# rajgandhi1/threecrate

Hardware: AMD Instinct MI355X
Metric: ICP iterations/sec (whole job: k=16 normals + 50-iter point-to-plane ICP per 1M-pt pair; tc_cloud handles, inputs resident in HBM) (higher is better)
Workload: dtype f32; 1 GPU; 1000000-pt uniform-random cloud, k=16 normals + 50-iter point-to-plane ICP, independent sigma = 0.0001 noise on source and target, correspondences returned (BASELINE configs[1]; one independent pair per GPU); points=1000000, k=16, parallelism=pairs1, interface=tc_cloud handles (one index build per cloud)

## Files before the change

threecrate_amd/csrc/cloud.hip:

```cpp
#include "tc_internal.h"

#include <algorithm>
#include <cmath>
#include <cstring>

struct tc_cloud {
    tc_context *ctx = nullptr;
    size_t n = 0;
    tc::DevBuf xyz;
    tc::DeviceIndex ix;
    bool indexed = false;
    float factor = 0.0f;
    bool has_normals = false;
    tc::DevBuf normals6;
    bool has_normals6 = false;
};

namespace {

using namespace tc;


float shared_factor(float want) {
    return (want > 0.8f * kIcpCellFactor && want < 1.25f * kIcpCellFactor) ? kIcpCellFactor : want;
}

__global__ void __launch_bounds__(256) cloud_unsort_normals_kernel(const float4 *__restrict__ pts, const float4 *__restrict__ sorted_nrm,
                                                                  const float *__restrict__ xyz, uint32_t n, float *__restrict__ out6) {
    const uint32_t p = blockIdx.x * blockDim.x + threadIdx.x;
    if (p >= n) return;
    const uint32_t orig = __float_as_uint(pts[p].w);
    const float4 nr = sorted_nrm[p];
    float *o = out6 + 6 * (size_t)orig;
    o[0] = xyz[3 * (size_t)orig]; o[1] = xyz[3 * (size_t)orig + 1]; o[2] = xyz[3 * (size_t)orig + 2];
    o[3] = nr.x; o[4] = nr.y; o[5] = nr.z;
}

tc_status ensure_index(tc_cloud *c, float want_factor, float target_ppo, float min_h) {
    tc_context *ctx = c->ctx;
    const float f = shared_factor(want_factor);
    if (c->indexed && c->factor > 0.8f * f && c->factor < 1.25f * f && min_h <= c->ix.geom.h) return TC_OK;
    if (c->has_normals && !c->has_normals6 && c->indexed && c->n) {
        if (tc_status s = ensure(ctx, c->normals6, c->n * 6 * sizeof(float))) return s;
        hipLaunchKernelGGL(cloud_unsort_normals_kernel, dim3((unsigned)((c->n + 255) / 256)), dim3(256), 0, ctx->stream,
                           (const float4 *)c->ix.pts.p, (const float4 *)c->ix.normals.p, (const float *)c->xyz.p, (uint32_t)c->n,
                           (float *)c->normals6.p);
        TC_HIP_TRY(ctx, hipGetLastError());
        c->has_normals6 = true;
    }
    c->has_normals = false;
    if (tc_status s = build_index(ctx, c->ix, (const float *)c->xyz.p, c->n, f, nullptr, nullptr, nullptr, min_h, target_ppo)) return s;
    c->indexed = true;
    c->factor = f;
    return TC_OK;
}

tc_status cloud_create(tc_context *ctx, const float *p, size_t n, bool from_host, tc_cloud **out) {
    if (!ctx || !out) return TC_INVALID_DATA;
    *out = nullptr;
    if (tc_status s = check_point_count(ctx, n)) return s;
    TC_HIP_TRY(ctx, hipSetDevice(ctx->device));
    tc_cloud *c = new tc_cloud();
    c->ctx = ctx;
    c->n = n;
    if (n) {
        tc_status s = ensure(ctx, c->xyz, n * 3 * sizeof(float));
        if (s == TC_OK && hipMemcpyAsync(c->xyz.p, p, n * 3 * sizeof(float), from_host ? hipMemcpyHostToDevice : hipMemcpyDeviceToDevice,
                                         ctx->stream) != hipSuccess) s = fail(ctx, TC_GPU, "cloud upload failed");
        if (s == TC_OK && from_host && hipStreamSynchronize(ctx->stream) != hipSuccess) s = fail(ctx, TC_GPU, "cloud upload failed");
        if (s != TC_OK) { recycle(ctx, c->xyz); delete c; return s; }
    }
    *out = c;
    return TC_OK;
}

tc_status adopt_normals(tc_cloud *c, const float *d_normals, size_t stride) {
    if (tc_status s = ensure_index(c, kIcpCellFactor, 2.5f, 0.0f)) return s;
    if (tc_status s = gather_normals(c->ctx, c->ix, d_normals, stride)) return s;
    c->has_normals = true;
    return TC_OK;
}

tc_status prepare_target(tc_cloud *tgt, bool p2plane);

tc_status cloud_icp(tc_cloud *src, tc_cloud *tgt, bool p2plane, const float init[7], size_t max_iters, float max_dist, float conv_thr,
                    tc_icp_result *res) {
    if (!src || !tgt || !res || !init) return TC_INVALID_DATA;
    tc_context *ctx = tgt->ctx;
    if (src->ctx != ctx) return fail(ctx, TC_INVALID_DATA, "source and target handles belong to different contexts");
    if (src->n == 0 || tgt->n == 0) return fail(ctx, TC_INVALID_DATA, "Source or target point cloud is empty");
    if (p2plane && !tgt->has_normals && !tgt->has_normals6)
        return fail(ctx, TC_INVALID_DATA, "target_normals length must equal the number of target points (the target handle has no normals: "
                                          "tc_cloud_estimate_normals or tc_cloud_set_normals_device first)");
    if (max_iters == 0) return fail(ctx, TC_INVALID_DATA, "Max iterations must be positive");
    TC_HIP_TRY(ctx, hipSetDevice(ctx->device));
    if (tc_status s = prepare_target(tgt, p2plane)) return s;
    return icp_run(ctx, p2plane, (const float *)src->xyz.p, src->n, (const float *)tgt->xyz.p, tgt->n, nullptr, 0, init, max_iters, max_dist,
                   conv_thr, res, true, 0, &tgt->ix, (src->indexed && src != tgt) ? &src->ix : nullptr);
}

tc_status prepare_target(tc_cloud *tgt, bool p2plane) {
    tc_context *ctx = tgt->ctx;
    if (tc_status s = ensure_index(tgt, kIcpCellFactor, 2.5f, 0.0f)) return s;
    if (p2plane && !tgt->has_normals) {
        if (!tgt->has_normals6) return fail(ctx, TC_INVALID_DATA, "the target handle has no normals in input order to re-sort after its index was rebuilt");
        if (tc_status s = gather_normals(ctx, tgt->ix, (const float *)tgt->normals6.p + 3, 6)) return s;
        tgt->has_normals = true;
    }
    return TC_OK;
}

}

extern "C" {

tc_status tc_cloud_sharded_icp(tc_comm *comm, int shard_mode, int point_to_plane, const float *d_source, size_t n_source, tc_cloud *target,
                               const float init[7], size_t max_iters, float max_dist, float conv_thr, tc_icp_result *result) try {
    if (!comm || !target || !result || !init) return TC_INVALID_DATA;
    tc_context *ctx = target->ctx;
    if (comm->ctx != ctx) return fail(ctx, TC_INVALID_DATA, "the communicator belongs to another context");
    if (shard_mode != TC_SHARD_SPATIAL && shard_mode != TC_SHARD_LOCAL && shard_mode != TC_SHARD_INDEX) return fail(ctx, TC_INVALID_DATA, "unknown shard mode");
    const bool may_be_empty = shard_mode == TC_SHARD_LOCAL && comm->nranks > 1;
    if ((n_source == 0 && !may_be_empty) || target->n == 0) return fail(ctx, TC_INVALID_DATA, "Source or target point cloud is empty");
    if (point_to_plane && !target->has_normals && !target->has_normals6)
        return fail(ctx, TC_INVALID_DATA, "target_normals length must equal the number of target points (the target handle has no normals)");
    if (max_iters == 0) return fail(ctx, TC_INVALID_DATA, "Max iterations must be positive");
    TC_HIP_TRY(ctx, hipSetDevice(ctx->device));
    if (tc_status s = prepare_target(target, point_to_plane != 0)) return s;
    return icp_run_sharded(ctx, comm, shard_mode, point_to_plane != 0, d_source, n_source, (const float *)target->xyz.p, target->n, nullptr, 0, init,
                           max_iters, max_dist, conv_thr, result, &target->ix);
} TC_CATCH_STATUS((comm ? comm->ctx : nullptr))

tc_status tc_cloud_upload(tc_context *ctx, const float *xyz, size_t n, tc_cloud **out) try { return cloud_create(ctx, xyz, n, true, out); } TC_CATCH_STATUS(ctx)
tc_status tc_cloud_upload_device(tc_context *ctx, const float *d_xyz, size_t n, tc_cloud **out) try { return cloud_create(ctx, d_xyz, n, false, out); } TC_CATCH_STATUS(ctx)
size_t tc_cloud_size(const tc_cloud *c) { return c ? c->n : 0; }
const float *tc_cloud_points_device(const tc_cloud *c) { return c ? (const float *)c->xyz.p : nullptr; }
const float *tc_cloud_normals_device(const tc_cloud *cc) try {
    tc_cloud *c = const_cast<tc_cloud *>(cc);
    if (!c || c->n == 0) return nullptr;
    if (c->has_normals6) return (const float *)c->normals6.p;
    if (!c->has_normals || !c->indexed) return nullptr;
    tc_context *ctx = c->ctx;
    if (hipSetDevice(ctx->device) != hipSuccess) { (void)fail(ctx, TC_GPU, "tc_cloud_normals_device: hipSetDevice failed"); return nullptr; }
    if (ensure(ctx, c->normals6, c->n * 6 * sizeof(float)) != TC_OK) return nullptr;
    hipLaunchKernelGGL(cloud_unsort_normals_kernel, dim3((unsigned)((c->n + 255) / 256)), dim3(256), 0, ctx->stream,
                       (const float4 *)c->ix.pts.p, (const float4 *)c->ix.normals.p, (const float *)c->xyz.p, (uint32_t)c->n,
                       (float *)c->normals6.p);
    hipError_t e = hipGetLastError();
    if (e == hipSuccess) e = hipStreamSynchronize(ctx->stream);
    if (e != hipSuccess) { (void)fail(ctx, TC_GPU, std::string("tc_cloud_normals_device: ") + hipGetErrorString(e)); return nullptr; }
    c->has_normals6 = true;
    return (const float *)c->normals6.p;
} TC_CATCH_VALUE(nullptr)

static tc_status cloud_normals(tc_cloud *c, const tc_normal_config *cfg, float *out, bool out_on_host, bool keep6) {
    if (!c || !cfg) return TC_INVALID_DATA;
    tc_context *ctx = c->ctx;
    if (c->n == 0) return TC_OK;
    if (cfg->k_neighbors < 3) return fail(ctx, TC_INVALID_DATA, "k_neighbors must be at least 3");
    TC_HIP_TRY(ctx, hipSetDevice(ctx->device));
    const float min_h = cfg->has_radius ? cfg->radius * 0.5005f : 0.0f;
    c->has_normals = false;
    c->has_normals6 = false;
    if (tc_status s = ensure_index(c, normals_cell_factor(cfg->k_neighbors, c->n >= kAdaptMinPoints), normals_target_ppo(cfg->k_neighbors), min_h)) return s;
    if (tc_status s = ensure(ctx, c->ix.normals, c->n * sizeof(float4))) return s;
    const bool direct = out != nullptr && !out_on_host && !keep6;
    const bool want6 = (out != nullptr || keep6) && !direct;
    float *d_out6 = direct ? out : nullptr;
    if (want6) {
        if (tc_status s = ensure(ctx, c->normals6, c->n * 6 * sizeof(float))) return s;
        d_out6 = (float *)c->normals6.p;
    }
    c->has_normals = false;
    c->has_normals6 = false;
    if (tc_status s = normals_on_index(ctx, c->ix, false, 0.0f, (const float *)c->xyz.p, c->n, cfg, d_out6, 0, (size_t)-1, false,
                                       (float4 *)c->ix.normals.p, true)) return s;
    c->has_normals = true;
    c->has_normals6 = want6;
    if (out && !direct) TC_HIP_TRY(ctx, hipMemcpyAsync(out, d_out6, c->n * 6 * sizeof(float), out_on_host ? hipMemcpyDeviceToHost : hipMemcpyDeviceToDevice, ctx->stream));
    TC_HIP_TRY(ctx, hipStreamSynchronize(ctx->stream));
    return TC_OK;
}

tc_status tc_cloud_estimate_normals(tc_cloud *c, const tc_normal_config *cfg, float *out) try { return cloud_normals(c, cfg, out, true, false); } TC_CATCH_STATUS(c ? c->ctx : nullptr)
tc_status tc_cloud_estimate_normals_device(tc_cloud *c, const tc_normal_config *cfg, float *d_out) try { return cloud_normals(c, cfg, d_out, false, false); } TC_CATCH_STATUS(c ? c->ctx : nullptr)

tc_status tc_cloud_set_normals_device(tc_cloud *c, const float *d_normals, size_t n_normals, size_t stride) try {
    if (!c) return TC_INVALID_DATA;
    tc_context *ctx = c->ctx;
    if (n_normals != c->n) return fail(ctx, TC_INVALID_DATA, "target_normals length must equal the number of target points");
    if (stride < 3) return fail(ctx, TC_INVALID_DATA, "normal_stride must be >= 3");
    if (c->n == 0) return TC_OK;
    TC_HIP_TRY(ctx, hipSetDevice(ctx->device));
    c->has_normals = false;
    c->has_normals6 = false;
    if (tc_status s = adopt_normals(c, d_normals, stride)) return s;
    TC_HIP_TRY(ctx, hipStreamSynchronize(ctx->stream));
    return TC_OK;
} TC_CATCH_STATUS((c ? c->ctx : nullptr))

tc_status tc_cloud_icp_point_to_plane(tc_cloud *source, tc_cloud *target, const float init[7], size_t max_iters, float max_dist,
                                      float conv_thr, tc_icp_result *result) try {
    return cloud_icp(source, target, true, init, max_iters, max_dist, conv_thr, result);
} TC_CATCH_STATUS((source ? source->ctx : nullptr))

tc_status tc_cloud_icp_detailed(tc_cloud *source, tc_cloud *target, const float init[7], size_t max_iters, float max_dist,
                                float conv_thr, tc_icp_result *result) try {
    return cloud_icp(source, target, false, init, max_iters, max_dist, conv_thr, result);
} TC_CATCH_STATUS((source ? source->ctx : nullptr))

void tc_cloud_destroy(tc_cloud *c) try {
    if (!c) return;
    (void)hipSetDevice(c->ctx->device);
    (void)hipStreamSynchronize(c->ctx->stream);
    tc::recycle(c->ctx, c->xyz); tc::recycle(c->ctx, c->normals6);
    tc::recycle_index(c->ctx, c->ix);
    delete c;
} TC_CATCH_VOID

}
```

threecrate_amd/csrc/grid.hip:

```cpp
#include "tc_internal.h"
#include <rocprim/device/device_radix_sort.hpp>

#include <algorithm>
#include <cmath>
#include <cstring>

namespace tc {

__device__ __forceinline__ void isometry_apply(const float q[4], const float t[3], float x, float y, float z,
                                               float &ox, float &oy, float &oz) {
    float tx = (q[1] * z - q[2] * y) * 2.0f;
    float ty = (q[2] * x - q[0] * z) * 2.0f;
    float tz = (q[0] * y - q[1] * x) * 2.0f;
    float cx = q[1] * tz - q[2] * ty;
    float cy = q[2] * tx - q[0] * tz;
    float cz = q[0] * ty - q[1] * tx;
    ox = ((tx * q[3] + cx) + x) + t[0];
    oy = ((ty * q[3] + cy) + y) + t[1];
    oz = ((tz * q[3] + cz) + z) + t[2];
}

constexpr int kBboxBlocks = 256;
__device__ __forceinline__ uint32_t f2ord(float f) { const uint32_t b = __float_as_uint(f); return (b & 0x80000000u) ? ~b : (b | 0x80000000u); }
__device__ __forceinline__ float ord2f(uint32_t u) { return __uint_as_float((u & 0x80000000u) ? (u ^ 0x80000000u) : ~u); }
constexpr uint32_t kOrdPlusInf = 0xFF800000u, kOrdMinusInf = 0x007FFFFFu;
constexpr uint32_t kBboxAccStride = 32;
constexpr size_t kBboxStateBytes = 31 * kBboxAccStride * sizeof(uint32_t), kBboxBufBytes = kBboxStateBytes + 128 + 256;

template <bool VEC>
__global__ void __launch_bounds__(256) bbox_kernel(const float *__restrict__ xyz, uint32_t n, uint32_t *__restrict__ state, int robust,
                                                  float *__restrict__ out, uint32_t *__restrict__ done) {
    const bool sbox = robust != 0;
    __shared__ float sm[4][30];
    float v[30];
#pragma unroll
    for (int k = 0; k < 30; ++k) v[k] = (k % 6 < 3) ? INFINITY : -INFINITY;
    auto take = [&](float x, float y, float z, uint32_t i, int s) {
        if (!(fabsf(x) <= 3.0e38f && fabsf(y) <= 3.0e38f && fabsf(z) <= 3.0e38f)) return;
        v[0] = fminf(v[0], x); v[1] = fminf(v[1], y); v[2] = fminf(v[2], z);
        v[3] = fmaxf(v[3], x); v[4] = fmaxf(v[4], y); v[5] = fmaxf(v[5], z);
        if (sbox && ((i * 2654435761u) >> 28) == 0u) {
            float *b = v + 6 + 6 * s;
            b[0] = fminf(b[0], x); b[1] = fminf(b[1], y); b[2] = fminf(b[2], z);
            b[3] = fmaxf(b[3], x); b[4] = fmaxf(b[4], y); b[5] = fmaxf(b[5], z);
        }
    };
    const uint32_t gt = blockIdx.x * blockDim.x + threadIdx.x, stride = gridDim.x * blockDim.x;
    if constexpr (VEC) {
        const float4 *__restrict__ q = reinterpret_cast<const float4 *>(xyz);
        const uint32_t nq = n >> 2;
        constexpr int U = 4;
        for (uint32_t c0 = gt; c0 < nq; c0 += U * stride) {
            float4 a[U], b[U], c[U];
#pragma unroll
            for (int u = 0; u < U; ++u) {
                const uint32_t cc = min(c0 + (uint32_t)u * stride, nq - 1u);
                a[u] = q[3 * (size_t)cc]; b[u] = q[3 * (size_t)cc + 1]; c[u] = q[3 * (size_t)cc + 2];
            }
#pragma unroll
            for (int u = 0; u < U; ++u) {
                const uint32_t i = 4u * min(c0 + (uint32_t)u * stride, nq - 1u);
                take(a[u].x, a[u].y, a[u].z, i, 0);
                take(a[u].w, b[u].x, b[u].y, i + 1u, 1);
                take(b[u].z, b[u].w, c[u].x, i + 2u, 2);
                take(c[u].y, c[u].z, c[u].w, i + 3u, 3);
            }
        }
        if (gt < (n & 3u)) {
            const uint32_t i = (nq << 2) + gt;
            const float x = xyz[3 * (size_t)i], y = xyz[3 * (size_t)i + 1], z = xyz[3 * (size_t)i + 2];
            if ((i & 3u) == 0u) take(x, y, z, i, 0); else if ((i & 3u) == 1u) take(x, y, z, i, 1); else take(x, y, z, i, 2);
        }
    } else {
        for (uint32_t i = gt; i < n; i += stride) {
            const float x = xyz[3 * (size_t)i], y = xyz[3 * (size_t)i + 1], z = xyz[3 * (size_t)i + 2];
            const uint32_t sidx = threadIdx.x & 3u;
            if (sidx == 0u) take(x, y, z, i, 0); else if (sidx == 1u) take(x, y, z, i, 1); else if (sidx == 2u) take(x, y, z, i, 2); else take(x, y, z, i, 3);
        }
    }
#pragma unroll
    for (int k = 0; k < 30; ++k) {
        if (k < 6 || sbox) {
#pragma unroll
            for (int o = 32; o > 0; o >>= 1) {
                const float w = __shfl_xor(v[k], o);
                v[k] = (k % 6 < 3) ? fminf(v[k], w) : fmaxf(v[k], w);
            }
        }
    }
    if ((threadIdx.x & 63) == 0) {
#pragma unroll
        for (int k = 0; k < 30; ++k) sm[threadIdx.x >> 6][k] = v[k];
    }
    __syncthreads();
    uint32_t *acc = state + kBboxAccStride;
    if (threadIdx.x < (sbox ? 30 : 6)) {
        const bool is_min = threadIdx.x % 6 < 3;
        float r = sm[0][threadIdx.x];
        for (int w = 1; w < 4; ++w) r = is_min ? fminf(r, sm[w][threadIdx.x]) : fmaxf(r, sm[w][threadIdx.x]);
        if (is_min) atomicMin(&acc[threadIdx.x * kBboxAccStride], f2ord(r)); else atomicMax(&acc[threadIdx.x * kBboxAccStride], f2ord(r));
    }
    __shared__ uint32_t s_last;
    if (threadIdx.x < 64) {
        asm volatile("s_waitcnt vmcnt(0)" ::: "memory");
        if (threadIdx.x == 0) s_last = __hip_atomic_fetch_add(state, 1u, __ATOMIC_RELAXED, __HIP_MEMORY_SCOPE_AGENT) == gridDim.x - 1u ? 1u : 0u;
    }
    __syncthreads();
    if (!s_last) return;
    if (threadIdx.x < 30) {
        const uint32_t u = __hip_atomic_load(&acc[threadIdx.x * kBboxAccStride], __ATOMIC_RELAXED, __HIP_MEMORY_SCOPE_AGENT);
        __hip_atomic_store(&out[threadIdx.x], ord2f(u), __ATOMIC_RELAXED, __HIP_MEMORY_SCOPE_SYSTEM);
        __hip_atomic_store(&acc[threadIdx.x * kBboxAccStride], (threadIdx.x % 6 < 3) ? kOrdPlusInf : kOrdMinusInf, __ATOMIC_RELAXED, __HIP_MEMORY_SCOPE_AGENT);
    }
    if (threadIdx.x == 0) __hip_atomic_store(state, 0u, __ATOMIC_RELAXED, __HIP_MEMORY_SCOPE_AGENT);
    if (done) {
        if (threadIdx.x < 30) __threadfence_system();
        __syncthreads();
        if (threadIdx.x == 0) __hip_atomic_store(done, 1u, __ATOMIC_RELEASE, __HIP_MEMORY_SCOPE_SYSTEM);
    }
}

__global__ void bbox_state_init_kernel(uint32_t *__restrict__ state) {
    const uint32_t t = threadIdx.x;
    if (t == 0) state[0] = 0u;
    if (t < 30) state[(t + 1) * kBboxAccStride] = (t % 6 < 3) ? kOrdPlusInf : kOrdMinusInf;
}


__global__ void __launch_bounds__(256) cell_hist_kernel(const float *__restrict__ xyz, uint32_t n, GridGeom g,
                                                       const IcpState *__restrict__ st, TileGeom tg, int tile_major, uint32_t nkeys,
                                                       uint32_t *__restrict__ cell_of, uint32_t *__restrict__ hist,
                                                       uint32_t *__restrict__ arrival, uint32_t *__restrict__ pts_pad,
                                                       uint32_t *__restrict__ cs_front, uint32_t *__restrict__ cs_tail, uint32_t rank_max) {
    uint32_t i = blockIdx.x * blockDim.x + threadIdx.x;
    if (blockIdx.x == 0 && threadIdx.x < 4 * kPtsPad + kCellStartFront + kCellStartPad) {
        const uint32_t t = threadIdx.x;
        if (t < 4 * kPtsPad) pts_pad[t] = 0x7F7F7F7Fu;
        else if (t < 4 * kPtsPad + kCellStartFront) cs_front[t - 4 * kPtsPad] = 0u;
        else cs_tail[t - 4 * kPtsPad - kCellStartFront] = 0u;
    }
    if (i >= n) return;
    float x = xyz[3 * (size_t)i], y = xyz[3 * (size_t)i + 1], z = xyz[3 * (size_t)i + 2];
    if (st) {
        float q[4] = {st->q[0], st->q[1], st->q[2], st->q[3]}, t[3] = {st->t[0], st->t[1], st->t[2]};
        float ox, oy, oz;
        isometry_apply(q, t, x, y, z, ox, oy, oz);
        x = ox; y = oy; z = oz;
    }
    int ix = cell_coord(x, g.minx, g.inv_h, g.gx);
    int iy = cell_coord(y, g.miny, g.inv_h, g.gy);
    int iz = cell_coord(z, g.minz, g.inv_h, g.gz);
    uint32_t c = tile_major ? tile_major_id(tg, ix, iy, iz) : ((uint32_t)iz * g.gy + iy) * g.gx + ix;
    if (!(fabsf(x) <= 3.0e38f && fabsf(y) <= 3.0e38f && fabsf(z) <= 3.0e38f)) c = nkeys;
    cell_of[i] = c;
    const uint32_t a = atomicAdd(&hist[c], 1u);
    arrival[i] = a;
    if (a == rank_max) hist[nkeys + 1] = 1u;
}

__global__ void __launch_bounds__(256) iota_kernel(uint32_t *__restrict__ p, uint32_t n) {
    const uint32_t i = blockIdx.x * blockDim.x + threadIdx.x;
    if (i < n) p[i] = i;
}

constexpr int kScanItems = 8;
constexpr int kScanBlock = 256;
constexpr int kScanTile = kScanItems * kScanBlock;

__global__ void __launch_bounds__(kScanBlock) scan_reduce_kernel(const uint32_t *__restrict__ in, uint32_t n,
                                                                 uint32_t *__restrict__ blocksum) {
    __shared__ uint32_t wsum[kScanBlock / 64], wnz[kScanBlock / 64];
    uint32_t base = blockIdx.x * kScanTile;
    uint32_t s = 0, nz = 0;
#pragma unroll
    for (int k = 0; k < kScanItems; ++k) {
        uint32_t i = base + k * kScanBlock + threadIdx.x;
        if (i < n) { const uint32_t v = in[i]; s += v; nz += v != 0; }
    }
#pragma unroll
    for (int o = 32; o > 0; o >>= 1) { s += __shfl_xor(s, o); nz += __shfl_xor(nz, o); }
    if ((threadIdx.x & 63) == 0) { wsum[threadIdx.x >> 6] = s; wnz[threadIdx.x >> 6] = nz; }
    __syncthreads();
    if (threadIdx.x == 0) {
        blocksum[blockIdx.x] = wsum[0] + wsum[1] + wsum[2] + wsum[3];
        blocksum[gridDim.x + blockIdx.x] = wnz[0] + wnz[1] + wnz[2] + wnz[3];
    }
}

constexpr uint32_t kScanFusedMax = 2048;
__global__ void __launch_bounds__(1024) scan_top_kernel(uint32_t *__restrict__ blocksum, uint32_t nb) {
    __shared__ uint32_t wtot[16];
    uint32_t carry = 0;
    for (uint32_t base = 0; base < nb; base += 1024) {
        const uint32_t i = base + threadIdx.x;
        const uint32_t v = i < nb ? blocksum[i] : 0u;
        uint32_t inc = v;
#pragma unroll
        for (int o = 1; o < 64; o <<= 1) {
            const uint32_t t = __shfl_up(inc, o);
            if ((threadIdx.x & 63) >= (unsigned)o) inc += t;
        }
        if ((threadIdx.x & 63) == 63) wtot[threadIdx.x >> 6] = inc;
        __syncthreads();
        uint32_t woff = 0, tot = 0;
        for (int w = 0; w < 16; ++w) { if (w < (int)(threadIdx.x >> 6)) woff += wtot[w]; tot += wtot[w]; }
        if (i < nb) blocksum[i] = carry + woff + inc - v;
        carry += tot;
        __syncthreads();
    }
}

__global__ void __launch_bounds__(kScanBlock) scan_apply_kernel(const uint32_t *__restrict__ in, uint32_t n,
                                                                uint32_t *__restrict__ blocksum,
                                                                uint32_t *__restrict__ out , uint32_t *__restrict__ occ_out, int prefixed,
                                                                unsigned long long *__restrict__ occ_host) {
    __shared__ uint32_t wtot[kScanBlock / 64];
    __shared__ uint32_t wpre[kScanBlock / 64], wnz[kScanBlock / 64];
    uint32_t pre = 0, nzt = 0;
    if (prefixed) { if (threadIdx.x == 0) pre = blocksum[blockIdx.x]; }
    else for (uint32_t i = threadIdx.x; i < blockIdx.x; i += kScanBlock) pre += blocksum[i];
    if (blockIdx.x == 0) for (uint32_t i = threadIdx.x; i < gridDim.x; i += kScanBlock) nzt += blocksum[gridDim.x + i];
#pragma unroll
    for (int o = 32; o > 0; o >>= 1) { pre += __shfl_xor(pre, o); nzt += __shfl_xor(nzt, o); }
    if ((threadIdx.x & 63) == 0) { wpre[threadIdx.x >> 6] = pre; wnz[threadIdx.x >> 6] = nzt; }
    uint32_t base = blockIdx.x * kScanTile + threadIdx.x * kScanItems;
    uint32_t v[kScanItems];
    uint32_t s = 0;
#pragma unroll
    for (int k = 0; k < kScanItems; ++k) {
        uint32_t i = base + k;
        v[k] = (i < n) ? in[i] : 0;
        s += v[k];
    }
    uint32_t inc = s;
#pragma unroll
    for (int o = 1; o < 64; o <<= 1) {
        uint32_t t = __shfl_up(inc, o);
        if ((threadIdx.x & 63) >= (unsigned)o) inc += t;
    }
    if ((threadIdx.x & 63) == 63) wtot[threadIdx.x >> 6] = inc;
    __syncthreads();
    uint32_t woff = 0;
    for (int w = 0; w < (int)(threadIdx.x >> 6); ++w) woff += wtot[w];
    uint32_t block_pre = 0;
    for (int w = 0; w < kScanBlock / 64; ++w) block_pre += wpre[w];
    if (blockIdx.x == 0 && threadIdx.x == 0) {
        uint32_t t = 0;
        for (int w = 0; w < kScanBlock / 64; ++w) t += wnz[w];
        blocksum[2 * gridDim.x] = t;
        if (occ_out) *occ_out = t;
        if (occ_host) __hip_atomic_store(occ_host, (1ull << 32) | (unsigned long long)t, __ATOMIC_RELAXED, __HIP_MEMORY_SCOPE_SYSTEM);
    }
    uint32_t run = block_pre + woff + inc - s;
#pragma unroll
    for (int k = 0; k < kScanItems; ++k) {
        uint32_t i = base + k;
        if (i < n) out[i] = run;
        run += v[k];
        if (i == n - 1) out[n] = run;
    }
}

__global__ void __launch_bounds__(256) rank_gather_kernel(const float *__restrict__ xyz, uint32_t n, uint32_t nkeys,
                                                         const uint32_t *__restrict__ cell_of,
                                                         const uint32_t *__restrict__ cell_start,
                                                         const uint32_t *__restrict__ slot,
                                                         float4 *__restrict__ pts, int slot_is_ordered, uint32_t rank_max) {
    uint32_t p = blockIdx.x * blockDim.x + threadIdx.x;
    if (p >= n) return;
    uint32_t i = slot[p];
    uint32_t c = cell_of[i];
    uint32_t s = cell_start[c], e = cell_start[c + 1];
    uint32_t rank;
    if (slot_is_ordered) {
        rank = p - s;
    } else if (e - s <= rank_max) {
        rank = 0;
        for (uint32_t j = s; j < e; ++j) rank += (slot[j] < i) ? 1u : 0u;
    } else {
        rank = p - s;
    }
    float4 r;
    r.x = xyz[3 * (size_t)i]; r.y = xyz[3 * (size_t)i + 1]; r.z = xyz[3 * (size_t)i + 2];
    if (c == nkeys) r.x = r.y = r.z = __uint_as_float(0x7F7F7F7Fu);
    r.w = __uint_as_float(i);
    pts[s + rank] = r;
}

__global__ void __launch_bounds__(256) place_kernel(const float *__restrict__ xyz, uint32_t n, uint32_t nkeys,
                                                   const uint32_t *__restrict__ cell_of, const uint32_t *__restrict__ cell_start,
                                                   const uint32_t *__restrict__ arrival, float4 *__restrict__ tmp) {
    const uint32_t i = blockIdx.x * blockDim.x + threadIdx.x;
    if (i >= n) return;
    const uint32_t c = cell_of[i];
    const uint32_t pos = cell_start[c] + arrival[i];
    float4 r;
    r.x = xyz[3 * (size_t)i]; r.y = xyz[3 * (size_t)i + 1]; r.z = xyz[3 * (size_t)i + 2];
    if (c == nkeys) r.x = r.y = r.z = __uint_as_float(0x7F7F7F7Fu);
    r.w = __uint_as_float(i);
    tmp[pos] = r;
}

__global__ void __launch_bounds__(256) rerank_kernel(uint32_t n, GridGeom g, const IcpState *__restrict__ st, TileGeom tg, int tile_major,
                                                    uint32_t nkeys, const uint32_t *__restrict__ cell_start, const float4 *__restrict__ tmp,
                                                    float4 *__restrict__ pts, uint32_t rank_max) {
    const uint32_t p = blockIdx.x * blockDim.x + threadIdx.x;
    if (p >= n) return;
    const float4 r = tmp[p];
    uint32_t c;
    {
        float x = r.x, y = r.y, z = r.z;
        if (st) {
            float q[4] = {st->q[0], st->q[1], st->q[2], st->q[3]}, t[3] = {st->t[0], st->t[1], st->t[2]};
            float ox, oy, oz;
            isometry_apply(q, t, x, y, z, ox, oy, oz);
            x = ox; y = oy; z = oz;
        }
        const int ix = cell_coord(x, g.minx, g.inv_h, g.gx), iy = cell_coord(y, g.miny, g.inv_h, g.gy), iz = cell_coord(z, g.minz, g.inv_h, g.gz);
        c = tile_major ? tile_major_id(tg, ix, iy, iz) : ((uint32_t)iz * g.gy + iy) * g.gx + ix;
        if (!(fabsf(x) <= 3.0e38f && fabsf(y) <= 3.0e38f && fabsf(z) <= 3.0e38f)) c = nkeys;
    }
    const uint32_t s = cell_start[c], e = cell_start[c + 1];
    const uint32_t i = __float_as_uint(r.w);
    uint32_t rank;
    if (e - s <= rank_max) {
        rank = 0;
#pragma unroll 4
        for (uint32_t j = s; j < e; ++j) rank += (__float_as_uint(tmp[j].w) < i) ? 1u : 0u;
    } else {
        rank = p - s;
    }
    pts[s + rank] = r;
}

__global__ void __launch_bounds__(256) gather_normals_kernel(const float4 *__restrict__ pts, uint32_t n,
                                                            const float *__restrict__ nrm, size_t stride,
                                                            float4 *__restrict__ out) {
    uint32_t p = blockIdx.x * blockDim.x + threadIdx.x;
    if (p >= n) return;
    uint32_t i = __float_as_uint(pts[p].w);
    const float *s = nrm + (size_t)i * stride;
    out[p] = make_float4(s[0], s[1], s[2], 0.0f);
}

GridView view_of(const DeviceIndex &ix) {
    GridView v;
    v.g = ix.geom;
    v.pts = (const float4 *)ix.pts.p;
    v.cell_start = (const uint32_t *)ix.cell_start.p + kCellStartFront;
    v.pts12 = ix.pts12_valid ? (const float *)ix.pts12.p : nullptr;
    return v;
}

static void set_cell_edge(GridGeom &g, double h, size_t n, double cells_per_point) {
    const double e[3] = {(double)g.maxx - g.minx, (double)g.maxy - g.miny, (double)g.maxz - g.minz};
    const double max_cells = std::max<double>(cells_per_point * (double)n, 4096.0);
    for (int guard = 0; guard < 200; ++guard) {
        double gx = std::floor(e[0] / h) + 1.0, gy = std::floor(e[1] / h) + 1.0, gz = std::floor(e[2] / h) + 1.0;
        if (gx * gy * gz <= max_cells && gx * gy * gz < 2.0e9) {
            g.gx = (int)gx; g.gy = (int)gy; g.gz = (int)gz;
            break;
        }
        h *= 1.2;
    }
    g.h = (float)h;
    g.inv_h = 1.0f / g.h;
    g.ncell = (uint32_t)g.gx * (uint32_t)g.gy * (uint32_t)g.gz;
    g.n = (uint32_t)n;
}

static void derive_geom(GridGeom &g, const float mn[3], const float mx[3], size_t n, float f, float min_h) {
    g.minx = mn[0]; g.miny = mn[1]; g.minz = mn[2];
    g.maxx = mx[0]; g.maxy = mx[1]; g.maxz = mx[2];
    g.cx = 0.5f * (mn[0] + mx[0]); g.cy = 0.5f * (mn[1] + mx[1]); g.cz = 0.5f * (mn[2] + mx[2]);
    double e[3] = {(double)mx[0] - mn[0], (double)mx[1] - mn[1], (double)mx[2] - mn[2]};
    double emax = std::max(e[0], std::max(e[1], e[2]));
    double h = 1.0;
    if (!(emax > 0.0) || !std::isfinite(emax)) {
        h = 1.0;
    } else {
        double measure = 1.0;
        int dims = 0;
        for (int a = 0; a < 3; ++a)
            if (e[a] > 1e-6 * emax) { measure *= e[a]; ++dims; }
        h = f * std::pow(measure / (double)std::max<size_t>(n, 1), 1.0 / (double)dims);
        if (!(h > 0.0) || !std::isfinite(h)) h = emax;
        h = std::max(h, emax * 1e-4);
    }
    if (min_h > 0.0f && std::isfinite(min_h)) h = std::max(h, (double)min_h);
    set_cell_edge(g, h, n, 8.0);
}

TileGeom make_tiles(const GridGeom &g, int tx, int ty, int tz) {
    TileGeom t;
    t.tx = std::max(tx, 1); t.ty = std::max(ty, 1); t.tz = std::max(tz, 1);
    t.ntx = (g.gx + t.tx - 1) / t.tx; t.nty = (g.gy + t.ty - 1) / t.ty; t.ntz = (g.gz + t.tz - 1) / t.tz;
    t.cpt = (uint32_t)(t.tx * t.ty * t.tz);
    t.ntiles = (uint32_t)t.ntx * (uint32_t)t.nty * (uint32_t)t.ntz;
    return t;
}

tc_status exclusive_scan_u32(tc_context *ctx, const uint32_t *d_in, uint32_t n, uint32_t *d_out, DevBuf &blocksum, uint32_t *occ_out,
                             unsigned long long *occ_host) {
    hipStream_t st = ctx->stream;
    const uint32_t nscan = (n + kScanTile - 1) / kScanTile;
    if (tc_status s = ensure(ctx, blocksum, ((size_t)2 * nscan + 1) * sizeof(uint32_t))) return s;
    hipLaunchKernelGGL(scan_reduce_kernel, dim3(nscan), dim3(kScanBlock), 0, st, d_in, n, (uint32_t *)blocksum.p);
    const char *fm = getenv("TC_SCAN_FUSED_MAX");
    const bool prefixed = nscan > (fm ? (uint32_t)atoi(fm) : kScanFusedMax);
    if (prefixed) hipLaunchKernelGGL(scan_top_kernel, dim3(1), dim3(1024), 0, st, (uint32_t *)blocksum.p, nscan);
    hipLaunchKernelGGL(scan_apply_kernel, dim3(nscan), dim3(kScanBlock), 0, st, d_in, n, (uint32_t *)blocksum.p, d_out, occ_out, prefixed ? 1 : 0, occ_host);
    TC_HIP_TRY(ctx, hipGetLastError());
    return TC_OK;
}

static tc_status cloud_bbox_impl(tc_context *ctx, const float *d_xyz, size_t n, float mn[3], float mx[3], float *rmn, float *rmx,
                                 bool *clamped) {
    hipStream_t st = ctx->stream;
    const int nb = (int)((n + 255) / 256);
    const int bb = std::min(nb, kBboxBlocks);
    const bool robust = rmn != nullptr && n >= 4096;
    const bool poll = pinned_poll_enabled();
    const bool fresh = ctx->bbox.p == nullptr;
    if (tc_status s = ensure(ctx, ctx->bbox, kBboxBufBytes)) return s;
    uint32_t *d_state = (uint32_t *)ctx->bbox.p;
    if (fresh) hipLaunchKernelGGL(bbox_state_init_kernel, dim3(1), dim3(64), 0, st, d_state);
    float *hb = (float *)((char *)ctx->pinned + 2048);
    volatile uint32_t *h_done = (volatile uint32_t *)((char *)ctx->pinned + 2048 + 8192 + 192);
    float *d_out = (float *)((char *)ctx->bbox.p + kBboxStateBytes + 128);
    uint32_t *d_done = nullptr;
    if (poll) {
        d_out = (float *)pinned_dev_ptr(ctx, hb);
        d_done = (uint32_t *)pinned_dev_ptr(ctx, (const void *)h_done);
        if (!d_out || !d_done) return fail(ctx, TC_GPU, "bbox: the pinned block has no device address");
        *h_done = 0u;
    }
    {
        ProfScope ps(ctx, "bbox");
        if (((uintptr_t)d_xyz & 15u) == 0u)
            hipLaunchKernelGGL(bbox_kernel<true>, dim3(std::min((int)((n / 4 + 255) / 256) + 1, kBboxBlocks)), dim3(256), 0, st, d_xyz, (uint32_t)n, d_state, robust ? 1 : 0, d_out, d_done);
        else
            hipLaunchKernelGGL(bbox_kernel<false>, dim3(bb), dim3(256), 0, st, d_xyz, (uint32_t)n, d_state, robust ? 1 : 0, d_out, d_done);
    }
    TC_HIP_TRY(ctx, hipGetLastError());
    if (poll) {
        if (tc_status s = wait_pinned_word(ctx, h_done, "bounding box")) { hipLaunchKernelGGL(bbox_state_init_kernel, dim3(1), dim3(64), 0, st, d_state); return s; }
    } else {
        TC_HIP_TRY(ctx, hipMemcpyAsync(hb, d_out, 30 * sizeof(float), hipMemcpyDeviceToHost, st));
        TC_HIP_TRY(ctx, hipStreamSynchronize(st));
    }
    const float *hs = hb + 6;
    for (int c = 0; c < 3; ++c) { mn[c] = INFINITY; mx[c] = -INFINITY; }
    for (int c = 0; c < 3; ++c) { mn[c] = std::fmin(mn[c], hb[c]); mx[c] = std::fmax(mx[c], hb[3 + c]); }
    if (rmn) {
        for (int c = 0; c < 3; ++c) { rmn[c] = mn[c]; rmx[c] = mx[c]; }
        *clamped = false;
    }
    if (!robust) return TC_OK;
    float acc[24];
    for (int i = 0; i < 24; ++i) acc[i] = (i % 6 < 3) ? INFINITY : -INFINITY;
    for (int i = 0; i < 24; ++i) acc[i] = (i % 6 < 3) ? (hs[i] < acc[i] ? hs[i] : acc[i]) : (hs[i] > acc[i] ? hs[i] : acc[i]);
    for (int c = 0; c < 3; ++c) {
        float lo[4], hi[4];
        for (int k = 0; k < 4; ++k) { lo[k] = acc[6 * k + c]; hi[k] = acc[6 * k + 3 + c]; }
        std::sort(lo, lo + 4);
        std::sort(hi, hi + 4, [](float a, float b) { return a > b; });
        const float slo = lo[2], shi = hi[2];
        if (!(slo <= shi) || !std::isfinite(slo) || !std::isfinite(shi)) continue;
        const float ext = shi - slo, full = mx[c] - mn[c];
        if (!(full > 1.3f * ext) || !(full > 0.0f)) continue;
        rmn[c] = std::fmax(mn[c], slo - 0.05f * ext);
        rmx[c] = std::fmin(mx[c], shi + 0.05f * ext);
        *clamped = true;
    }
    return TC_OK;
}

tc_status cloud_bbox(tc_context *ctx, const float *d_xyz, size_t n, float mn[3], float mx[3]) {
    return cloud_bbox_impl(ctx, d_xyz, n, mn, mx, nullptr, nullptr, nullptr);
}


constexpr int kBinBlocks = 256;
constexpr int kBinWalkThreads = 1024;
#ifndef TC_BIN_TARGET
#define TC_BIN_TARGET 2048
#endif
#ifndef TC_BIN_PLACE_THREADS
#define TC_BIN_PLACE_THREADS 512
#endif
constexpr uint32_t kBinTarget = TC_BIN_TARGET;
constexpr uint32_t kBinCap = 2 * kBinTarget;
constexpr uint32_t kBinKeysMax = 2 * kBinTarget;
static_assert((kBinKeysMax + 3 * kBinCap) * sizeof(uint32_t) + 256 <= 160 * 1024, "bin_place_kernel's static LDS exceeds a gfx950 CU's 160 KB");
#if defined(__HIP_DEVICE_COMPILE__) && !defined(__gfx950__)
#error "libthreecrate_hip is written for gfx950 (MI355X): bin_place_kernel alone needs more than 64 KB of LDS per workgroup"
#endif
constexpr uint32_t kBinMaxBins = 8192;
constexpr int kBinPlaceThreads = TC_BIN_PLACE_THREADS;

__device__ __forceinline__ uint32_t point_key(float x, float y, float z, const GridGeom &g, const IcpState *__restrict__ st, const TileGeom &tg,
                                              int tile_major, uint32_t nkeys) {
    if (st) {
        float q[4] = {st->q[0], st->q[1], st->q[2], st->q[3]}, t[3] = {st->t[0], st->t[1], st->t[2]};
        float ox, oy, oz;
        isometry_apply(q, t, x, y, z, ox, oy, oz);
        x = ox; y = oy; z = oz;
    }
    const int ix = cell_coord(x, g.minx, g.inv_h, g.gx), iy = cell_coord(y, g.miny, g.inv_h, g.gy), iz = cell_coord(z, g.minz, g.inv_h, g.gz);
    uint32_t c = tile_major ? tile_major_id(tg, ix, iy, iz) : ((uint32_t)iz * g.gy + iy) * g.gx + ix;
    if (!(fabsf(x) <= 3.0e38f && fabsf(y) <= 3.0e38f && fabsf(z) <= 3.0e38f)) c = nkeys;
    return c;
}

__global__ void __launch_bounds__(kBinWalkThreads) bin_count_kernel(const float *__restrict__ xyz, uint32_t n, GridGeom g, const IcpState *__restrict__ st,
                                                       TileGeom tg, int tile_major, uint32_t nkeys, uint32_t kpb, uint32_t nbins,
                                                       uint32_t *__restrict__ cnt , uint32_t *__restrict__ pts_pad,
                                                       uint32_t *__restrict__ cs_front, uint32_t *__restrict__ cs_tail) {
    __shared__ uint32_t c[kBinMaxBins];
    if (blockIdx.x == 0 && threadIdx.x < 4 * kPtsPad + kCellStartFront + kCellStartPad) {
        const uint32_t t = threadIdx.x;
        if (t < 4 * kPtsPad) pts_pad[t] = 0x7F7F7F7Fu;
        else if (t < 4 * kPtsPad + kCellStartFront) cs_front[t - 4 * kPtsPad] = 0u;
        else cs_tail[t - 4 * kPtsPad - kCellStartFront] = 0u;
    }
    for (uint32_t b = threadIdx.x; b < nbins; b += kBinWalkThreads) c[b] = 0u;
    __syncthreads();
    const uint32_t per = (n + kBinBlocks - 1) / kBinBlocks;
    const uint32_t i0 = blockIdx.x * per, i1 = min(i0 + per, n);
    for (uint32_t i = i0 + threadIdx.x; i < i1; i += kBinWalkThreads) {
        const uint32_t k = point_key(xyz[3 * (size_t)i], xyz[3 * (size_t)i + 1], xyz[3 * (size_t)i + 2], g, st, tg, tile_major, nkeys);
        atomicAdd(&c[min(k / kpb, nbins - 1u)], 1u);
    }
    __syncthreads();
    for (uint32_t b = threadIdx.x; b < nbins; b += kBinWalkThreads) cnt[(size_t)b * kBinBlocks + blockIdx.x] = c[b];
}

static_assert(kBinBlocks == 256, "one wave x four entries per lane");
__global__ void __launch_bounds__(256) bin_offsets_kernel(uint32_t *__restrict__ cnt, uint32_t nbins, uint32_t *__restrict__ tot) {
    const uint32_t b = blockIdx.x * 4u + (threadIdx.x >> 6), lane = threadIdx.x & 63u;
    if (b >= nbins) return;
    uint4 *row = reinterpret_cast<uint4 *>(cnt + (size_t)b * kBinBlocks);
    const uint4 v = row[lane];
    const uint32_t s = v.x + v.y + v.z + v.w;
    uint32_t inc = s;
#pragma unroll
    for (int o = 1; o < 64; o <<= 1) {
        const uint32_t t = __shfl_up(inc, o);
        if (lane >= (unsigned)o) inc += t;
    }
    const uint32_t ex = inc - s;
    row[lane] = make_uint4(ex, ex + v.x, ex + v.x + v.y, ex + v.x + v.y + v.z);
    if (lane == 63u) tot[b] = inc;
}

__global__ void __launch_bounds__(kBinWalkThreads) bin_scatter_kernel(const float *__restrict__ xyz, uint32_t n, GridGeom g, const IcpState *__restrict__ st,
                                                         TileGeom tg, int tile_major, uint32_t nkeys, uint32_t kpb, uint32_t nbins,
                                                         const uint32_t *__restrict__ off ,
                                                         const uint32_t *__restrict__ tot, uint32_t *__restrict__ binstart,
                                                         uint32_t *__restrict__ occ_ticket, unsigned long long *__restrict__ host_word,
                                                         float4 *__restrict__ tmp) {
    static_assert(kBinWalkThreads == 1024, "the scan below is written for 16 waves");
    __shared__ uint32_t cur[kBinMaxBins];
    __shared__ uint32_t wtot[16], wmax[16];
    uint32_t carry = 0, mx = 0;
    for (uint32_t base = 0; base < nbins; base += kBinWalkThreads) {
        const uint32_t i = base + threadIdx.x;
        const uint32_t v = i < nbins ? tot[i] : 0u;
        const uint32_t o_mine = i < nbins ? off[(size_t)i * kBinBlocks + blockIdx.x] : 0u;
        mx = max(mx, v);
        uint32_t inc = v;
#pragma unroll
        for (int o = 1; o < 64; o <<= 1) {
            const uint32_t t = __shfl_up(inc, o);
            if ((threadIdx.x & 63) >= (unsigned)o) inc += t;
        }
        if ((threadIdx.x & 63) == 63) wtot[threadIdx.x >> 6] = inc;
        __syncthreads();
        uint32_t woff = 0, total = 0;
        for (int w = 0; w < 16; ++w) { if (w < (int)(threadIdx.x >> 6)) woff += wtot[w]; total += wtot[w]; }
        const uint32_t start = carry + woff + inc - v;
        if (i < nbins) {
            cur[i] = start + o_mine;
            if (blockIdx.x == 0) binstart[i] = start;
        }
        carry += total;
        __syncthreads();
    }
    if (blockIdx.x == 0) {
#pragma unroll
        for (int o = 32; o > 0; o >>= 1) mx = max(mx, (uint32_t)__shfl_xor(mx, o));
        if ((threadIdx.x & 63) == 0) wmax[threadIdx.x >> 6] = mx;
        __syncthreads();
        if (threadIdx.x == 0) {
            binstart[nbins] = carry;
            uint32_t m = 0;
            for (int w = 0; w < 16; ++w) m = max(m, wmax[w]);
            occ_ticket[0] = 0u; occ_ticket[1] = 0u;
            occ_ticket[2] = m;
            __hip_atomic_store(host_word, (1ull << 32) | (unsigned long long)m, __ATOMIC_RELAXED, __HIP_MEMORY_SCOPE_SYSTEM);
        }
    }
    const uint32_t per = (n + kBinBlocks - 1) / kBinBlocks;
    const uint32_t i0 = blockIdx.x * per, i1 = min(i0 + per, n);
    for (uint32_t i = i0 + threadIdx.x; i < i1; i += kBinWalkThreads) {
        float4 r;
        r.x = xyz[3 * (size_t)i]; r.y = xyz[3 * (size_t)i + 1]; r.z = xyz[3 * (size_t)i + 2];
        const uint32_t k = point_key(r.x, r.y, r.z, g, st, tg, tile_major, nkeys);
        if (k == nkeys) r.x = r.y = r.z = __uint_as_float(0x7F7F7F7Fu);
        r.w = __uint_as_float(i);
        tmp[atomicAdd(&cur[min(k / kpb, nbins - 1u)], 1u)] = r;
    }
}

__global__ void __launch_bounds__(kBinPlaceThreads) bin_place_kernel(const float4 *__restrict__ tmp, const uint32_t *__restrict__ binstart,
                                                                     uint32_t nbins, uint32_t kpb, uint32_t nkeys, GridGeom g,
                                                                     const IcpState *__restrict__ st, TileGeom tg, int tile_major,
                                                                     uint32_t *__restrict__ cs, float4 *__restrict__ pts,
                                                                     uint32_t *__restrict__ occ_ticket, uint32_t *__restrict__ occ_out,
                                                                     unsigned long long *__restrict__ occ_host) {
    __shared__ uint32_t cnt[kBinKeysMax];
    __shared__ uint32_t rkey[kBinCap];
    __shared__ uint32_t ridx[kBinCap];
    __shared__ uint32_t slot[kBinCap];
    __shared__ uint32_t wsum[kBinPlaceThreads / 64];
    __shared__ uint32_t s_occ;
    const uint32_t bin = blockIdx.x, tid = threadIdx.x;
    if (occ_ticket[2] > kBinCap) return;
    const uint32_t bs = binstart[bin], P = binstart[bin + 1] - bs;
    const uint32_t k0 = bin * kpb, K = min(kpb, nkeys + 1u - k0);
    for (uint32_t k = tid; k < K; k += kBinPlaceThreads) cnt[k] = 0u;
    if (tid == 0) s_occ = 0u;
    __syncthreads();
    for (uint32_t i = tid; i < P; i += kBinPlaceThreads) {
        const float4 r = tmp[bs + i];
        const uint32_t k = min(point_key(r.x, r.y, r.z, g, st, tg, tile_major, nkeys) - k0, K - 1u);
        const uint32_t a = atomicAdd(&cnt[k], 1u);
        rkey[i] = k | (a << 16);
        ridx[i] = __float_as_uint(r.w);
    }
    __syncthreads();
    constexpr uint32_t kPer = kBinKeysMax / kBinPlaceThreads;
    uint32_t v[kPer], sum = 0, nz = 0;
#pragma unroll
    for (uint32_t t = 0; t < kPer; ++t) {
        const uint32_t k = tid * kPer + t;
        v[t] = k < K ? cnt[k] : 0u;
        sum += v[t];
        nz += v[t] != 0u;
    }
    uint32_t inc = sum;
#pragma unroll
    for (int o = 1; o < 64; o <<= 1) {
        const uint32_t t2 = __shfl_up(inc, o);
        if ((tid & 63) >= (unsigned)o) inc += t2;
    }
#pragma unroll
    for (int o = 32; o > 0; o >>= 1) nz += __shfl_xor(nz, o);
    if ((tid & 63) == 63) wsum[tid >> 6] = inc;
    if ((tid & 63) == 0 && nz) atomicAdd(&s_occ, nz);
    __syncthreads();
    uint32_t run = inc - sum;
    for (uint32_t w = 0; w < (tid >> 6); ++w) run += wsum[w];
#pragma unroll
    for (uint32_t t = 0; t < kPer; ++t) {
        const uint32_t k = tid * kPer + t;
        if (k < K) { cnt[k] = run; cs[k0 + k] = bs + run; }
        run += v[t];
    }
    if (bin == nbins - 1 && tid == 0) cs[nkeys + 1] = bs + P;
    __syncthreads();
    for (uint32_t i = tid; i < P; i += kBinPlaceThreads) slot[cnt[rkey[i] & 0xFFFFu] + (rkey[i] >> 16)] = ridx[i];
    __syncthreads();
    for (uint32_t i = tid; i < P; i += kBinPlaceThreads) {
        const uint32_t k = rkey[i] & 0xFFFFu, me = ridx[i];
        const uint32_t s0 = cnt[k], e0 = (k + 1 < K) ? cnt[k + 1] : P;
        uint32_t rank = 0;
        for (uint32_t j = s0; j < e0; ++j) rank += slot[j] < me ? 1u : 0u;
        rkey[i] = s0 + rank;
    }
    __syncthreads();
    for (uint32_t i = tid; i < P; i += kBinPlaceThreads) slot[rkey[i]] = i;
    __syncthreads();
    for (uint32_t t = tid; t < P; t += kBinPlaceThreads) pts[bs + t] = tmp[bs + slot[t]];
    if (tid == 0) {
        const unsigned long long mine = ((unsigned long long)s_occ << 32) | 1ull;
        const unsigned long long old = __hip_atomic_fetch_add(reinterpret_cast<unsigned long long *>(occ_ticket), mine, __ATOMIC_RELAXED, __HIP_MEMORY_SCOPE_AGENT);
        if ((uint32_t)old == nbins - 1u) {
            const uint32_t occ = (uint32_t)(old >> 32) + s_occ;
            if (occ_out) __hip_atomic_store(occ_out, occ, __ATOMIC_RELAXED, __HIP_MEMORY_SCOPE_AGENT);
            if (occ_host) __hip_atomic_store(occ_host, (1ull << 32) | (unsigned long long)occ, __ATOMIC_RELAXED, __HIP_MEMORY_SCOPE_SYSTEM);
        }
    }
}

static uint32_t rank_quadratic_max() {
    const char *e = getenv("TC_RANK_QUADRATIC_MAX");
    return e ? (uint32_t)std::max(1, atoi(e)) : kRankQuadraticMax;
}

static bool binned_build_enabled() {
    const char *e = getenv("TC_INDEX_BINNED");
    return !(e && atoi(e) == 0);
}

tc_status build_index(tc_context *ctx, DeviceIndex &ix, const float *d_xyz, size_t n, float cell_factor,
                      const GridGeom *reuse_geom, const IcpState *d_state_transform, const TileGeom *tile_major,
                      float min_cell_edge, float target_ppo, bool strict_order) {
    if (n == 0 || n >= kMaxPoints) return fail(ctx, TC_INVALID_DATA, "build_index: bad point count");
    ctx->stat_indexed_points += n;
    ctx->stat_index_builds += 1;
    ix.vor_valid = false;
    ix.pts12_valid = false;
    ix.occ_host_valid = false;
    hipStream_t st = ctx->stream;
    const uint32_t n32 = (uint32_t)n;
    const int nb = (int)((n + 255) / 256);
    const int dbg = debug_flags();
    const uint32_t rank_max = rank_quadratic_max();

    if (reuse_geom) {
        ix.geom = *reuse_geom;
        ix.geom.n = n32;
    } else {
        float mn[3], mx[3], rmn[3], rmx[3];
        bool clamped = false;
        if (tc_status s = cloud_bbox_impl(ctx, d_xyz, n, mn, mx, rmn, rmx, &clamped)) return s;
        if (dbg & 2048) clamped = false, std::memcpy(rmn, mn, sizeof(mn)), std::memcpy(rmx, mx, sizeof(mx));
        for (int c = 0; c < 3; ++c) {
            if (!(mn[c] <= mx[c]) || !std::isfinite(mn[c]) || !std::isfinite(mx[c])) { mn[c] = 0.0f; mx[c] = 0.0f; rmn[c] = 0.0f; rmx[c] = 0.0f; }
            ix.exact_min[c] = mn[c]; ix.exact_max[c] = mx[c];
        }
        derive_geom(ix.geom, rmn, rmx, n, cell_factor, min_cell_edge);
        ix.geom.clamped = clamped ? 1 : 0;
        if ((dbg & 256) && clamped)
            fprintf(stderr, "[tc] index: box clamped to %g..%g %g..%g %g..%g (exact %g..%g %g..%g %g..%g)\n", rmn[0], rmx[0], rmn[1], rmx[1],
                    rmn[2], rmx[2], mn[0], mx[0], mn[1], mx[1], mn[2], mx[2]);
    }
    const bool adapt = target_ppo > 0.0f && !reuse_geom && !tile_major && n >= kAdaptMinPoints && !(dbg & 512);
    uint32_t nkeys_final = 0;
    const uint32_t *cs_final = nullptr;
    for (int attempt = 0;; ++attempt) {
        const GridGeom g = ix.geom;
        TileGeom tg{};
        uint32_t nkeys = g.ncell;
        if (tile_major) {
            tg = *tile_major;
            ix.tile = tg;
            const uint64_t nk = (uint64_t)tg.ntiles * tg.cpt;
            if (nk >= kMaxPoints) return fail(ctx, TC_UNSUPPORTED, "tile-major key space too large");
            nkeys = (uint32_t)nk;
        }

        if (tc_status s = ensure(ctx, ix.pts, (n + kPtsPad) * sizeof(float4))) return s;
        if (tc_status s = ensure(ctx, ix.cell_of, n * sizeof(uint32_t))) return s;
        if (tc_status s = ensure(ctx, ix.slot, n * sizeof(uint32_t))) return s;
        if (tc_status s = ensure(ctx, ix.arrival, n * sizeof(uint32_t))) return s;
        const size_t fill_bytes = (((size_t)nkeys + 2) * sizeof(uint32_t) + 255) & ~(size_t)255;
        if (tc_status s = ensure(ctx, ix.fill, fill_bytes)) return s;
        if (tc_status s = ensure(ctx, ix.cell_start, (kCellStartFront + (size_t)nkeys + 2 + kCellStartPad) * sizeof(uint32_t))) return s;
        uint32_t *const cs = (uint32_t *)ix.cell_start.p + kCellStartFront;
        nkeys_final = nkeys; cs_final = cs;
        const bool check = adapt && attempt < 3;
        volatile uint32_t *h_occ = (volatile uint32_t *)((char *)ctx->pinned + 2048 + 8192);

        bool binned_done = false;
        if (binned_build_enabled() && pinned_poll_enabled() && !strict_order && n >= kAdaptMinPoints && n <= (1u << 24) && nkeys < 0x7FFFFFF0u) {
            const uint32_t keys = nkeys + 1u;
            uint32_t nbins = std::max<uint32_t>((n32 + kBinTarget - 1) / kBinTarget, (keys + kBinKeysMax - 1) / kBinKeysMax);
            const uint32_t kpb = (keys + nbins - 1) / nbins;
            nbins = (keys + kpb - 1) / kpb;
            if (nbins <= kBinMaxBins && kpb <= kBinKeysMax) {
                const size_t words = 4 + (size_t)kBinBlocks * nbins + nbins + (nbins + 1);
                if (tc_status s = ensure(ctx, ix.fill, std::max(fill_bytes, words * sizeof(uint32_t)))) return s;
                uint32_t *occ_ticket = (uint32_t *)ix.fill.p, *cnt = occ_ticket + 4, *tot = cnt + (size_t)kBinBlocks * nbins, *binstart = tot + nbins;
                volatile uint32_t *h_max = (volatile uint32_t *)((char *)ctx->pinned + 2048 + 8192 + 256);
                unsigned long long *d_max = (unsigned long long *)pinned_dev_ptr(ctx, (const void *)h_max);
                if (!d_max) return fail(ctx, TC_GPU, "index build: the pinned block has no device address");
                h_max[0] = 0u; h_max[1] = 0u;
                {
                    ProfScope ps(ctx, "cell_bin_count");
                    hipLaunchKernelGGL(bin_count_kernel, dim3(kBinBlocks), dim3(kBinWalkThreads), 0, st, d_xyz, n32, g, d_state_transform, tg, tile_major ? 1 : 0, nkeys, kpb,
                                       nbins, cnt, reinterpret_cast<uint32_t *>((float4 *)ix.pts.p + n), (uint32_t *)ix.cell_start.p, cs + nkeys + 2);
                }
                {
                    ProfScope ps(ctx, "cell_bin_offsets");
                    hipLaunchKernelGGL(bin_offsets_kernel, dim3((nbins + 3) / 4), dim3(256), 0, st, cnt, nbins, tot);
                }
                if (tc_status s = ensure(ctx, ctx->build_tmp, (n + kPtsPad) * sizeof(float4))) return s;
                {
                    ProfScope ps(ctx, "cell_bin_scatter");
                    hipLaunchKernelGGL(bin_scatter_kernel, dim3(kBinBlocks), dim3(kBinWalkThreads), 0, st, d_xyz, n32, g, d_state_transform, tg, tile_major ? 1 : 0, nkeys,
                                       kpb, nbins, (const uint32_t *)cnt, (const uint32_t *)tot, binstart, occ_ticket, d_max, (float4 *)ctx->build_tmp.p);
                }
                if (check) { h_occ[0] = 0u; h_occ[1] = 0u; }
                unsigned long long *d_occ_host = check ? (unsigned long long *)pinned_dev_ptr(ctx, (const void *)h_occ) : nullptr;
                {
                    ProfScope ps(ctx, "cell_bin_place");
                    hipLaunchKernelGGL(bin_place_kernel, dim3(nbins), dim3(kBinPlaceThreads), 0, st, (const float4 *)ctx->build_tmp.p, (const uint32_t *)binstart,
                                       nbins, kpb, nkeys, g, d_state_transform, tg, tile_major ? 1 : 0, cs, (float4 *)ix.pts.p, occ_ticket,
                                       (uint32_t *)ix.cell_start.p, d_occ_host);
                }
                TC_HIP_TRY(ctx, hipGetLastError());
                if (tc_status s = wait_pinned_word(ctx, h_max + 1, "index build (bin populations)")) return s;
                if (h_max[0] <= kBinCap) {
                    binned_done = true;
                } else if (dbg & 256) {
                    fprintf(stderr, "[tc] index: largest bin holds %u points (> %u): atomic counting sort\n", h_max[0], kBinCap);
                }
            }
        }
        if (!binned_done) {
        TC_HIP_TRY(ctx, hipMemsetAsync(ix.fill.p, 0, fill_bytes, st));
        {
            ProfScope ps(ctx, "cell_hist");
            hipLaunchKernelGGL(cell_hist_kernel, dim3(nb), dim3(256), 0, st, d_xyz, n32, g, d_state_transform, tg, tile_major ? 1 : 0, nkeys,
                               (uint32_t *)ix.cell_of.p, (uint32_t *)ix.fill.p, (uint32_t *)ix.arrival.p,
                               reinterpret_cast<uint32_t *>((float4 *)ix.pts.p + n), (uint32_t *)ix.cell_start.p, cs + nkeys + 2, rank_max);
        }
        {
            ProfScope ps(ctx, "cell_scan");
            if (check) { h_occ[0] = 0u; h_occ[1] = 0u; }
            unsigned long long *d_occ_host = (check && pinned_poll_enabled()) ? (unsigned long long *)pinned_dev_ptr(ctx, (const void *)h_occ) : nullptr;
            if (check && pinned_poll_enabled() && !d_occ_host) return fail(ctx, TC_GPU, "index build: the pinned block has no device address");
            if (tc_status s = exclusive_scan_u32(ctx, (const uint32_t *)ix.fill.p, nkeys + 1, cs, ix.blocksum, (uint32_t *)ix.cell_start.p, d_occ_host)) return s;
        }
        if (tc_status s = ensure(ctx, ctx->build_tmp, (n + kPtsPad) * sizeof(float4))) return s;
        {
            ProfScope ps(ctx, "cell_place");
            hipLaunchKernelGGL(place_kernel, dim3(nb), dim3(256), 0, st, d_xyz, n32, nkeys, (const uint32_t *)ix.cell_of.p, (const uint32_t *)cs,
                               (const uint32_t *)ix.arrival.p, (float4 *)ctx->build_tmp.p);
        }
        {
            ProfScope ps(ctx, "cell_rerank");
            hipLaunchKernelGGL(rerank_kernel, dim3(nb), dim3(256), 0, st, n32, g, d_state_transform, tg, tile_major ? 1 : 0, nkeys, (const uint32_t *)cs,
                               (const float4 *)ctx->build_tmp.p, (float4 *)ix.pts.p, rank_max);
        }
        }
        TC_HIP_TRY(ctx, hipGetLastError());
        if (!check) break;
        if (pinned_poll_enabled()) {
            if (tc_status s = wait_pinned_word(ctx, h_occ + 1, "index build (occupied cells)")) return s;
        } else {
            const uint32_t nscan = (nkeys + 1 + kScanTile - 1) / kScanTile;
            TC_HIP_TRY(ctx, hipMemcpyAsync((void *)h_occ, (const uint32_t *)ix.blocksum.p + 2 * nscan, sizeof(uint32_t), hipMemcpyDeviceToHost, st));
            TC_HIP_TRY(ctx, hipStreamSynchronize(st));
        }
        const uint32_t occ_now = h_occ[0];
        const double ppo = (double)n / (double)std::max<uint32_t>(occ_now, 1u);
        ix.occ_host = occ_now; ix.occ_host_valid = true;
        if (dbg & 256)
            fprintf(stderr, "[tc] index: n %zu h %.5f grid %d x %d x %d = %u cells (%.2f n), %u occupied, %.2f points each (want %.1f)\n", n,
                    g.h, g.gx, g.gy, g.gz, g.ncell, (double)g.ncell / (double)n, occ_now, ppo, target_ppo);
        if (!(ppo > 2.0 * target_ppo)) break;
        double h = (double)g.h * std::min(0.8, std::max(0.35, std::sqrt((double)target_ppo / ppo)));
        if (min_cell_edge > 0.0f) h = std::max(h, (double)min_cell_edge);
        GridGeom ng = g;
        set_cell_edge(ng, h, n, 32.0);
        if (!(ng.h < 0.95f * g.h)) break;
        ix.geom = ng;
        ix.occ_host_valid = false;
    }
    if (strict_order) {
        uint32_t *h_big = (uint32_t *)((char *)ctx->pinned + 2048 + 8192 + 64);
        TC_HIP_TRY(ctx, hipMemcpyAsync(h_big, (const uint32_t *)ix.fill.p + nkeys_final + 1, sizeof(uint32_t), hipMemcpyDeviceToHost, st));
        TC_HIP_TRY(ctx, hipStreamSynchronize(st));
        if (*h_big) {
            if (tc_status s = ensure(ctx, ctx->overflow, n * sizeof(uint32_t))) return s;
            uint32_t *iota = (uint32_t *)ix.arrival.p, *keys_out = (uint32_t *)ctx->overflow.p;
            hipLaunchKernelGGL(iota_kernel, dim3(nb), dim3(256), 0, st, iota, n32);
            unsigned bits = 1;
            while (bits < 32 && (1ull << bits) <= (unsigned long long)nkeys_final) ++bits;
            size_t temp_bytes = 0;
            TC_HIP_TRY(ctx, rocprim::radix_sort_pairs(nullptr, temp_bytes, (const uint32_t *)ix.cell_of.p, keys_out, (const uint32_t *)iota,
                                                      (uint32_t *)ix.slot.p, n, 0u, bits, st));
            if (tc_status s = ensure(ctx, ix.blocksum, temp_bytes)) return s;
            TC_HIP_TRY(ctx, rocprim::radix_sort_pairs(ix.blocksum.p, temp_bytes, (const uint32_t *)ix.cell_of.p, keys_out, (const uint32_t *)iota,
                                                      (uint32_t *)ix.slot.p, n, 0u, bits, st));
            ProfScope ps(ctx, "cell_rank_gather_strict");
            hipLaunchKernelGGL(rank_gather_kernel, dim3(nb), dim3(256), 0, st, d_xyz, n32, nkeys_final, (const uint32_t *)ix.cell_of.p,
                               (const uint32_t *)cs_final, (const uint32_t *)ix.slot.p, (float4 *)ix.pts.p, 1, rank_max);
            TC_HIP_TRY(ctx, hipGetLastError());
        }
    }
    return TC_OK;
}

tc_status gather_normals(tc_context *ctx, DeviceIndex &ix, const float *d_normals, size_t stride) {
    const size_t n = ix.geom.n;
    if (tc_status s = ensure(ctx, ix.normals, n * sizeof(float4))) return s;
    ProfScope ps(ctx, "gather_normals");
    hipLaunchKernelGGL(gather_normals_kernel, dim3((unsigned)((n + 255) / 256)), dim3(256), 0, ctx->stream,
                       (const float4 *)ix.pts.p, (uint32_t)n, d_normals, stride, (float4 *)ix.normals.p);
    TC_HIP_TRY(ctx, hipGetLastError());
    return TC_OK;
}

}
```

threecrate_amd/csrc/icp.hip:

```cpp
#include "tc_internal.h"
#include <hip/hip_ext.h>

#include <algorithm>
#include <type_traits>
#include <cmath>
#include <cstring>
#include <cstdlib>
#include <cstdio>

namespace tc {

__device__ __forceinline__ void iso_apply(const float q[4], const float t[3], float x, float y, float z,
                                          float &ox, float &oy, float &oz) {
    float tx = (q[1] * z - q[2] * y) * 2.0f;
    float ty = (q[2] * x - q[0] * z) * 2.0f;
    float tz = (q[0] * y - q[1] * x) * 2.0f;
    float cx = q[1] * tz - q[2] * ty;
    float cy = q[2] * tx - q[0] * tz;
    float cz = q[0] * ty - q[1] * tx;
    ox = ((tx * q[3] + cx) + x) + t[0];
    oy = ((ty * q[3] + cy) + y) + t[1];
    oz = ((tz * q[3] + cz) + z) + t[2];
}

// ... 691 lines not shown
__device__ __forceinline__ unsigned long long refine_shell(const GridView &tgt, const __amdgpu_buffer_rsrc_t &cs_rsrc,
                                                           const __amdgpu_buffer_rsrc_t &pt_rsrc, int Rrt, int lg, float x, float y,
                                                           float z, int cx, int cy, int cz, unsigned long long bestkey, bool &touched) {
    const GridGeom &g = tgt.g;
    const int R = RC > 0 ? RC : Rrt;
    const int W = 2 * R + 1, V = W - 2;
    const int ncell = 2 * W * W + 2 * W * V + 2 * V * V;
    const float bestd = __uint_as_float((uint32_t)(bestkey >> 32));
    const bool have = bestkey != ~0ull;
    unsigned long long lk = ~0ull;
    touched = false;
    for (int idx0 = lg; idx0 < ncell; idx0 += kRG * kRB) {
        uint32_t s0[kRB], e0[kRB];
#pragma unroll
        for (int t = 0; t < kRB; ++t) {
            const int idx = idx0 + t * kRG;
            int ox = 0, oy = 0, oz = 0;
            shell_cell(min(idx, ncell - 1), R, W, V, ox, oy, oz);
            const int ccx = cx + ox, ccy = cy + oy, ccz = cz + oz;
            bool in = idx < ncell && ccx >= 0 && ccx < g.gx && ccy >= 0 && ccy < g.gy && ccz >= 0 && ccz < g.gz;
            if (in && have) {
                const float gx = axis_gap(x, g.minx, g.h, ccx, g.gx - 1, g.clamped), gy = axis_gap(y, g.miny, g.h, ccy, g.gy - 1, g.clamped),
                            gz = axis_gap(z, g.minz, g.h, ccz, g.gz - 1, g.clamped);
                in = !(gx * gx + gy * gy + gz * gz > bestd);
            }
            touched |= in;
            const uint32_t c = in ? ((uint32_t)ccz * g.gy + ccy) * g.gx + ccx : 0u;
            const uint2 w = __builtin_bit_cast(uint2, __builtin_amdgcn_raw_buffer_load_b64(cs_rsrc, c << 2, 0, 0));
            s0[t] = w.x;
            e0[t] = in ? w.y : w.x;
        }
#pragma unroll
        for (int t = 0; t < kRB; ++t) {
            const uint32_t jj = s0[t], o = jj << 4;
            const f32x3 p0 = __builtin_bit_cast(f32x3, __builtin_amdgcn_raw_buffer_load_b96(pt_rsrc, o, 0, 0));
            const f32x3 p1 = __builtin_bit_cast(f32x3, __builtin_amdgcn_raw_buffer_load_b96(pt_rsrc, o + 16u, 0, 0));
            const f32x3 p2 = __builtin_bit_cast(f32x3, __builtin_amdgcn_raw_buffer_load_b96(pt_rsrc, o + 32u, 0, 0));
            const f32x3 p3 = __builtin_bit_cast(f32x3, __builtin_amdgcn_raw_buffer_load_b96(pt_rsrc, o + 48u, 0, 0));
            const unsigned long long k0 = ((unsigned long long)__float_as_uint(d2_nc(p0.x, p0.y, p0.z, x, y, z)) << 32) | jj;
            const unsigned long long k1 = ((unsigned long long)__float_as_uint(d2_nc(p1.x, p1.y, p1.z, x, y, z)) << 32) | (jj + 1);
            const unsigned long long k2 = ((unsigned long long)__float_as_uint(d2_nc(p2.x, p2.y, p2.z, x, y, z)) << 32) | (jj + 2);
            const unsigned long long k3 = ((unsigned long long)__float_as_uint(d2_nc(p3.x, p3.y, p3.z, x, y, z)) << 32) | (jj + 3);
            const unsigned long long ka = k0 < k1 ? k0 : k1, kb = k2 < k3 ? k2 : k3;
            const unsigned long long kc = ka < kb ? ka : kb;
            if (s0[t] < e0[t]) lk = kc < lk ? kc : lk;
        }
#pragma unroll
        for (int t = 0; t < kRB; ++t) {
            for (uint32_t jj = s0[t] + 4; jj < e0[t]; ++jj) {
                const f32x3 p = __builtin_bit_cast(f32x3, __builtin_amdgcn_raw_buffer_load_b96(pt_rsrc, jj << 4, 0, 0));
                const unsigned long long key = ((unsigned long long)__float_as_uint(d2_nc(p.x, p.y, p.z, x, y, z)) << 32) | jj;
                lk = key < lk ? key : lk;
            }
        }
    }
    return group_min_u64(lk);
}

__device__ __forceinline__ unsigned long long refine_ball_scan(const GridView &tgt, const __amdgpu_buffer_rsrc_t &cs_rsrc,
                                                               const __amdgpu_buffer_rsrc_t &pt_rsrc, int lg, float x, float y, float z,
                                                               unsigned long long bestkey, float cap2) {
    const GridGeom &g = tgt.g;
    float lim = fminf(__uint_as_float((uint32_t)(bestkey >> 32)), cap2);
    const float ox = g.clamped ? 0.0f : fmaxf(fmaxf(g.minx - x, x - g.maxx), 0.0f) * 0.9999f;
    const float oy = g.clamped ? 0.0f : fmaxf(fmaxf(g.miny - y, y - g.maxy), 0.0f) * 0.9999f;
    const float oz = g.clamped ? 0.0f : fmaxf(fmaxf(g.minz - z, z - g.maxz), 0.0f) * 0.9999f;
    const float ry = sqrtf(fmaxf(lim - ox * ox - oz * oz, 0.0f)) * 1.0001f + 4e-3f * g.h;
    const float rz = sqrtf(fmaxf(lim - ox * ox - oy * oy, 0.0f)) * 1.0001f + 4e-3f * g.h;
    const int y0 = cell_coord(fminf(fmaxf(y - ry, g.miny), g.maxy), g.miny, g.inv_h, g.gy), y1 = cell_coord(fminf(fmaxf(y + ry, g.miny), g.maxy), g.miny, g.inv_h, g.gy);
    const int z0 = cell_coord(fminf(fmaxf(z - rz, g.minz), g.maxz), g.minz, g.inv_h, g.gz), z1 = cell_coord(fminf(fmaxf(z + rz, g.minz), g.maxz), g.minz, g.inv_h, g.gz);
    const int ny = y1 - y0 + 1;
    const uint32_t nrows = (uint32_t)ny * (uint32_t)(z1 - z0 + 1);
    unsigned long long lk = bestkey;
    uint32_t batch = 0;
    for (uint32_t r0i = (uint32_t)lg; r0i < nrows; r0i += kRG * kRB, ++batch) {
        uint32_t s0[kRB], e0[kRB];
#pragma unroll
        for (int t = 0; t < kRB; ++t) {
            const uint32_t ri = r0i + (uint32_t)t * kRG;
            const int zz = z0 + (int)(min(ri, nrows - 1) / (uint32_t)ny), yy = y0 + (int)(min(ri, nrows - 1) % (uint32_t)ny);
            const float gy = axis_gap(y, g.miny, g.h, yy, g.gy - 1, g.clamped), gz = axis_gap(z, g.minz, g.h, zz, g.gz - 1, g.clamped);
            const float rg = gy * gy + gz * gz;
            bool in = ri < nrows && !(rg + ox * ox > lim);
            int xa = 0, xb = 0;
            if (in) {
                const float rx = __builtin_amdgcn_sqrtf(fmaxf(lim - rg, 0.0f)) * 1.0001f + 4e-3f * g.h;
                const float fa = fminf(fmaxf((x - rx - g.minx) * g.inv_h, 0.0f), (float)(g.gx - 1));
                const float fb = fmaxf(fminf((x + rx - g.minx) * g.inv_h, (float)(g.gx - 1)), 0.0f);
                xa = (int)fa; xb = (int)fb;
                in = xa <= xb;
            }
            const uint32_t row = ((uint32_t)zz * g.gy + yy) * g.gx;
            uint32_t s = 0, e = 0;
            if (in) {
                s = __builtin_amdgcn_raw_buffer_load_b32(cs_rsrc, (row + (uint32_t)xa) << 2, 0, 0);
                e = __builtin_amdgcn_raw_buffer_load_b32(cs_rsrc, (row + (uint32_t)xb + 1u) << 2, 0, 0);
            }
            s0[t] = s; e0[t] = e;
        }
#pragma unroll
        for (int t = 0; t < kRB; ++t) {
            for (uint32_t jj = s0[t]; jj < e0[t]; jj += 4) {
                const uint32_t o = jj << 4;
                const f32x3 p0 = __builtin_bit_cast(f32x3, __builtin_amdgcn_raw_buffer_load_b96(pt_rsrc, o, 0, 0));
                const f32x3 p1 = __builtin_bit_cast(f32x3, __builtin_amdgcn_raw_buffer_load_b96(pt_rsrc, o + 16u, 0, 0));
                const f32x3 p2 = __builtin_bit_cast(f32x3, __builtin_amdgcn_raw_buffer_load_b96(pt_rsrc, o + 32u, 0, 0));
                const f32x3 p3 = __builtin_bit_cast(f32x3, __builtin_amdgcn_raw_buffer_load_b96(pt_rsrc, o + 48u, 0, 0));
                const unsigned long long k0 = ((unsigned long long)__float_as_uint(d2_nc(p0.x, p0.y, p0.z, x, y, z)) << 32) | jj;
                const unsigned long long k1 = ((unsigned long long)__float_as_uint(d2_nc(p1.x, p1.y, p1.z, x, y, z)) << 32) | (jj + 1);
                const unsigned long long k2 = ((unsigned long long)__float_as_uint(d2_nc(p2.x, p2.y, p2.z, x, y, z)) << 32) | (jj + 2);
                const unsigned long long k3 = ((unsigned long long)__float_as_uint(d2_nc(p3.x, p3.y, p3.z, x, y, z)) << 32) | (jj + 3);
                const unsigned long long ka = k0 < k1 ? k0 : k1, kb = k2 < k3 ? k2 : k3;
                const unsigned long long kc = ka < kb ? ka : kb;
                lk = kc < lk ? kc : lk;
            }
        }
        lim = fminf(lim, __uint_as_float((uint32_t)(lk >> 32)));
        if ((batch & 3u) == 3u) {
            float gl = lim;
#pragma unroll
            for (int o = kRG / 2; o > 0; o >>= 1) gl = fminf(gl, __shfl_xor(gl, o));
            lim = gl;
        }
    }
    return group_min_u64(lk);
}

template <int MODE>
__global__ void __launch_bounds__(kRefineThreads) icp_refine_kernel(
    GridView tgt, const float4 *__restrict__ tgt_nrm, const float4 *__restrict__ src,
    IcpState *__restrict__ st, uint32_t *__restrict__ corr_pos , uint32_t *__restrict__ rlist,
    const double *__restrict__ main_rows, uint32_t n_main_rows, uint32_t seg_stride, double *__restrict__ partial_rows,
    const float4 *__restrict__ src_cov, int dbg) {
    constexpr bool P2PLANE = MODE == 1;
    constexpr int NACC = MODE == 0 ? TC_ICP_SUMS_P2P : TC_ICP_SUMS_P2PLANE;
    const IcpHeader hd = load_header(st);
    const bool dbg_shells = (dbg & 8192) != 0;
    __shared__ float lacc[kRefineThreads / kRG][TC_ICP_SUMS_STRIDE];
    const uint32_t rows_per = (n_main_rows + gridDim.x - 1) / gridDim.x;
    const uint32_t mr0 = min(blockIdx.x * rows_per, n_main_rows), mr1 = min(mr0 + rows_per, n_main_rows);
    constexpr int kFoldBatch = kMaxPartialBlocks / kRefineBlocks;
    double fr[kFoldBatch];
#pragma unroll
    for (int k = 0; k < kFoldBatch; ++k) {
        const double v = main_rows[(size_t)min(mr0 + k, n_main_rows - 1) * TC_ICP_SUMS_STRIDE + (threadIdx.x & (TC_ICP_SUMS_STRIDE - 1))];
        fr[k] = (mr0 + k < mr1) ? v : 0.0;
    }
    constexpr int kSegPerRow = kIcpBlock / 64;
    constexpr int kCntPer = kMaxPartialBlocks * kSegPerRow / kRefineThreads;
    const uint32_t n_segs = n_main_rows * kSegPerRow;
    constexpr uint32_t per = kCntPer;
    uint32_t cnt[kCntPer];
#pragma unroll
    for (int k = 0; k < kCntPer; ++k) {
        const uint32_t b = threadIdx.x * per + k;
        const uint32_t v = rlist[min(b, n_segs - 1)];
        cnt[k] = b < n_segs ? v : 0u;
    }
    if (hd.done) return;
    double folded = 0.0;
#pragma unroll
    for (int k = 0; k < kFoldBatch; ++k) folded += fr[k];
    if (threadIdx.x < TC_ICP_SUMS_STRIDE)
        for (uint32_t r = mr0 + kFoldBatch; r < mr1; ++r) folded += main_rows[(size_t)r * TC_ICP_SUMS_STRIDE + threadIdx.x];
    const GridGeom &g = tgt.g;
    const float q[4] = {hd.q[0], hd.q[1], hd.q[2], hd.q[3]};
    const float max_dist = hd.max_dist;
    __shared__ uint32_t seg_off[kMaxPartialBlocks * kSegPerRow + 1];
    __shared__ uint32_t wave_tot[kRefineThreads / 64];
    {
        uint32_t run = 0;
#pragma unroll
        for (int k = 0; k < kCntPer; ++k) run += cnt[k];
        uint32_t inc = run;
#pragma unroll
        for (int o = 1; o < 64; o <<= 1) {
            const uint32_t v = __shfl_up(inc, o);
            if ((int)(threadIdx.x & 63) >= o) inc += v;
        }
        if ((threadIdx.x & 63) == 63) wave_tot[threadIdx.x >> 6] = inc;
        __syncthreads();
        uint32_t ex = inc - run;
        for (int w2 = 0; w2 < (int)(threadIdx.x >> 6); ++w2) ex += wave_tot[w2];
#pragma unroll
        for (int k = 0; k < kCntPer; ++k) {
            const uint32_t b = threadIdx.x * per + k;
            if (b <= n_segs) seg_off[b] = ex;
            ex += cnt[k];
        }
        if (threadIdx.x == kRefineThreads - 1) seg_off[n_segs] = ex;
        __syncthreads();
    }
    const uint32_t count = seg_off[n_segs];
    const uint4 *__restrict__ entries = refine_entries(rlist);
    if (blockIdx.x == 0 && threadIdx.x == 0) {
        st->refine_total += count;
        st->refine_max = max(st->refine_max, count);
    }
    if ((uint32_t)blockIdx.x >= count) {
        if (threadIdx.x < TC_ICP_SUMS_STRIDE) partial_rows[(size_t)blockIdx.x * TC_ICP_SUMS_STRIDE + threadIdx.x] = folded;
        return;
    }
    const __amdgpu_buffer_rsrc_t pt_rsrc = raw_rsrc(tgt.pts), cs_rsrc = raw_rsrc(tgt.cell_start);
    const int lg = threadIdx.x & (kRG - 1);
    const uint32_t group = (threadIdx.x / kRG) * gridDim.x + blockIdx.x, ngroups = gridDim.x * kRefineThreads / kRG;
    const unsigned long long gmask = (kRG == 64) ? ~0ull : (((1ull << kRG) - 1ull) << ((threadIdx.x & 63) & ~(kRG - 1)));
    float *const acc = lacc[threadIdx.x / kRG];
    for (int k = lg; k < NACC; k += kRG) acc[k] = 0.0f;
    __builtin_amdgcn_fence(__ATOMIC_RELEASE, "wavefront");
    auto locate = [&](uint32_t i) -> size_t {
        uint32_t lo = 0, nleft = n_segs;
        while (nleft > 1) {
            const uint32_t stride = (nleft + kRG - 1) / kRG;
            const bool le = (uint32_t)lg * stride < nleft && seg_off[lo + lg * stride] <= i;
            const uint32_t m = (uint32_t)((__ballot(le) & gmask) >> ((threadIdx.x & 63) & ~(kRG - 1)));
            const uint32_t k = 31u - (uint32_t)__clz((int)m);
            lo += k * stride;
            nleft = min(stride, nleft - k * stride);
        }
        return (size_t)lo * seg_stride + (i - seg_off[lo]);
    };
    uint4 n0 = make_uint4(0, 0, 0, 0), n1 = n0;
    if (group < count) { const size_t a = locate(group); n0 = entries[2 * a]; n1 = entries[2 * a + 1]; }
    for (uint32_t i = group; i < count; i += ngroups) {
        const uint4 e0 = n0, e1 = n1;
        if (i + ngroups < count) { const size_t a = locate(i + ngroups); n0 = entries[2 * a]; n1 = entries[2 * a + 1]; }
        const uint32_t j = e0.w, pj = e1.y;
        const float x = __uint_as_float(e0.x), y = __uint_as_float(e0.y), z = __uint_as_float(e0.z);
        const float qx = fminf(fmaxf(x, g.minx), g.maxx), qy = fminf(fmaxf(y, g.miny), g.maxy),
                    qz = fminf(fmaxf(z, g.minz), g.maxz);
        const int cx = cell_coord(qx, g.minx, g.inv_h, g.gx), cy = cell_coord(qy, g.miny, g.inv_h, g.gy),
                  cz = cell_coord(qz, g.minz, g.inv_h, g.gz);
        const float fx = (qx - g.minx) * g.inv_h - (float)cx, fy = (qy - g.miny) * g.inv_h - (float)cy,
                    fz = (qz - g.minz) * g.inv_h - (float)cz;
        const float out2 = outside_d2(x, y, z, qx, qy, qz, g.clamped);
        unsigned long long bestkey = ~0ull;
        if (pj != 0xFFFFFFFFu) bestkey = ((unsigned long long)e1.x << 32) | pj;
        if (bestkey != ~0ull && !dbg_shells)
            bestkey = refine_ball_scan(tgt, cs_rsrc, pt_rsrc, lg, x, y, z, bestkey, max_dist >= 0.0f ? max_dist * max_dist * 1.0001f : INFINITY);
        else
        for (int R = 2;; ++R) {
            bool touched;
            const unsigned long long lk = (R == 2) ? refine_shell<2>(tgt, cs_rsrc, pt_rsrc, 2, lg, x, y, z, cx, cy, cz, bestkey, touched)
                                                   : refine_shell<0>(tgt, cs_rsrc, pt_rsrc, R, lg, x, y, z, cx, cy, cz, bestkey, touched);
            bestkey = lk < bestkey ? lk : bestkey;
            const bool any_touched = (__ballot(touched) & gmask) != 0ull;
            const bool covers = (cx - R <= 0) && (cx + R >= g.gx - 1) && (cy - R <= 0) && (cy + R >= g.gy - 1) &&
                                (cz - R <= 0) && (cz + R >= g.gz - 1);
            const float big = 1.0e30f;
            const float mf = fmaxf(fminf(fminf(fminf(cx - R >= 1 ? fx : big, cx + R <= g.gx - 2 ? 1.0f - fx : big),
                                               fminf(cy - R >= 1 ? fy : big, cy + R <= g.gy - 2 ? 1.0f - fy : big)),
                                         fminf(cz - R >= 1 ? fz : big, cz + R <= g.gz - 2 ? 1.0f - fz : big)), 0.0f);
            const float bound = ((float)R + mf - 2e-3f) * g.h;
            const float bd = __uint_as_float((uint32_t)(bestkey >> 32));
#ifdef TC_REFINE_STATS
            if (lg == 0 && (covers || !any_touched || (bestkey != ~0ull && bd <= bound * bound + out2) || (max_dist >= 0.0f && bound > max_dist)))
                atomicAdd(const_cast<uint32_t *>(&st->refine_ring_hist[min(R, 7)]), 1u);
#endif
            if (covers || !any_touched) break;
            if (bestkey != ~0ull && bd <= bound * bound + out2) break;
            if (max_dist >= 0.0f && bound > max_dist) break;
            if (bestkey != ~0ull && !(dbg_shells)) {
                bestkey = refine_ball_scan(tgt, cs_rsrc, pt_rsrc, lg, x, y, z, bestkey, max_dist >= 0.0f ? max_dist * max_dist * 1.0001f : INFINITY);
                break;
            }
        }
        if (lg == 0) {
            const float best = __uint_as_float((uint32_t)(bestkey >> 32));
            const uint32_t bestg = (uint32_t)bestkey;
            bool valid = bestkey != ~0ull;
            if (valid && max_dist >= 0.0f) valid = !(sqrtf(best) > max_dist);
            corr_pos[4 * (size_t)j] = valid ? bestg : 0xFFFFFFFFu;
            if (valid) {
                const float4 c = tgt.pts[bestg];
                float a[NACC];
#pragma unroll
                for (int k = 0; k < NACC; ++k) a[k] = acc[k];
                if constexpr (MODE == 2) {
                    float R[9];
                    quat_to_rot(q, R);
                    accumulate_gicp(a, x, y, z, c, best, R, src_cov[2 * (size_t)j], src_cov[2 * (size_t)j + 1], tgt_nrm[2 * (size_t)bestg],
                                    tgt_nrm[2 * (size_t)bestg + 1]);
                } else {
                    float4 n = make_float4(0.f, 0.f, 0.f, 0.f);
                    if (P2PLANE) n = tgt_nrm[bestg];
                    accumulate_pair<P2PLANE, NACC>(g, a, x, y, z, c, n);
                }
#pragma unroll
                for (int k = 0; k < NACC; ++k) acc[k] = a[k];
            }
        }
    }
    __syncthreads();
    if (threadIdx.x < TC_ICP_SUMS_STRIDE) {
        double sum = 0.0;
        if (threadIdx.x < NACC) {
#pragma unroll 8
            for (int g2 = 0; g2 < kRefineThreads / kRG; ++g2) sum += (double)lacc[g2][threadIdx.x];
        }
        partial_rows[(size_t)blockIdx.x * TC_ICP_SUMS_STRIDE + threadIdx.x] = sum + folded;
    }
}

__global__ void __launch_bounds__(256) icp_write_corr_kernel(GridView tgt, const float4 *__restrict__ src, uint32_t ns,
                                                            const uint32_t *__restrict__ corr_pos,
                                                            uint32_t *__restrict__ corr) {
    const uint32_t j = blockIdx.x * blockDim.x + threadIdx.x;
    if (j >= ns) return;
    const uint32_t so = __float_as_uint(src[j].w);
    const uint32_t pj = corr_pos[4 * (size_t)j];
    corr[so] = (pj == 0xFFFFFFFFu) ? 0xFFFFFFFFu : __float_as_uint(tgt.pts[pj].w);
}

__global__ void __launch_bounds__(kIcpBlock) icp_final_mse_kernel(GridView tgt, const float4 *__restrict__ src, uint32_t ns,
                                                                  uint32_t chunk, const IcpState *__restrict__ st,
                                                                  const uint32_t *__restrict__ corr_pos,
                                                                  double *__restrict__ partials) {
    if (st->done) return;
    __shared__ double red[kIcpBlock / 64][TC_ICP_SUMS_STRIDE];
    const float q[4] = {st->q[0], st->q[1], st->q[2], st->q[3]};
    const float t[3] = {st->t[0], st->t[1], st->t[2]};
    double acc[2] = {0.0, 0.0};
    const uint32_t beg = blockIdx.x * chunk, end = min(beg + chunk, ns);
    for (uint32_t j = beg + threadIdx.x; j < end; j += kIcpBlock) {
        const float4 s = src[j];
        const uint32_t bj = __float_as_uint(s.w);
        if (bj == 0xFFFFFFFFu) continue;
        float x, y, z;
        iso_apply(q, t, s.x, s.y, s.z, x, y, z);
        const float4 c = tgt.pts[bj];
        const float ex = x - c.x, ey = y - c.y, ez = z - c.z;
        acc[0] += (double)(ex * ex + ey * ey + ez * ez);
        acc[1] += 1.0;
    }
    block_reduce_store<2>(acc, partials + (size_t)blockIdx.x * TC_ICP_SUMS_STRIDE, red);
}

__global__ void __launch_bounds__(256) icp_target_nn_bound_kernel(GridView tgt, float4 *__restrict__ vor, const IcpState *__restrict__ st) {
    const uint32_t p = blockIdx.x * blockDim.x + threadIdx.x;
    const GridGeom &g = tgt.g;
    if (p >= g.n || (st && st->done)) return;
    const float4 q = tgt.pts[p];
    const int cx = cell_coord(q.x, g.minx, g.inv_h, g.gx), cy = cell_coord(q.y, g.miny, g.inv_h, g.gy), cz = cell_coord(q.z, g.minz, g.inv_h, g.gz);
    const int x0 = max(cx - 1, 0), x1 = min(cx + 1, g.gx - 1);
    const float hb = 0.996f * g.h;
    float m = hb * hb;
    for (int z = max(cz - 1, 0); z <= min(cz + 1, g.gz - 1); ++z)
        for (int y = max(cy - 1, 0); y <= min(cy + 1, g.gy - 1); ++y) {
            const uint32_t row = ((uint32_t)z * g.gy + y) * g.gx;
            const uint32_t s = tgt.cell_start[row + x0], e = tgt.cell_start[row + x1 + 1];
            for (uint32_t j = s; j < e; ++j) {
                const float4 c = tgt.pts[j];
                const float v = d2_nc(c.x, c.y, c.z, q.x, q.y, q.z);
                m = (j != p) ? fminf(m, v) : m;
            }
        }
    vor[p] = make_float4(q.x, q.y, q.z, 0.25f * 0.9999f * m);
}

__device__ __forceinline__ constexpr int tri(int r, int c) { return r * (r + 1) / 2 + c; }
__device__ __forceinline__ bool chol6_solve(const double *Su, const double *b, double (&x)[6]) {
    double L[21];
    {
        int o = 0;
#pragma unroll
        for (int r = 0; r < 6; ++r)
#pragma unroll
            for (int c = r; c < 6; ++c) { L[tri(c, r)] = Su[o]; ++o; }
    }
    bool ok = true;
    double rinv[6];
#pragma unroll
    for (int j = 0; j < 6; ++j) {
#pragma unroll
        for (int k = 0; k < j; ++k) {
            const double f = L[tri(j, k)];
#pragma unroll
            for (int r = j; r < 6; ++r) L[tri(r, j)] -= f * L[tri(r, k)];
        }
        const double d = L[tri(j, j)];
        ok = ok && (d > 0.0);
        const double dp = d > 0.0 ? d : 1.0;
        double inv = __builtin_amdgcn_rsq(dp);
        inv = inv * fma(-0.5 * dp * inv, inv, 1.5);
        inv = inv * fma(-0.5 * dp * inv, inv, 1.5);
        const double sd = dp * inv;
        rinv[j] = inv;
        L[tri(j, j)] = sd;
#pragma unroll
        for (int r = j + 1; r < 6; ++r) L[tri(r, j)] *= inv;
    }
    if (!ok) return false;
#pragma unroll
    for (int i = 0; i < 6; ++i) {
        double s = b[i];
#pragma unroll
        for (int k = 0; k < i; ++k) s -= L[tri(i, k)] * x[k];
        x[i] = s * rinv[i];
    }
#pragma unroll
    for (int i = 5; i >= 0; --i) {
        double s = x[i];
#pragma unroll
        for (int k = i + 1; k < 6; ++k) s -= L[tri(k, i)] * x[k];
        x[i] = s * rinv[i];
    }
    return true;
}

__device__ __noinline__ bool lu6_solve(double (*A)[6], double *x) {
    for (int i = 0; i < 6; ++i) {
        int piv = i; double best = fabs(A[i][i]);
        for (int r = i + 1; r < 6; ++r) { const double v = fabs(A[r][i]); if (v > best) { best = v; piv = r; } }
        if (A[piv][i] == 0.0) continue;
        if (piv != i) {
            for (int c = 0; c < 6; ++c) { const double tt = A[i][c]; A[i][c] = A[piv][c]; A[piv][c] = tt; }
            const double tt = x[i]; x[i] = x[piv]; x[piv] = tt;
        }
        const double inv = 1.0 / A[i][i];
        for (int r = i + 1; r < 6; ++r) {
            const double f = A[r][i] * inv;
            A[r][i] = f;
            for (int c = i + 1; c < 6; ++c) A[r][c] -= f * A[i][c];
            x[r] -= f * x[i];
        }
    }
    for (int i = 5; i >= 0; --i) {
        if (A[i][i] == 0.0) return false;
        double s = x[i];
        for (int c = i + 1; c < 6; ++c) s -= A[i][c] * x[c];
        x[i] = s / A[i][i];
    }
    return true;
}

__device__ __forceinline__ void quat_mul_f(const float a[4], const float b[4], float o[4]) {
    const float w = a[3] * b[3] - a[0] * b[0] - a[1] * b[1] - a[2] * b[2];
    const float i = a[3] * b[0] + a[0] * b[3] + a[1] * b[2] - a[2] * b[1];
    const float j = a[3] * b[1] - a[0] * b[2] + a[1] * b[3] + a[2] * b[0];
    const float k = a[3] * b[2] + a[0] * b[1] - a[1] * b[0] + a[2] * b[3];
    o[0] = i; o[1] = j; o[2] = k; o[3] = w;
}

__device__ void compose(const IcpHeader &hd, IcpState *st, const float dq[4], const float dt[3], const GridGeom &g, double searchers, double pairs, int cert_active) {
    if (cert_active != 0) {
        st->searchers = (uint32_t)fmin(searchers, 4.0e9);
        const bool was_on = hd.d_ang >= 0.0f;
        bool wanted = false;
        float ang = -1.0f, tn = 0.0f;
        if (was_on || searchers > 0.1 * pairs) {
            ang = 2.0f * __builtin_amdgcn_sqrtf(dq[0] * dq[0] + dq[1] * dq[1] + dq[2] * dq[2]) * 1.0001f;
            tn = __builtin_amdgcn_sqrtf(dt[0] * dt[0] + dt[1] * dt[1] + dt[2] * dt[2]) * 1.0001f;
            const float rx_ = fmaxf(fabsf(g.minx), fabsf(g.maxx)), ry_ = fmaxf(fabsf(g.miny), fabsf(g.maxy)), rz_ = fmaxf(fabsf(g.minz), fabsf(g.maxz));
            const float far = __builtin_amdgcn_sqrtf(rx_ * rx_ + ry_ * ry_ + rz_ * rz_) * 1.0001f;
            const float moved = ang * far + tn;
            wanted = ang < 5e-3f && moved < (was_on ? 0.01f : 0.003f) * g.h;
        }
        st->d_ang = wanted ? ang : -1.0f;
        st->d_t = tn;
        st->d_run = (wanted && (cert_active & 1)) ? min(hd.d_run + 1u, 1000000u) : 0u;
    }
    const float cq[4] = {hd.q[0], hd.q[1], hd.q[2], hd.q[3]};
    const float ct[3] = {hd.t[0], hd.t[1], hd.t[2]};
    const float zero[3] = {0.0f, 0.0f, 0.0f};
    float rx, ry, rz;
    iso_apply(dq, zero, ct[0], ct[1], ct[2], rx, ry, rz);
    float nq[4];
    quat_mul_f(dq, cq, nq);
    st->q[0] = nq[0]; st->q[1] = nq[1]; st->q[2] = nq[2]; st->q[3] = nq[3];
    st->t[0] = dt[0] + rx; st->t[1] = dt[1] + ry; st->t[2] = dt[2] + rz;
}

__device__ void kabsch_rotation(const double Hin[3][3], double R[3][3]) {
    double H[3][3], V[3][3];
    for (int i = 0; i < 3; ++i) for (int j = 0; j < 3; ++j) { H[i][j] = Hin[i][j]; V[i][j] = (i == j) ? 1.0 : 0.0; }
    for (int sweep = 0; sweep < 30; ++sweep) {
        double off = 0.0;
        for (int p = 0; p < 2; ++p) for (int qq = p + 1; qq < 3; ++qq) {
            double alpha = 0, beta = 0, gamma = 0;
            for (int i = 0; i < 3; ++i) { alpha += H[i][p] * H[i][p]; beta += H[i][qq] * H[i][qq]; gamma += H[i][p] * H[i][qq]; }
            if (gamma == 0.0 || fabs(gamma) <= 1e-18 * sqrt(alpha * beta)) continue;
            off = fmax(off, fabs(gamma) / sqrt(alpha * beta));
            const double zeta = (beta - alpha) / (2.0 * gamma);
            const double tt = (zeta >= 0.0 ? 1.0 : -1.0) / (fabs(zeta) + sqrt(1.0 + zeta * zeta));
            const double c = 1.0 / sqrt(1.0 + tt * tt), s = c * tt;
            for (int i = 0; i < 3; ++i) {
                const double hp = H[i][p], hq = H[i][qq];
                H[i][p] = c * hp - s * hq; H[i][qq] = s * hp + c * hq;
                const double vp = V[i][p], vq = V[i][qq];
                V[i][p] = c * vp - s * vq; V[i][qq] = s * vp + c * vq;
            }
        }
        if (off < 1e-15) break;
    }
    double sig[3], U[3][3];
    for (int j = 0; j < 3; ++j) sig[j] = sqrt(H[0][j] * H[0][j] + H[1][j] * H[1][j] + H[2][j] * H[2][j]);
    int order[3] = {0, 1, 2};
    for (int i = 0; i < 3; ++i) for (int j = i + 1; j < 3; ++j) if (sig[order[j]] > sig[order[i]]) { int t0 = order[i]; order[i] = order[j]; order[j] = t0; }
    const int i0 = order[0], i1 = order[1], i2 = order[2];
    const double smax = sig[i0];
    for (int i = 0; i < 3; ++i) { U[i][i0] = 0; U[i][i1] = 0; U[i][i2] = 0; }
    if (smax > 0.0) for (int i = 0; i < 3; ++i) U[i][i0] = H[i][i0] / smax; else U[0][i0] = 1.0;
    if (sig[i1] > 1e-14 * smax && sig[i1] > 0.0) {
        for (int i = 0; i < 3; ++i) U[i][i1] = H[i][i1] / sig[i1];
    } else {
        double ax = fabs(U[0][i0]), ay = fabs(U[1][i0]), az = fabs(U[2][i0]);
        double e[3] = {0, 0, 0};
        e[(ax <= ay && ax <= az) ? 0 : (ay <= az ? 1 : 2)] = 1.0;
        double d = e[0] * U[0][i0] + e[1] * U[1][i0] + e[2] * U[2][i0];
        double v[3] = {e[0] - d * U[0][i0], e[1] - d * U[1][i0], e[2] - d * U[2][i0]};
        double nv = sqrt(v[0] * v[0] + v[1] * v[1] + v[2] * v[2]);
        for (int i = 0; i < 3; ++i) U[i][i1] = v[i] / nv;
    }
    bool u2_from_cross = !(sig[i2] > 1e-14 * smax && sig[i2] > 0.0);
    if (!u2_from_cross) {
        for (int i = 0; i < 3; ++i) U[i][i2] = H[i][i2] / sig[i2];
    } else {
        U[0][i2] = U[1][i0] * U[2][i1] - U[2][i0] * U[1][i1];
        U[1][i2] = U[2][i0] * U[0][i1] - U[0][i0] * U[2][i1];
        U[2][i2] = U[0][i0] * U[1][i1] - U[1][i0] * U[0][i1];
    }
    for (int i = 0; i < 3; ++i) for (int j = 0; j < 3; ++j) R[i][j] = V[i][0] * U[j][0] + V[i][1] * U[j][1] + V[i][2] * U[j][2];
    const double det = R[0][0] * (R[1][1] * R[2][2] - R[1][2] * R[2][1]) - R[0][1] * (R[1][0] * R[2][2] - R[1][2] * R[2][0]) +
                       R[0][2] * (R[1][0] * R[2][1] - R[1][1] * R[2][0]);
    if (det < 0.0) {
        for (int i = 0; i < 3; ++i) for (int j = 0; j < 3; ++j) R[i][j] -= 2.0 * V[i][i2] * U[j][i2];
    }
}

__device__ void rotmat_to_quat(const double m[3][3], float q[4]) {
    const double tr = m[0][0] + m[1][1] + m[2][2];
    double w, i, j, k;
    if (tr > 0.0) {
        const double d = sqrt(tr + 1.0) * 2.0;
        w = 0.25 * d; i = (m[2][1] - m[1][2]) / d; j = (m[0][2] - m[2][0]) / d; k = (m[1][0] - m[0][1]) / d;
    } else if (m[0][0] > m[1][1] && m[0][0] > m[2][2]) {
        const double d = sqrt(1.0 + m[0][0] - m[1][1] - m[2][2]) * 2.0;
        w = (m[2][1] - m[1][2]) / d; i = 0.25 * d; j = (m[0][1] + m[1][0]) / d; k = (m[0][2] + m[2][0]) / d;
    } else if (m[1][1] > m[2][2]) {
        const double d = sqrt(1.0 + m[1][1] - m[0][0] - m[2][2]) * 2.0;
        w = (m[0][2] - m[2][0]) / d; i = (m[0][1] + m[1][0]) / d; j = 0.25 * d; k = (m[1][2] + m[2][1]) / d;
    } else {
        const double d = sqrt(1.0 + m[2][2] - m[0][0] - m[1][1]) * 2.0;
        w = (m[1][0] - m[0][1]) / d; i = (m[0][2] + m[2][0]) / d; j = (m[1][2] + m[2][1]) / d; k = 0.25 * d;
    }
    const double nq = sqrt(w * w + i * i + j * j + k * k);
    q[0] = (float)(i / nq); q[1] = (float)(j / nq); q[2] = (float)(k / nq); q[3] = (float)(w / nq);
}

__device__ void finish_iteration(const IcpHeader &hd, IcpState *st, float mse, uint32_t n) {
    st->iterations = hd.iterations + 1u;
    st->mse = mse;
    st->n_corr = n;
    const float change = fabsf(hd.prev_mse - mse);
    if (change < hd.conv_thr) { st->converged = 1; st->done = 1; return; }
    st->prev_mse = mse;
}

constexpr int kFinalizeThreads = 512;
template <int MODE>
__device__ void finalize_body(const double *__restrict__ partials, uint32_t nblocks, IcpState *__restrict__ st, const GridGeom &g,
                              int do_sum, int do_apply, double (*sm)[TC_ICP_SUMS_STRIDE], const IcpHeader &hd, int cert_active = 0) {
    const bool done = hd.done != 0;
    constexpr bool P2PLANE = MODE != 0;
    if (do_sum) {
        constexpr int G = kFinalizeThreads / 32;
        {
            const int col = threadIdx.x & 31, grp = threadIdx.x >> 5;
            double s0 = 0.0, s1 = 0.0, s2 = 0.0, s3 = 0.0;
            uint32_t b = grp;
            if (nblocks == 256) {
                double v[256 / G];
#pragma unroll
                for (int k = 0; k < 256 / G; ++k) v[k] = partials[(size_t)(grp + G * k) * TC_ICP_SUMS_STRIDE + col];
#pragma unroll
                for (int k = 0; k < 256 / G; k += 4) { s0 += v[k]; s1 += v[k + 1]; s2 += v[k + 2]; s3 += v[k + 3]; }
                b = 256 + grp;
            }
            for (; b + 3 * G < nblocks; b += 4 * G) {
                s0 += partials[(size_t)b * TC_ICP_SUMS_STRIDE + col];
                s1 += partials[(size_t)(b + G) * TC_ICP_SUMS_STRIDE + col];
                s2 += partials[(size_t)(b + 2 * G) * TC_ICP_SUMS_STRIDE + col];
                s3 += partials[(size_t)(b + 3 * G) * TC_ICP_SUMS_STRIDE + col];
            }
            for (; b < nblocks; b += G) s0 += partials[(size_t)b * TC_ICP_SUMS_STRIDE + col];
            sm[grp][col] = (s0 + s1) + (s2 + s3);
        }
        __syncthreads();
        double tot = 0.0;
        if (threadIdx.x < TC_ICP_SUMS_STRIDE) {
#pragma unroll
            for (int gi = 0; gi < G; ++gi) tot += sm[gi][threadIdx.x];
            if (!done) st->sums[threadIdx.x] = tot;
        }
        __syncthreads();
        if (threadIdx.x < TC_ICP_SUMS_STRIDE) sm[0][threadIdx.x] = tot;
        __syncthreads();
    }
    if (!do_apply || threadIdx.x != 0 || done) return;
    const double *S = do_sum ? &sm[0][0] : st->sums;
    if (P2PLANE) {
        const double cnt = S[28];
        if (cnt < 6.0) { st->status = TC_ALGORITHM; st->done = 1; return; }
        double x[6];
        if (!chol6_solve(S, S + 21, x)) {
            __shared__ double sA[6][6], sx[6];
            int o = 0;
#pragma unroll
            for (int r = 0; r < 6; ++r)
#pragma unroll
                for (int c = r; c < 6; ++c) { sA[r][c] = S[o]; sA[c][r] = S[o]; ++o; }
#pragma unroll
            for (int r = 0; r < 6; ++r) sx[r] = S[21 + r];
            if (!lu6_solve(sA, sx)) { st->status = TC_ALGORITHM; st->done = 1; return; }
#pragma unroll
            for (int r = 0; r < 6; ++r) x[r] = sx[r];
        }
        const float hx = (float)x[0] / 2.0f, hy = (float)x[1] / 2.0f, hz = (float)x[2] / 2.0f;
        float sx, cx, sy, cy, sz, cz;
        sincosf(hx, &sx, &cx); sincosf(hy, &sy, &cy); sincosf(hz, &sz, &cz);
        const float qx[4] = {sx, 0.0f, 0.0f, cx};
        const float qy[4] = {0.0f, sy, 0.0f, cy};
        const float qz[4] = {0.0f, 0.0f, sz, cz};
        float zy[4], rot[4];
        quat_mul_f(qz, qy, zy);
        quat_mul_f(zy, qx, rot);
        const float dt[3] = {(float)x[3], (float)x[4], (float)x[5]};
        compose(hd, st, rot, dt, g, S[kSearchersCol], cnt, cert_active);
        finish_iteration(hd, st, (float)(S[27] / cnt), (uint32_t)cnt);
    } else {
        const double cnt = S[16];
        if (cnt < 3.0) { st->status = TC_ALGORITHM; st->done = 1; return; }
        const double ms[3] = {S[0] / cnt, S[1] / cnt, S[2] / cnt}, mq[3] = {S[3] / cnt, S[4] / cnt, S[5] / cnt};
        double H[3][3], R[3][3];
        for (int r = 0; r < 3; ++r) for (int c = 0; c < 3; ++c) H[r][c] = S[6 + 3 * r + c] - cnt * ms[r] * mq[c];
        if (st->kiss) {
            double hn = 0.0;
            for (int r = 0; r < 3; ++r) for (int c = 0; c < 3; ++c) hn += H[r][c] * H[r][c];
            if (sqrt(hn) < 1e-10) { st->status = TC_ALGORITHM; st->done = 1; return; }
        }
        kabsch_rotation(H, R);
        const double cs[3] = {ms[0] + (double)g.cx, ms[1] + (double)g.cy, ms[2] + (double)g.cz};
        const double cq[3] = {mq[0] + (double)g.cx, mq[1] + (double)g.cy, mq[2] + (double)g.cz};
        float dq[4];
        rotmat_to_quat(R, dq);
        float dt[3];
        for (int r = 0; r < 3; ++r) dt[r] = (float)(cq[r] - (R[r][0] * cs[0] + R[r][1] * cs[1] + R[r][2] * cs[2]));
        compose(hd, st, dq, dt, g, S[kSearchersCol], cnt, cert_active);
        double nmse = S[15];
        if (st->kiss) {
            const double d0 = ms[0] - mq[0], d1 = ms[1] - mq[1], d2 = ms[2] - mq[2];
            double rh = 0.0;
            for (int i = 0; i < 3; ++i) for (int j = 0; j < 3; ++j) rh += R[i][j] * H[j][i];
            nmse = S[15] - cnt * (d0 * d0 + d1 * d1 + d2 * d2) + 2.0 * (H[0][0] + H[1][1] + H[2][2]) - 2.0 * rh;
            nmse = fmax(nmse, 0.0);
        }
        finish_iteration(hd, st, (float)(nmse / cnt), (uint32_t)cnt);
    }
}

template <int MODE>
__global__ void __launch_bounds__(kFinalizeThreads) icp_finalize_kernel(const double *__restrict__ partials, uint32_t nblocks,
                                                           IcpState *__restrict__ st, const GridGeom g, int do_sum, int do_apply,
                                                           int32_t *__restrict__ done_out, int cert_active) {
    const IcpHeader hd = load_header(st);
    __shared__ double sm[kFinalizeThreads / 32][TC_ICP_SUMS_STRIDE];
    if (hd.done && !do_sum) { if (done_out && threadIdx.x == 0) __hip_atomic_store(done_out, 1, __ATOMIC_RELAXED, __HIP_MEMORY_SCOPE_SYSTEM); return; }
#ifdef TC_PHASE_STAMPS
    const unsigned long long t0 = __builtin_amdgcn_s_memtime();
    finalize_body<MODE>(partials, nblocks, st, g, do_sum, 0, sm, hd);
    const unsigned long long t1 = __builtin_amdgcn_s_memtime();
    finalize_body<MODE>(partials, nblocks, st, g, 0, do_apply, sm, hd, cert_active | (done_out != nullptr ? 2 : 0));
    const unsigned long long t2 = __builtin_amdgcn_s_memtime();
    if (threadIdx.x == 0) { st->refine_ring_hist[0] += (uint32_t)(t1 - t0); st->refine_ring_hist[1] += (uint32_t)(t2 - t1); }
#else
    finalize_body<MODE>(partials, nblocks, st, g, do_sum, do_apply, sm, hd, cert_active | (done_out != nullptr ? 2 : 0));
#endif
    if (done_out && threadIdx.x == 0)
        __hip_atomic_store(done_out, (hd.done || st->done) ? 1 : (st->d_ang >= 0.0f ? 3 : 2), __ATOMIC_RELAXED, __HIP_MEMORY_SCOPE_SYSTEM);
}

constexpr int kStateWords = (int)(offsetof(IcpState, sums) / sizeof(uint32_t));
static_assert(kStateWords <= 64, "one lane per word");
__device__ __forceinline__ void publish_state(const IcpState *st, IcpState *host_out, uint32_t *lds) {
    if (threadIdx.x == 0) {
        const uint32_t *s = reinterpret_cast<const uint32_t *>(st);
        for (int i = 0; i < kStateWords; ++i) lds[i] = s[i];
    }
    __syncthreads();
    if ((int)threadIdx.x < kStateWords)
        __hip_atomic_store(reinterpret_cast<uint32_t *>(host_out) + threadIdx.x, lds[threadIdx.x], __ATOMIC_RELAXED, __HIP_MEMORY_SCOPE_SYSTEM);
}
__global__ void icp_finish_kernel(IcpState *__restrict__ st, const double *__restrict__ partials, uint32_t nblocks, int p2plane, int from_sums,
                                  IcpState *__restrict__ host_out) {
    __shared__ uint32_t lds[64];
    if (threadIdx.x == 0 && !st->done) {
    st->converged = 0;
    if (p2plane || st->kiss) {
        st->mse = st->prev_mse;
    } else {
        double s = 0.0, c = 0.0;
        if (from_sums) { s = st->sums[0]; c = st->sums[1]; }
        else for (uint32_t b = 0; b < nblocks; ++b) { s += partials[(size_t)b * TC_ICP_SUMS_STRIDE]; c += partials[(size_t)b * TC_ICP_SUMS_STRIDE + 1]; }
        st->mse = (c > 0.0) ? (float)(s / c) : st->prev_mse;
    }
    st->done = 1;
    }
    if (host_out) publish_state(st, host_out, lds);
}

__global__ void icp_final_mse_fold_kernel(IcpState *__restrict__ st, const double *__restrict__ partials, uint32_t nblocks) {
    if (threadIdx.x >= TC_ICP_SUMS_STRIDE) return;
    double s = 0.0;
    if (threadIdx.x < 2 && !st->done)
        for (uint32_t b = 0; b < nblocks; ++b) s += partials[(size_t)b * TC_ICP_SUMS_STRIDE + threadIdx.x];
    st->sums[threadIdx.x] = s;
}

struct IcpLaunch {
    uint32_t nblocks = 0, chunk = 0;
    uint32_t mse_blocks = 0, mse_chunk = 0;
};
static IcpLaunch plan_launch(size_t ns) {
    IcpLaunch l;
    constexpr size_t kResidentBlocks = 4 * 256;
    size_t chunk = (ns + kResidentBlocks - 1) / kResidentBlocks;
    chunk = std::max<size_t>((chunk + kIcpBlock - 1) / kIcpBlock * kIcpBlock, kIcpBlock);
    uint32_t nb = (uint32_t)((ns + chunk - 1) / chunk);
    nb = std::max<uint32_t>((nb + 7) / 8 * 8, 8);
    l.nblocks = nb; l.chunk = (uint32_t)chunk;
    l.mse_blocks = nb; l.mse_chunk = (uint32_t)chunk;
    return l;
}

static TileGeom plan_tiles(const GridGeom &g, size_t ns) {
    const double rho = (double)ns / std::max<double>(g.ncell, 1.0);
    const double want = 256.0 / std::max(rho, 1e-6);
    static const int cand[][3] = {{8, 2, 2}, {8, 3, 2}, {8, 3, 3}, {8, 4, 3}, {8, 4, 4}, {8, 5, 4}, {8, 5, 5}, {8, 6, 5},
                                  {8, 6, 6}, {10, 6, 6}, {12, 6, 6}, {16, 6, 6}, {16, 8, 8}, {4, 2, 2}, {4, 2, 1}, {2, 2, 1}};
    int best = 0; double bd = 1e300;
    for (int i = 0; i < (int)(sizeof(cand) / sizeof(cand[0])); ++i) {
        const double c = (double)cand[i][0] * cand[i][1] * cand[i][2];
        const double d = std::fabs(std::log(c / want));
        if (d < bd) { bd = d; best = i; }
    }
    return make_tiles(g, cand[best][0], cand[best][1], cand[best][2]);
}

static void launch_iteration(tc_context *ctx, int mode, const GridView &tv, const float4 *nrm, const float4 *src,
                             uint32_t ns, const IcpLaunch &l, IcpState *st, uint32_t *corr_pos, uint32_t *rlist,
                             double *partials, bool do_sum, bool do_apply, bool do_reduce, const float4 *src_cov = nullptr,
                             const float4 *vor = nullptr, int32_t *done_out = nullptr, float4 *wl = nullptr, bool cert = false) {
    hipStream_t s = ctx->stream;
    const int dbg = debug_flags() | (ctx->profiling == 3 ? 8 : 0);
    double *refine_rows = partials + (size_t)l.nblocks * TC_ICP_SUMS_STRIDE;
    if (do_reduce) {
        {
            ProfScope ps(ctx, mode == 1 ? "icp_correspond_reduce_p2plane" : mode == 2 ? "icp_correspond_reduce_gicp" : "icp_correspond_reduce_p2p", true);
            auto kern = mode == 1 ? icp_correspond_reduce_kernel<1> : mode == 2 ? icp_correspond_reduce_kernel<2> : icp_correspond_reduce_kernel<0>;
            if (dbg & 8) kern = mode == 1 ? icp_correspond_reduce_kernel<1, true> : mode == 2 ? icp_correspond_reduce_kernel<2, true> : icp_correspond_reduce_kernel<0, true>;
            cert = cert && wl != nullptr && mode != 2 && !(dbg & 8);
            if (cert) kern = mode == 1 ? icp_correspond_reduce_kernel<1, false, true> : icp_correspond_reduce_kernel<0, false, true>;
            else if (done_out != nullptr && wl != nullptr && mode != 2 && !(dbg & 8))
                kern = mode == 1 ? icp_correspond_reduce_kernel<1, false, false, true> : icp_correspond_reduce_kernel<0, false, false, true>;
            const float4 *vor_arg = (dbg & 4) ? nullptr : vor;
            unsigned long long *times_arg = (dbg & 1024) ? (unsigned long long *)ctx->dbg_times.p : nullptr;
            if (ps.active())
                hipExtLaunchKernelGGL(kern, dim3(l.nblocks), dim3(kIcpBlock), 0, s, ps.e0, ps.e1, 0, tv, nrm, const_cast<float4 *>(src), ns, l.chunk,
                                      (const IcpState *)st, rlist, partials, dbg, src_cov, vor_arg, times_arg, tv.pts12);
            else
                hipLaunchKernelGGL(kern, dim3(l.nblocks), dim3(kIcpBlock), 0, s, tv, nrm, const_cast<float4 *>(src), ns, l.chunk, st, rlist, partials, dbg, src_cov,
                                   vor_arg, times_arg, tv.pts12);
        }
        ProfScope ps(ctx, "icp_refine");
        auto kern = mode == 1 ? icp_refine_kernel<1> : mode == 2 ? icp_refine_kernel<2> : icp_refine_kernel<0>;
        hipLaunchKernelGGL(kern, dim3(kRefineBlocks), dim3(kRefineThreads), 0, s, tv, nrm, src, st, corr_pos, rlist, partials, l.nblocks, l.chunk / (kIcpBlock / 64),
                           refine_rows, src_cov, dbg);
    }
    if (do_sum || do_apply) {
        ProfScope ps(ctx, "icp_finalize");
        const uint32_t rows = kRefineBlocks;
        auto kern = mode == 0 ? icp_finalize_kernel<0> : icp_finalize_kernel<1>;
        hipLaunchKernelGGL(kern, dim3(1), dim3(kFinalizeThreads), 0, s, refine_rows, rows, st, tv.g, do_sum ? 1 : 0, (do_apply && !(dbg & 32)) ? 1 : 0, do_apply ? done_out : nullptr, (cert && do_reduce) ? 1 : 0);
    }
}

static size_t vor_after() {
    static const size_t v = [] { const char *e = getenv("TC_VOR_AFTER"); return e ? (size_t)atoi(e) : (size_t)6; }();
    return v;
}
static tc_status launch_target_nn_bounds(tc_context *ctx, DeviceIndex &ix, const GridView &tv, const IcpState *st, const float4 **out) {
    *out = nullptr;
    if (ix.vor_valid) { *out = (const float4 *)ix.vor.p; return TC_OK; }
    if (tc_status s = ensure(ctx, ix.vor, (size_t)ix.geom.n * sizeof(float4))) return s;
    ProfScope ps(ctx, "icp_target_nn_bounds");
    const bool persistent = &ix != &ctx->tgt_index;
    hipLaunchKernelGGL(icp_target_nn_bound_kernel, dim3((ix.geom.n + 255) / 256), dim3(256), 0, ctx->stream, tv, (float4 *)ix.vor.p,
                       persistent ? nullptr : st);
    ix.vor_valid = persistent;
    *out = (const float4 *)ix.vor.p;
    return TC_OK;
}

__global__ void __launch_bounds__(256) icp_pack12_kernel(const float4 *__restrict__ pts, uint32_t n, uint32_t npad, float *__restrict__ out) {
    const uint32_t i = blockIdx.x * blockDim.x + threadIdx.x;
    if (i >= npad) return;
    float4 r = make_float4(__uint_as_float(0x7F7F7F7Fu), __uint_as_float(0x7F7F7F7Fu), __uint_as_float(0x7F7F7F7Fu), 0.f);
    if (i < n) r = pts[i];
    out[3 * (size_t)i] = r.x; out[3 * (size_t)i + 1] = r.y; out[3 * (size_t)i + 2] = r.z;
}

__global__ void __launch_bounds__(256) icp_working_source_kernel(const float4 *__restrict__ src, uint32_t n, float4 *__restrict__ out, float4 *__restrict__ wl) {
    const uint32_t i = blockIdx.x * blockDim.x + threadIdx.x;
    if (i >= n) return;
    if (wl) wl[i] = make_float4(0.f, 0.f, 0.f, 0.f);
    float4 r = src[i];
    r.w = __uint_as_float(0xFFFFFFFFu);
    out[i] = r;
}

struct IcpSetup {
    IcpLaunch l;
    GridView tv;
    TileGeom tg;
    DeviceIndex *tix = nullptr;
    const float4 *src = nullptr;
    float4 *wsrc = nullptr;
    float4 *wl = nullptr;
};
static inline uint32_t *match_words(float4 *wsrc) { return reinterpret_cast<uint32_t *>(wsrc) + 3; }

static tc_status icp_setup(tc_context *ctx, bool p2plane, const float *d_src, size_t ns, const float *d_tgt, size_t nt,
                           const float *d_nrm, size_t nstride, const float init[7], float max_dist, float conv_thr,
                           IcpSetup &out, int kiss = 0, DeviceIndex *tgt_prebuilt = nullptr, const DeviceIndex *src_presorted = nullptr,
                           bool strict_source_order = false) {
    if (nt >= (1ull << 28) || ns >= (1ull << 28)) return fail(ctx, TC_UNSUPPORTED, "ICP clouds are limited to 2^28 - 1 points");
    out.tix = tgt_prebuilt ? tgt_prebuilt : &ctx->tgt_index;
    if (!tgt_prebuilt) {
        if (tc_status s = build_index(ctx, ctx->tgt_index, d_tgt, nt, kIcpCellFactor, nullptr, nullptr, nullptr, 0.0f, 2.5f)) return s;
        if (tc_status s = wait_uploads(ctx)) return s;
        if (p2plane)
            if (tc_status s = gather_normals(ctx, ctx->tgt_index, d_nrm, nstride)) return s;
    }
    if (tc_status s = wait_uploads(ctx)) return s;
    if (tc_status s = ensure(ctx, ctx->state, sizeof(IcpState))) return s;
    IcpState *hs = (IcpState *)((char *)ctx->pinned + 256);
    std::memset(hs, 0, sizeof(IcpState));
    for (int i = 0; i < 4; ++i) hs->q[i] = init[i];
    for (int i = 0; i < 3; ++i) hs->t[i] = init[4 + i];
    hs->prev_mse = INFINITY;
    hs->d_ang = -1.0f; hs->d_t = 0.0f; hs->d_run = 0;
    hs->conv_thr = conv_thr;
    hs->max_dist = max_dist;
    hs->kiss = kiss;
    hs->status = TC_OK;
    TC_HIP_TRY(ctx, hipMemcpyAsync(ctx->state.p, hs, sizeof(IcpState), hipMemcpyHostToDevice, ctx->stream));
    out.tg = plan_tiles((*out.tix).geom, ns);
    if (src_presorted && src_presorted->geom.n == ns) {
        out.src = (const float4 *)src_presorted->pts.p;
    } else {
        if (ns > 0)
            if (tc_status s = build_index(ctx, ctx->src_index, d_src, ns, 0.0f, &(*out.tix).geom, (const IcpState *)ctx->state.p, &out.tg, 0.0f, 0.0f,
                                          strict_source_order)) return s;
        out.src = (const float4 *)ctx->src_index.pts.p;
    }
    out.l = plan_launch(ns);
    if (tc_status s = ensure(ctx, ctx->partials, ((size_t)(kMaxPartialBlocks + kRefineBlocks) * TC_ICP_SUMS_STRIDE + 2) * sizeof(double))) return s;
    if (tc_status s = ensure(ctx, ctx->corr, (2 * ns + (size_t)kMaxPartialBlocks * (kIcpBlock / 64) + 4 + kRefineEntryWords * (size_t)out.l.nblocks * out.l.chunk) * sizeof(uint32_t))) return s;
    if (!out.tix->pts12_valid) {
        const uint32_t npad = (uint32_t)nt + 16u;
        if (tc_status s = ensure(ctx, out.tix->pts12, (size_t)npad * 12 + 64)) return s;
        ProfScope ps(ctx, "icp_pack12");
        hipLaunchKernelGGL(icp_pack12_kernel, dim3((npad + 255) / 256), dim3(256), 0, ctx->stream, (const float4 *)(*out.tix).pts.p, (uint32_t)nt, npad,
                           (float *)out.tix->pts12.p);
        out.tix->pts12_valid = true;
    }
    out.tv = view_of((*out.tix));
    if (tc_status s = ensure(ctx, ctx->icp_wsrc, 2 * (ns + 4) * sizeof(float4))) return s;
    out.wsrc = (float4 *)ctx->icp_wsrc.p;
    out.wl = out.wsrc + ns + 4;
    if (ns > 0) {
        ProfScope ps(ctx, "icp_working_source");
        hipLaunchKernelGGL(icp_working_source_kernel, dim3((unsigned)((ns + 255) / 256)), dim3(256), 0, ctx->stream, out.src, (uint32_t)ns, out.wsrc, (float4 *)nullptr);
    }
    return TC_OK;
}

__global__ void __launch_bounds__(256) gather_cov_kernel(const float4 *__restrict__ pts_sorted, uint32_t n, const float4 *__restrict__ cov_orig,
                                                        float4 *__restrict__ out) {
    const uint32_t i = blockIdx.x * blockDim.x + threadIdx.x;
    if (i >= n) return;
    const uint32_t o = __float_as_uint(pts_sorted[i].w);
    out[2 * (size_t)i] = cov_orig[2 * (size_t)o];
    out[2 * (size_t)i + 1] = cov_orig[2 * (size_t)o + 1];
}

static tc_status icp_run_mode(tc_context *ctx, int mode, const float *d_src, size_t ns, const float *d_tgt, size_t nt,
                              const float *d_nrm, size_t nstride, const float init[7], size_t max_iters, float max_dist,
                              float conv_thr, tc_icp_result *res, bool corr_on_device, int kiss, const float *d_cov_src,
                              const float *d_cov_tgt, DeviceIndex *tgt_prebuilt = nullptr, const DeviceIndex *src_presorted = nullptr);

tc_status icp_run(tc_context *ctx, bool p2plane, const float *d_src, size_t ns, const float *d_tgt, size_t nt,
                  const float *d_nrm, size_t nstride, const float init[7], size_t max_iters, float max_dist,
                  float conv_thr, tc_icp_result *res, bool corr_on_device, int kiss, DeviceIndex *tgt_prebuilt, const DeviceIndex *src_presorted) {
    return icp_run_mode(ctx, p2plane ? 1 : 0, d_src, ns, d_tgt, nt, d_nrm, nstride, init, max_iters, max_dist, conv_thr, res, corr_on_device,
                        kiss, nullptr, nullptr, tgt_prebuilt, src_presorted);
}

tc_status icp_run_gicp(tc_context *ctx, const float *d_src, size_t ns, const float *d_tgt, size_t nt, const float *d_cov_src,
                       const float *d_cov_tgt, const float init[7], size_t max_iters, float max_dist, float conv_thr,
                       tc_icp_result *res, bool corr_on_device) {
    return icp_run_mode(ctx, 2, d_src, ns, d_tgt, nt, nullptr, 0, init, max_iters, max_dist, conv_thr, res, corr_on_device, 0, d_cov_src,
                        d_cov_tgt);
}

static void fold_search_stats(tc_context *ctx, const IcpState *hs) {
    if (!((debug_flags() & 8) || ctx->profiling == 3)) return;
    const uint32_t *h = hs->refine_ring_hist;
    unsigned long long needed;
    std::memcpy(&needed, &h[3], sizeof(needed));
    ctx->stat_icp[0] += hs->iterations; ctx->stat_icp[1] += h[5]; ctx->stat_icp[2] += h[6]; ctx->stat_icp[3] += h[7];
    ctx->stat_icp[4] += needed; ctx->stat_icp[5] += h[2];
    if (debug_flags() & 8)
        fprintf(stderr, "[tc] icp main pass over %u iterations: wave trips %u, without a search %u (%.1f %%); searches %u, candidate steps needed %llu "
                        "(%.2f per search), steps taken by the trips' slowest lanes %u (%.2f per searching trip): lock-step ratio (lane slots spent / steps needed) %.2f\n",
                hs->iterations, h[5], h[6], 100.0 * h[6] / std::max(h[5], 1u), h[7], needed, (double)needed / std::max(h[7], 1u), h[2],
                (double)h[2] / std::max(h[5] - h[6], 1u), (double)h[2] * 64.0 / std::max<double>((double)needed, 1.0));
}

static tc_status check_iteration_count(tc_context *ctx, const IcpState *hs, size_t max_iters) {
    if (hs->status == TC_OK && !hs->converged && hs->iterations != max_iters)
        return fail(ctx, TC_GPU, "internal error: the ICP loop executed " + std::to_string(hs->iterations) + " of " + std::to_string(max_iters) + " iterations");
    return TC_OK;
}

template <typename F>
static tc_status run_chunked(tc_context *ctx, size_t max_iters, IcpState *dstate, F &&enqueue_iteration) {
    auto chunk_len = [](size_t c) -> size_t { return c == 0 ? 6 : c == 1 ? 2 : c <= 4 ? 4 : 8; };
    size_t nchunks = 0;
    for (size_t covered = 0; covered < max_iters; ++nchunks) covered += chunk_len(nchunks);
    volatile int32_t *flags = (volatile int32_t *)((char *)ctx->pinned + 1024);
    int32_t *d_flags = nullptr;
    TC_HIP_TRY(ctx, hipHostGetDevicePointer((void **)&d_flags, (void *)flags, 0));
    const size_t max_flags = 200;
    size_t it = 0;
    const bool sticky = ctx->icp_cert_hint && nchunks >= 3;
    ctx->icp_cert = sticky;
    struct Hint { tc_context *c; bool wanted; ~Hint() { c->icp_cert_hint = wanted; } } hint{ctx, sticky};
    for (size_t c = 0; c < nchunks; ++c) {
        if (c >= 2 && c - 2 < max_flags) {
            if (tc_status s = wait_pinned_word(ctx, (volatile uint32_t *)&flags[c - 2], "ICP loop")) return s;
            if (flags[c - 2] == 1) break;
            hint.wanted = flags[c - 2] == 3;
            ctx->icp_cert = sticky || hint.wanted;
        }
        if (c < max_flags) flags[c] = 0;
        for (size_t k = 0; k < chunk_len(c) && it < max_iters; ++k, ++it) {
            const bool last = k + 1 == chunk_len(c) || it + 1 == max_iters;
            if (tc_status s = enqueue_iteration((last && c < max_flags) ? d_flags + c : nullptr)) return s;
        }
    }
    return TC_OK;
}

static tc_status icp_run_mode(tc_context *ctx, int mode, const float *d_src, size_t ns, const float *d_tgt, size_t nt,
                              const float *d_nrm, size_t nstride, const float init[7], size_t max_iters, float max_dist,
                              float conv_thr, tc_icp_result *res, bool corr_on_device, int kiss, const float *d_cov_src,
                              const float *d_cov_tgt, DeviceIndex *tgt_prebuilt, const DeviceIndex *src_presorted) {
    const bool p2plane = mode == 1;
    IcpSetup su;
    if (tc_status s = icp_setup(ctx, p2plane, d_src, ns, d_tgt, nt, d_nrm, nstride, init, max_dist, conv_thr, su, kiss, tgt_prebuilt,
                                mode == 2 ? nullptr : src_presorted)) return s;
    hipStream_t st = ctx->stream;
    IcpState *dstate = (IcpState *)ctx->state.p;
    uint32_t *corr = (uint32_t *)ctx->corr.p, *corr_pos = match_words(su.wsrc);
    double *partials = (double *)ctx->partials.p;
    const float4 *src = su.src;
    const float4 *src_cov = nullptr;
    if (mode == 2) {
        if (tc_status s = ensure(ctx, (*su.tix).normals, nt * 2 * sizeof(float4))) return s;
        if (tc_status s = ensure(ctx, ctx->gicp_src_cov, ns * 2 * sizeof(float4))) return s;
        hipLaunchKernelGGL(gather_cov_kernel, dim3((unsigned)((nt + 255) / 256)), dim3(256), 0, st, (const float4 *)(*su.tix).pts.p,
                           (uint32_t)nt, (const float4 *)d_cov_tgt, (float4 *)(*su.tix).normals.p);
        hipLaunchKernelGGL(gather_cov_kernel, dim3((unsigned)((ns + 255) / 256)), dim3(256), 0, st, src, (uint32_t)ns,
                           (const float4 *)d_cov_src, (float4 *)ctx->gicp_src_cov.p);
        src_cov = (const float4 *)ctx->gicp_src_cov.p;
    }
    const float4 *nrm = (const float4 *)(*su.tix).normals.p;

    size_t enq = 0;
    const float4 *vor = su.tix->vor_valid ? (const float4 *)su.tix->vor.p : nullptr;
    if (debug_flags() & 1024)
        if (tc_status s = ensure(ctx, ctx->dbg_times, 10 * (size_t)kMaxPartialBlocks * sizeof(unsigned long long))) return s;
    if (tc_status s = run_chunked(ctx, max_iters, dstate, [&](int32_t *done_out) -> tc_status {
            if (enq++ == vor_after() && !vor)
                if (tc_status s = launch_target_nn_bounds(ctx, (*su.tix), su.tv, dstate, &vor)) return s;
            launch_iteration(ctx, mode, su.tv, nrm, su.wsrc, (uint32_t)ns, su.l, dstate, corr_pos, corr + 2 * ns, partials, true, true, true, src_cov, vor, done_out, su.wl, ctx->icp_cert);
            return TC_OK;
        })) return s;
    if (mode == 0) {
        ProfScope ps(ctx, "icp_final_mse");
        hipLaunchKernelGGL(icp_final_mse_kernel, dim3(su.l.mse_blocks), dim3(kIcpBlock), 0, st, su.tv, (const float4 *)su.wsrc, (uint32_t)ns,
                           su.l.mse_chunk, dstate, corr_pos, partials);
    }
    IcpState *hs = (IcpState *)((char *)ctx->pinned + 640);
    IcpState *hs_dev = (IcpState *)pinned_dev_ptr(ctx, hs);
    if (!hs_dev) return fail(ctx, TC_GPU, "ICP: the pinned block has no device address");
    hs->status = TC_GPU; hs->iterations = 0;
    hipLaunchKernelGGL(icp_finish_kernel, dim3(1), dim3(64), 0, st, dstate, partials, su.l.mse_blocks, mode != 0 ? 1 : 0, 0, pinned_poll_enabled() ? hs_dev : nullptr);
    if (!pinned_poll_enabled()) TC_HIP_TRY(ctx, hipMemcpyAsync(hs, dstate, sizeof(IcpState), hipMemcpyDeviceToHost, st));
    if (res->corr_target) {
        hipLaunchKernelGGL(icp_write_corr_kernel, dim3((unsigned)((ns + 255) / 256)), dim3(256), 0, st, su.tv, src, (uint32_t)ns,
                           corr_pos, corr_on_device ? res->corr_target : corr);
        if (!corr_on_device) TC_HIP_TRY(ctx, hipMemcpyAsync(res->corr_target, corr, ns * sizeof(uint32_t), hipMemcpyDeviceToHost, st));
    }
    TC_HIP_TRY(ctx, hipStreamSynchronize(st));
    TC_HIP_TRY(ctx, hipGetLastError());
    if ((debug_flags() & 1024) && ctx->dbg_times.p) {
        std::vector<unsigned long long> h(2 * (size_t)su.l.nblocks);
        (void)hipMemcpy(h.data(), ctx->dbg_times.p, h.size() * sizeof(unsigned long long), hipMemcpyDeviceToHost);
        unsigned long long t0 = ~0ull, t1 = 0;
        for (size_t b = 0; b < su.l.nblocks; ++b) { t0 = std::min(t0, h[2 * b]); t1 = std::max(t1, h[2 * b + 1]); }
        std::vector<double> dur, endt, startt;
        for (size_t b = 0; b < su.l.nblocks; ++b) { dur.push_back((h[2 * b + 1] - h[2 * b]) * 0.01); endt.push_back((h[2 * b + 1] - t0) * 0.01); startt.push_back((h[2 * b] - t0) * 0.01); }
        std::sort(dur.begin(), dur.end()); std::sort(endt.begin(), endt.end()); std::sort(startt.begin(), startt.end());
        auto q = [](const std::vector<double> &v, double f) { return v[(size_t)(f * (v.size() - 1))]; };
        fprintf(stderr, "[tc] main pass blocks: %u; span %.1f us; block duration us min %.1f p10 %.1f p50 %.1f p90 %.1f p99 %.1f max %.1f; start p50 %.1f p99 %.1f max %.1f; end p10 %.1f p50 %.1f p90 %.1f\n",
                su.l.nblocks, (t1 - t0) * 0.01, dur.front(), q(dur, 0.1), q(dur, 0.5), q(dur, 0.9), q(dur, 0.99), dur.back(), q(startt, 0.5), q(startt, 0.99), startt.back(),
                q(endt, 0.1), q(endt, 0.5), q(endt, 0.9));
#ifdef TC_PHASE_STAMPS
        {
            std::vector<unsigned long long> hp(8 * (size_t)su.l.nblocks);
            (void)hipMemcpy(hp.data(), (unsigned long long *)ctx->dbg_times.p + 2 * kMaxPartialBlocks, hp.size() * sizeof(unsigned long long), hipMemcpyDeviceToHost);
            double m[8] = {0};
            for (size_t b = 0; b < su.l.nblocks; ++b) for (int i = 0; i < 8; ++i) m[i] += (double)hp[8 * b + i] / su.l.nblocks;
            fprintf(stderr, "[tc]   wave 0 phases, mean s_memtime ticks: stage1-2 %.0f  windows %.0f  loop %.0f  post %.0f  stage4 %.0f  fold %.0f  end %.0f\n", m[0], m[1], m[2], m[3], m[4], m[5], m[6]);
        }
#endif
        fprintf(stderr, "[tc]   per XCD (block & 7): mean duration / last end, us:");
        for (int x = 0; x < 8; ++x) {
            double sum = 0, last = 0; int cnt = 0;
            for (size_t b = x; b < su.l.nblocks; b += 8) { sum += (h[2 * b + 1] - h[2 * b]) * 0.01; last = std::max(last, (h[2 * b + 1] - t0) * 0.01); ++cnt; }
            fprintf(stderr, " %.1f/%.1f", sum / std::max(cnt, 1), last);
        }
        fprintf(stderr, "\n");
    }
    fold_search_stats(ctx, hs);
    if (debug_flags() & 64)
        fprintf(stderr, "[tc] icp: searching lanes at the last evaluation of the certificate's gate %u (d_run %u, wanted %d)\n", hs->searchers, hs->d_run, hs->d_ang >= 0.0f ? 1 : 0);
    if (debug_flags() & 64)
        fprintf(stderr, "[tc] icp: %u iterations, refine queries total %u max %u  exit ring hist %u %u %u %u %u %u %u %u\n", hs->iterations,
                hs->refine_total, hs->refine_max, hs->refine_ring_hist[0], hs->refine_ring_hist[1], hs->refine_ring_hist[2], hs->refine_ring_hist[3],
                hs->refine_ring_hist[4], hs->refine_ring_hist[5], hs->refine_ring_hist[6], hs->refine_ring_hist[7]);
    if (hs->status != TC_OK) {
        return fail(ctx, (tc_status)hs->status,
                    mode == 2 ? "GICP: insufficient correspondences (need >= 6) or ill-conditioned Gauss-Newton system"
                    : p2plane ? "Insufficient correspondences for point-to-plane ICP (need >= 6) or ill-conditioned system"
                            : "Insufficient correspondences found");
    }
    if (tc_status s = check_iteration_count(ctx, hs, max_iters)) return s;
    for (int i = 0; i < 4; ++i) res->transformation[i] = hs->q[i];
    for (int i = 0; i < 3; ++i) res->transformation[4 + i] = hs->t[i];
    res->mse = hs->mse;
    res->iterations = hs->converged ? hs->iterations : max_iters;
    res->converged = hs->converged;
    res->n_correspondences = hs->n_corr;
    return TC_OK;
}


__global__ void __launch_bounds__(256) icp_zero_u32_kernel(uint32_t *__restrict__ p, uint32_t n) {
    const uint32_t i = blockIdx.x * blockDim.x + threadIdx.x;
    if (i < n) p[i] = 0u;
}

tc_status icp_run_sharded(tc_context *ctx, tc_comm *comm, int shard_mode, bool p2plane, const float *d_src, size_t ns, const float *d_tgt,
                          size_t nt, const float *d_nrm, size_t nstride, const float init[7], size_t max_iters, float max_dist,
                          float conv_thr, tc_icp_result *res, DeviceIndex *tgt_prebuilt) {
    const int mode = p2plane ? 1 : 0;
    const int W = comm ? comm->nranks : 1, rank = comm ? comm->rank : 0;
    IcpSetup su;
    const size_t rows = (ns + (size_t)W - 1) / (size_t)W;
    size_t ilo = 0, ihi = ns;
    if (shard_mode == TC_SHARD_INDEX) { ilo = std::min((size_t)rank * rows, ns); ihi = std::min(ilo + rows, ns); }
    const size_t n_setup = ihi - ilo;
    tc_status setup_rc = icp_setup(ctx, p2plane, d_src + 3 * ilo, n_setup, d_tgt, nt, d_nrm, nstride, init, max_dist, conv_thr, su, 0, tgt_prebuilt, nullptr,
                                   shard_mode == TC_SHARD_SPATIAL && W > 1);
    if (setup_rc == TC_OK && !su.tix->vor_valid) setup_rc = ensure(ctx, su.tix->vor, (size_t)su.tix->geom.n * sizeof(float4));
    const bool gather_index = shard_mode == TC_SHARD_INDEX && res->corr_target && ns > 0 && (W > 1 || (comm && comm->nccl));
    if (setup_rc == TC_OK && gather_index) setup_rc = ensure(ctx, ctx->out_a, (size_t)W * rows * sizeof(uint32_t));
    if (tc_status s = comm_agree(comm, setup_rc)) return s;
    hipStream_t st = ctx->stream;
    IcpState *dstate = (IcpState *)ctx->state.p;
    size_t lo = 0, hi = n_setup;
    if (shard_mode == TC_SHARD_SPATIAL) { lo = ns * (size_t)rank / (size_t)W; hi = ns * ((size_t)rank + 1) / (size_t)W; }
    const size_t nl = hi - lo;
    const IcpLaunch l = plan_launch(nl);
    uint32_t *corr = (uint32_t *)ctx->corr.p, *rlist = corr + 2 * n_setup;
    double *partials = (double *)ctx->partials.p;
    const float4 *src = su.src + lo;
    float4 *wsrc = su.wsrc + lo;
    uint32_t *corr_pos = match_words(wsrc);
    const float4 *nrm = (const float4 *)(*su.tix).normals.p;
    size_t enq = 0;
    const float4 *vor = su.tix->vor_valid ? (const float4 *)su.tix->vor.p : nullptr;
    if (tc_status s = run_chunked(ctx, max_iters, dstate, [&](int32_t *done_out) -> tc_status {
            if (enq++ == vor_after() && !vor)
                if (tc_status s = launch_target_nn_bounds(ctx, (*su.tix), su.tv, dstate, &vor)) return s;
            launch_iteration(ctx, mode, su.tv, nrm, wsrc, (uint32_t)nl, l, dstate, corr_pos, rlist, partials, true, false, true, nullptr, vor);
            if (tc_status s = comm_allreduce_f64(comm, dstate->sums, TC_ICP_SUMS_STRIDE)) return s;
            launch_iteration(ctx, mode, su.tv, nrm, wsrc, (uint32_t)nl, l, dstate, corr_pos, rlist, partials, false, true, false, nullptr, nullptr, done_out);
            return TC_OK;
        })) return s;
    if (mode == 0) {
        hipLaunchKernelGGL(icp_final_mse_kernel, dim3(l.mse_blocks), dim3(kIcpBlock), 0, st, su.tv, (const float4 *)wsrc, (uint32_t)nl, l.mse_chunk, dstate,
                           corr_pos, partials);
        hipLaunchKernelGGL(icp_final_mse_fold_kernel, dim3(1), dim3(64), 0, st, dstate, partials, l.mse_blocks);
        if (tc_status s = comm_allreduce_f64(comm, dstate->sums, TC_ICP_SUMS_STRIDE)) return s;
    }
    IcpState *hs = (IcpState *)((char *)ctx->pinned + 640);
    IcpState *hs_dev = (IcpState *)pinned_dev_ptr(ctx, hs);
    if (!hs_dev) return fail(ctx, TC_GPU, "ICP: the pinned block has no device address");
    hs->status = TC_GPU; hs->iterations = 0;
    hipLaunchKernelGGL(icp_finish_kernel, dim3(1), dim3(64), 0, st, dstate, partials, 0u, mode != 0 ? 1 : 0, 1, pinned_poll_enabled() ? hs_dev : nullptr);
    if (!pinned_poll_enabled()) TC_HIP_TRY(ctx, hipMemcpyAsync(hs, dstate, sizeof(IcpState), hipMemcpyDeviceToHost, st));
    if (res->corr_target && ns > 0) {
        if (gather_index) {
            uint32_t *all = (uint32_t *)ctx->out_a.p;
            if (nl > 0)
                hipLaunchKernelGGL(icp_write_corr_kernel, dim3((unsigned)((nl + 255) / 256)), dim3(256), 0, st, su.tv, src, (uint32_t)nl, corr_pos,
                                   all + (size_t)rank * rows);
            if (tc_status s = comm_allgather(comm, all, rows * sizeof(uint32_t))) return s;
            TC_HIP_TRY(ctx, hipMemcpyAsync(res->corr_target, all, ns * sizeof(uint32_t), hipMemcpyDeviceToDevice, st));
        } else {
            const bool gather = shard_mode == TC_SHARD_SPATIAL && (W > 1 || (comm && comm->nccl));
            if (gather) hipLaunchKernelGGL(icp_zero_u32_kernel, dim3((unsigned)((ns + 255) / 256)), dim3(256), 0, st, corr, (uint32_t)ns);
            if (nl > 0)
                hipLaunchKernelGGL(icp_write_corr_kernel, dim3((unsigned)((nl + 255) / 256)), dim3(256), 0, st, su.tv, src, (uint32_t)nl, corr_pos, corr);
            if (gather)
                if (tc_status s = comm_allreduce_u32(comm, corr, ns)) return s;
            TC_HIP_TRY(ctx, hipMemcpyAsync(res->corr_target, corr, n_setup * sizeof(uint32_t), hipMemcpyDeviceToDevice, st));
        }
    }
    TC_HIP_TRY(ctx, hipStreamSynchronize(st));
    TC_HIP_TRY(ctx, hipGetLastError());
    fold_search_stats(ctx, hs);
    if (hs->status != TC_OK)
        return fail(ctx, (tc_status)hs->status, p2plane ? "Insufficient correspondences for point-to-plane ICP (need >= 6) or ill-conditioned system"
                                                        : "Insufficient correspondences found");
    if (tc_status s = check_iteration_count(ctx, hs, max_iters)) return s;
    for (int i = 0; i < 4; ++i) res->transformation[i] = hs->q[i];
    for (int i = 0; i < 3; ++i) res->transformation[4 + i] = hs->t[i];
    res->mse = hs->mse;
    res->iterations = hs->converged ? hs->iterations : max_iters;
    res->converged = hs->converged;
    res->n_correspondences = hs->n_corr;
    return TC_OK;
}

}

struct tc_icp_shard {
    tc_context *ctx;
    bool p2plane;
    size_t ns;
    tc::IcpSetup su;
};

extern "C" {

tc_status tc_icp_shard_create(tc_context *ctx, int point_to_plane, const float *d_source_slice, size_t n_source_slice,
                              const float *d_target, size_t n_target, const float *d_target_normals, size_t normal_stride,
                              const float init[7], float max_correspondence_distance, float convergence_threshold,
                              tc_icp_shard **out) try {
    if (!ctx || !out) return TC_INVALID_DATA;
    if (n_source_slice == 0 || n_target == 0) return tc::fail(ctx, TC_INVALID_DATA, "Source or target point cloud is empty");
    if (!point_to_plane) return tc::fail(ctx, TC_UNSUPPORTED, "tc_icp_shard_*: point-to-plane only; use tc_sharded_icp_detailed_device");
    tc_icp_shard *s = new tc_icp_shard{ctx, point_to_plane != 0, n_source_slice, {}};
    tc_status rc = tc::icp_setup(ctx, s->p2plane, d_source_slice, n_source_slice, d_target, n_target, d_target_normals,
                                 normal_stride, init, max_correspondence_distance, convergence_threshold, s->su);
    if (rc != TC_OK) { delete s; return rc; }
    *out = s;
    return TC_OK;
} TC_CATCH_STATUS(ctx)

double *tc_icp_shard_sums(tc_icp_shard *s) { return ((tc::IcpState *)s->ctx->state.p)->sums; }

tc_status tc_icp_shard_get_sums(tc_icp_shard *s, double *d_out) try {
    tc_context *ctx = s->ctx;
    TC_HIP_TRY(ctx, hipMemcpyAsync(d_out, ((tc::IcpState *)ctx->state.p)->sums, TC_ICP_SUMS_STRIDE * sizeof(double),
                                   hipMemcpyDeviceToDevice, ctx->stream));
    return TC_OK;
} TC_CATCH_STATUS((s ? s->ctx : nullptr))

tc_status tc_icp_shard_set_sums(tc_icp_shard *s, const double *d_in) try {
    tc_context *ctx = s->ctx;
    TC_HIP_TRY(ctx, hipMemcpyAsync(((tc::IcpState *)ctx->state.p)->sums, d_in, TC_ICP_SUMS_STRIDE * sizeof(double),
                                   hipMemcpyDeviceToDevice, ctx->stream));
    return TC_OK;
} TC_CATCH_STATUS((s ? s->ctx : nullptr))

tc_status tc_icp_shard_done(tc_icp_shard *s, int *done) try {
    tc_context *ctx = s->ctx;
    int32_t *h = (int32_t *)((char *)ctx->pinned + 1024);
    TC_HIP_TRY(ctx, hipMemcpyAsync(h, &((tc::IcpState *)ctx->state.p)->done, sizeof(int32_t), hipMemcpyDeviceToHost, ctx->stream));
    TC_HIP_TRY(ctx, hipStreamSynchronize(ctx->stream));
    *done = *h;
    return TC_OK;
} TC_CATCH_STATUS((s ? s->ctx : nullptr))

tc_status tc_icp_shard_reduce(tc_icp_shard *s) try {
    tc_context *ctx = s->ctx;
    uint32_t *corr = (uint32_t *)ctx->corr.p;
    tc::launch_iteration(ctx, s->p2plane, s->su.tv, (const float4 *)ctx->tgt_index.normals.p, s->su.wsrc,
                         (uint32_t)s->ns, s->su.l, (tc::IcpState *)ctx->state.p, tc::match_words(s->su.wsrc), corr + 2 * s->ns,
                         (double *)ctx->partials.p, true, false, true);
    TC_HIP_TRY(ctx, hipGetLastError());
    return TC_OK;
} TC_CATCH_STATUS((s ? s->ctx : nullptr))

tc_status tc_icp_shard_apply(tc_icp_shard *s) try {
    tc_context *ctx = s->ctx;
    uint32_t *corr = (uint32_t *)ctx->corr.p;
    tc::launch_iteration(ctx, s->p2plane, s->su.tv, (const float4 *)ctx->tgt_index.normals.p, s->su.wsrc,
                         (uint32_t)s->ns, s->su.l, (tc::IcpState *)ctx->state.p, tc::match_words(s->su.wsrc), corr + 2 * s->ns,
                         (double *)ctx->partials.p, false, true, false);
    TC_HIP_TRY(ctx, hipGetLastError());
    return TC_OK;
} TC_CATCH_STATUS((s ? s->ctx : nullptr))

tc_status tc_icp_shard_finish(tc_icp_shard *s, size_t max_iters, tc_icp_result *res) try {
    tc_context *ctx = s->ctx;
    hipStream_t st = ctx->stream;
    tc::IcpState *dstate = (tc::IcpState *)ctx->state.p;
    hipLaunchKernelGGL(tc::icp_finish_kernel, dim3(1), dim3(64), 0, st, dstate, (const double *)ctx->partials.p, 0u, 1, 0, (tc::IcpState *)nullptr);
    tc::IcpState *hs = (tc::IcpState *)((char *)ctx->pinned + 256);
    TC_HIP_TRY(ctx, hipMemcpyAsync(hs, dstate, sizeof(tc::IcpState), hipMemcpyDeviceToHost, st));
    if (res->corr_target) {
        uint32_t *corr = (uint32_t *)ctx->corr.p;
        hipLaunchKernelGGL(tc::icp_write_corr_kernel, dim3((unsigned)((s->ns + 255) / 256)), dim3(256), 0, st, s->su.tv,
                           (const float4 *)ctx->src_index.pts.p, (uint32_t)s->ns, tc::match_words(s->su.wsrc), corr);
        TC_HIP_TRY(ctx, hipMemcpyAsync(res->corr_target, corr, s->ns * sizeof(uint32_t), hipMemcpyDeviceToDevice, st));
    }
    TC_HIP_TRY(ctx, hipStreamSynchronize(st));
    tc::fold_search_stats(ctx, hs);
    if (hs->status != TC_OK) return tc::fail(ctx, (tc_status)hs->status, "ICP failed (insufficient correspondences / singular system)");
    for (int i = 0; i < 4; ++i) res->transformation[i] = hs->q[i];
    for (int i = 0; i < 3; ++i) res->transformation[4 + i] = hs->t[i];
    res->mse = hs->mse;
    res->iterations = hs->converged ? hs->iterations : max_iters;
    res->converged = hs->converged;
    res->n_correspondences = hs->n_corr;
    return TC_OK;
} TC_CATCH_STATUS((s ? s->ctx : nullptr))

void tc_icp_shard_destroy(tc_icp_shard *s) { delete s; }

}
```

threecrate_amd/csrc/tc_internal.h:

```cpp
#pragma once
#include <hip/hip_runtime.h>
#include <stddef.h>
#include <stdint.h>
#include <new>
#include <exception>
#include <string>
#include <vector>

#include "../../include/threecrate_hip.h"

namespace tc {

struct GridGeom {
    float minx, miny, minz;
    float maxx, maxy, maxz;
    float h, inv_h;
    int   gx, gy, gz;
    uint32_t ncell;
    uint32_t n;
    float cx, cy, cz;
    int   clamped;
};

struct TileGeom {
    int tx, ty, tz;
    int ntx, nty, ntz;
    uint32_t cpt;
    uint32_t ntiles;
};

struct GridView {
    GridGeom g;
    const float4   *pts;
    const uint32_t *cell_start;
    const float    *pts12;
};

struct IcpState {
    float    q[4];
    float    t[3];
    float    prev_mse;
    float    mse;
    uint32_t iterations;
    int32_t  converged;
    int32_t  status;
    int32_t  done;
    uint32_t n_corr;
    float    conv_thr;
    float    max_dist;
    int32_t  kiss;
    uint32_t refine_total;
    uint32_t refine_max;
    uint32_t refine_ring_hist[8];
    float    d_ang;
    float    d_t;
    uint32_t d_run;
    uint32_t searchers;
    double   sums[TC_ICP_SUMS_STRIDE];
};

static_assert(offsetof(IcpState, refine_ring_hist) % 8 == 4 && offsetof(IcpState, sums) % 8 == 0,
              "refine_ring_hist[3..4] is ONE 64-bit counter of the statistics instantiation (icp.hip): it must sit on an 8-byte boundary");
constexpr int kIcpBlock = 256;
constexpr size_t kPtsPad = 4, kCellStartPad = 4;
constexpr size_t kCellStartFront = 4;
constexpr uint32_t kRankQuadraticMax = 1u << 20;
constexpr int kMaxPartialBlocks = 1024;
constexpr uint32_t kAdaptMinPoints = 1u << 18;

#if defined(__HIPCC__)
__device__ __forceinline__ uint32_t tile_major_id(const TileGeom &t, int cx, int cy, int cz) {
    const int ax = cx / t.tx, ay = cy / t.ty, az = cz / t.tz;
    const int lx = cx - ax * t.tx, ly = cy - ay * t.ty, lz = cz - az * t.tz;
    const uint32_t tile = ((uint32_t)az * t.nty + ay) * t.ntx + ax;
    return tile * t.cpt + ((uint32_t)lz * t.ty + ly) * t.tx + lx;
}
__device__ __forceinline__ float d2_nc(float ax, float ay, float az, float bx, float by, float bz) {
    float dx = ax - bx, dy = ay - by, dz = az - bz;
    return dx * dx + dy * dy + dz * dz;
}
__device__ __forceinline__ int cell_coord(float v, float mn, float inv_h, int g) {
    float f = (v - mn) * inv_h;
    int c = (f >= 0.0f) ? (int)f : 0;
    return c < g ? c : g - 1;
}
#endif

struct DevBuf {
    void  *p = nullptr;
    size_t cap = 0;
};

struct ScopedBuf : DevBuf {
    ScopedBuf() = default;
    ScopedBuf(const ScopedBuf &) = delete; ScopedBuf &operator=(const ScopedBuf &) = delete;
    ~ScopedBuf() { if (p) (void)hipFree(p); }
};

struct KernelTimer {
    std::string name;
    std::vector<std::pair<hipEvent_t, hipEvent_t>> pending;
    uint64_t launches = 0;
    double   total_ms = 0.0;
    double   min_ms = 1e300, max_ms = 0.0;
};

struct DeviceIndex {
    GridGeom geom{};
    TileGeom tile{};
    float exact_min[3] = {0, 0, 0}, exact_max[3] = {0, 0, 0};
    DevBuf pts;
    DevBuf cell_start;
    DevBuf normals;
    DevBuf vor;
    bool vor_valid = false;
    DevBuf pts12;
    bool pts12_valid = false;
    uint32_t occ_host = 0;
    bool occ_host_valid = false;
    DevBuf cell_of;
    DevBuf slot;
    DevBuf arrival;
    DevBuf fill;
    DevBuf blocksum;
};
template <class F> void for_each_scratch_buf(DeviceIndex &ix, F f) { for (DevBuf *b : {&ix.cell_of, &ix.slot, &ix.arrival, &ix.fill, &ix.blocksum}) f(*b); }
template <class F> void for_each_buf(DeviceIndex &ix, F f) {
    for (DevBuf *b : {&ix.pts, &ix.cell_start, &ix.normals, &ix.vor, &ix.pts12}) f(*b);
    for_each_scratch_buf(ix, f);
}

enum CluSlot {
    CLU_PARENT, CLU_SIZE, CLU_MIN_INDEX,
    CLU_FLAG, CLU_POS,
    CLU_KEYS,
    CLU_ROOTS,
    CLU_RANK_OF, CLU_SIZES,
    CLU_LABELS, CLU_SORT_TEMP, CLU_COMP,
    CLU_SLOTS
};
enum FpfhSlot {
    FPFH_XYZ, FPFH_SPFH, FPFH_MODE,
    FPFH_FB_POS, FPFH_FB_XYZ, FPFH_FB_COUNT,
    FPFH_SORTED_OF,
    FPFH_KNN_IDX, FPFH_KNN_DIST, FPFH_KNN_COUNT,
    FPFH_SLOTS
};

}

struct tc_context {
    int device = 0;
    hipStream_t stream = nullptr;
    bool own_stream = true;
    std::string last_error;
    int profiling = 0;
    uint32_t prof_tick = 0;
    std::vector<tc::KernelTimer> timers;
    std::vector<hipEvent_t> event_pool;
    std::vector<tc::DevBuf> pool;
    size_t pool_bytes = 0;
    size_t pool_largest = 0;
    hipEvent_t order_event = nullptr;
    hipEvent_t release_event = nullptr;
    std::vector<hipEvent_t> chunk_events;
    hipStream_t copy_stream = nullptr;
    hipEvent_t upload_event = nullptr;
    bool upload_pending = false;
    bool upload_used_copy_stream = false;

    tc::DeviceIndex tgt_index;
    tc::DeviceIndex src_index;
    tc::DevBuf in_a, in_b, in_c;
    tc::DevBuf out_a;
    tc::DevBuf bbox;
    tc::DevBuf state;
    tc::DevBuf partials;
    tc::DevBuf corr;
    tc::DevBuf gicp_src_cov;
    tc::DevBuf icp_wsrc;
    tc::DevBuf dbg_times;
    tc::DevBuf overflow;
    tc::DevBuf build_tmp;
    tc::DevBuf normals_hard;
    unsigned long long stat_indexed_points = 0, stat_index_builds = 0;
    unsigned long long stat_icp[6] = {0, 0, 0, 0, 0, 0};
    bool icp_cert = false;
    bool icp_cert_hint = false;
    bool normals_hard_clean = false;
    tc::DeviceIndex vox_index;
    tc::DevBuf clu[tc::CLU_SLOTS];
    tc::DevBuf fpfh[tc::FPFH_SLOTS];
    tc::DevBuf fpfh_np;
    void *pinned = nullptr;
    void *pinned_dev = nullptr;
    size_t pinned_cap = 0;
};
template <class F> void for_each_buf(tc_context &c, F f) {
    for (tc::DeviceIndex *ix : {&c.tgt_index, &c.src_index, &c.vox_index}) tc::for_each_buf(*ix, f);
    for (auto &b : c.clu) f(b);
    for (auto &b : c.fpfh) f(b);
    for (tc::DevBuf *b : {&c.fpfh_np, &c.in_a, &c.in_b, &c.in_c, &c.out_a, &c.bbox, &c.state, &c.partials, &c.corr, &c.gicp_src_cov,
                          &c.overflow, &c.normals_hard, &c.build_tmp, &c.dbg_times, &c.icp_wsrc}) f(*b);
}

struct tc_comm {
    tc_context *ctx = nullptr;
    int rank = 0, nranks = 1;
    void *nccl = nullptr;
    bool own_nccl = false;
    tc_host_collective_fn host_fn = nullptr;
    void *host_user = nullptr;
    void *agree_word = nullptr;
};

namespace tc {

tc_status fail(tc_context *ctx, tc_status st, const std::string &msg);
tc_status fail_nothrow(tc_context *ctx, tc_status st, const char *msg) noexcept;
void fault_point(const char *site);
#define TC_CATCH_STATUS(CTX)                                                                                            \
    catch (const std::bad_alloc &) { return tc::fail_nothrow((CTX), TC_GPU, "out of host memory"); }                    \
    catch (const std::exception &e_) { return tc::fail_nothrow((CTX), TC_GPU, e_.what()); }                             \
    catch (...) { return tc::fail_nothrow((CTX), TC_GPU, "unknown C++ exception"); }
#define TC_CATCH_VOID catch (...) { }
#define TC_CATCH_VALUE(V) catch (...) { return V; }
#define TC_HIP_TRY(ctx, expr)                                                                  \
    do {                                                                                       \
        hipError_t _e = (expr);                                                                \
        if (_e != hipSuccess)                                                                  \
            return tc::fail((ctx), TC_GPU, std::string(#expr) + ": " + hipGetErrorString(_e)); \
    } while (0)

tc_status ensure(tc_context *ctx, DevBuf &b, size_t bytes);
constexpr size_t kMaxPoints = 0xFFFFFFF0ull, kMaxK = 2048;
inline tc_status check_point_count(tc_context *ctx, size_t a, size_t b = 0) {
    return (a >= kMaxPoints || b >= kMaxPoints) ? fail(ctx, TC_UNSUPPORTED, "more than 2^32 points") : TC_OK;
}
tc_status upload_async(tc_context *ctx, void *d_dst, const void *h_src, size_t bytes);
tc_status uploads_issued(tc_context *ctx);
tc_status wait_uploads(tc_context *ctx);
void *pinned_dev_ptr(tc_context *ctx, const void *host_addr);
bool pinned_poll_enabled();
tc_status wait_pinned_word(tc_context *ctx, volatile uint32_t *word, const char *what);
void recycle(tc_context *ctx, DevBuf &b);

struct ProfScope {
    tc_context *ctx; int idx = -1; hipEvent_t e0 = nullptr, e1 = nullptr; bool ext = false;
    ProfScope(tc_context *c, const char *name, bool dominant = false);
    ~ProfScope();
    bool active() const { return idx >= 0; }
};

tc_status build_index(tc_context *ctx, DeviceIndex &ix, const float *d_xyz, size_t n,
                      float cell_factor, const GridGeom *reuse_geom, const IcpState *d_state_transform,
                      const TileGeom *tile_major = nullptr, float min_cell_edge = 0.0f, float target_ppo = 0.0f, bool strict_order = false);
TileGeom make_tiles(const GridGeom &g, int tx, int ty, int tz);
tc_status gather_normals(tc_context *ctx, DeviceIndex &ix, const float *d_normals, size_t stride);
GridView view_of(const DeviceIndex &ix);

tc_status exclusive_scan_u32(tc_context *ctx, const uint32_t *d_in, uint32_t n, uint32_t *d_out , DevBuf &blocksum, uint32_t *occ_out = nullptr,
                             unsigned long long *occ_host = nullptr);
tc_status cloud_bbox(tc_context *ctx, const float *d_xyz, size_t n, float mn[3], float mx[3]);

tc_status voxel_filter_device(tc_context *ctx, const float *d_xyz, size_t n, float voxel, float *d_out, size_t *n_out);
tc_status range_filter_device(tc_context *ctx, const float *d_xyz, size_t n, float min_range, float max_range, float *d_out, size_t *n_out);

tc_status cluster_extract_device(tc_context *ctx, const float *d_xyz, size_t n, float tol, size_t min_size, size_t max_size,
                                 uint32_t *d_labels, uint32_t *d_members, uint64_t *d_offsets, size_t *n_clusters);

tc_status fpfh_device(tc_context *ctx, const float *d_np6, size_t n, float radius, size_t k, float *d_out);

tc_status launch_normals(tc_context *ctx, const DeviceIndex &ix, const float *d_xyz, const tc_normal_config &cfg,
                         const float vp[3], float *d_out6, size_t p_begin = 0, size_t p_end = (size_t)-1, bool slice_out = false,
                         float4 *d_sorted_nrm = nullptr, float4 *d_vor = nullptr);
tc_status normals_on_index(tc_context *ctx, DeviceIndex &ix, bool build, float cell_factor_override, const float *d_xyz, size_t n,
                           const tc_normal_config *cfg, float *d_out6, size_t p_begin, size_t p_end, bool slice_out, float4 *d_sorted_nrm,
                           bool with_bounds = false);
float normals_cell_factor(size_t k, bool large);
float normals_target_ppo(size_t k);
constexpr float kIcpCellFactor = 1.13f;
void free_index(DeviceIndex &ix);
void recycle_index(tc_context *ctx, DeviceIndex &ix);
tc_status launch_radius_all(tc_context *ctx, const DeviceIndex &ix, const float *d_queries, size_t nq, float radius, uint32_t *d_counts,
                            const unsigned long long *d_offsets, uint32_t *d_idx, float *d_dist);
tc_status launch_normals_unsort(tc_context *ctx, const DeviceIndex &ix, const float *d_sorted6, float *d_out6);

tc_status launch_knn(tc_context *ctx, const DeviceIndex &ix, const float *d_queries, size_t nq, size_t k,
                     uint32_t *d_idx, float *d_dist, uint32_t *d_count, float radius_sq = INFINITY);

int debug_flags();

tc_status comm_allreduce_f64(tc_comm *comm, double *d_buf, size_t count);
tc_status comm_allreduce_u32(tc_comm *comm, uint32_t *d_buf, size_t count);
tc_status comm_allgather(tc_comm *comm, void *d_buf, size_t bytes_per_rank);
tc_status comm_agree(tc_comm *comm, tc_status local);

tc_status icp_run_sharded(tc_context *ctx, tc_comm *comm, int shard_mode, bool p2plane, const float *d_src, size_t ns, const float *d_tgt,
                          size_t nt, const float *d_nrm, size_t nstride, const float init[7], size_t max_iters, float max_dist,
                          float conv_thr, tc_icp_result *res, DeviceIndex *tgt_prebuilt = nullptr);
tc_status icp_run(tc_context *ctx, bool p2plane, const float *d_src, size_t ns, const float *d_tgt, size_t nt,
                  const float *d_nrm, size_t nstride, const float init[7], size_t max_iters,
                  float max_dist, float conv_thr, tc_icp_result *res, bool corr_on_device, int kiss = 0,
                  DeviceIndex *tgt_prebuilt = nullptr, const DeviceIndex *src_presorted = nullptr);
tc_status icp_run_gicp(tc_context *ctx, const float *d_src, size_t ns, const float *d_tgt, size_t nt, const float *d_cov_src,
                       const float *d_cov_tgt, const float init[7], size_t max_iters, float max_dist, float conv_thr,
                       tc_icp_result *res, bool corr_on_device);

}
```

Baseline: 18130 it/s.

## Fuse bbox into cloud upload copy and emit side buffers during index build

Device-to-device cloud creation now runs a copy kernel that also reduces the bounding box (plus sampled sub-boxes) into a per-cloud pinned slot, so the later index build reuses it instead of launching a separate bbox pass. The binned placement kernel now also writes the packed xyz (pts12) target layout and the ICP working-source buffer, which removes separate conversion and working-source passes. The ICP finish reduction is folded into the correspondence-write kernel when correspondences are requested. These changes cut kernel launches and redundant reads of 1M-point arrays, at the cost of a slot ring, extra state and more complex kernels.

```diff
diff --git a/threecrate_amd/csrc/cloud.hip b/threecrate_amd/csrc/cloud.hip
--- a/threecrate_amd/csrc/cloud.hip
+++ b/threecrate_amd/csrc/cloud.hip
@@ -14,6 +14,8 @@
     bool has_normals = false;
     tc::DevBuf normals6;
     bool has_normals6 = false;
+    int box_slot = -1;
+    tc::PendingBox box;
 };
 
 namespace {
@@ -49,7 +51,14 @@
         c->has_normals6 = true;
     }
     c->has_normals = false;
-    if (tc_status s = build_index(ctx, c->ix, (const float *)c->xyz.p, c->n, f, nullptr, nullptr, nullptr, min_h, target_ppo)) return s;
+    BuildExtras ex;
+    if (f == kIcpCellFactor) {
+        if (tc_status s = ensure(ctx, c->ix.pts12, (c->n + 16) * 12 + 64)) return s;
+        ex.pts12 = (float *)c->ix.pts12.p;
+    }
+    if (tc_status s = build_index(ctx, c->ix, (const float *)c->xyz.p, c->n, f, nullptr, nullptr, nullptr, min_h, target_ppo, false,
+                                  c->box_slot >= 0 ? &c->box : nullptr, &ex)) return s;
+    c->ix.pts12_valid = ex.made;
     c->indexed = true;
     c->factor = f;
     return TC_OK;
@@ -65,6 +74,17 @@
     c->n = n;
     if (n) {
         tc_status s = ensure(ctx, c->xyz, n * 3 * sizeof(float));
+        if (s == TC_OK && !from_host) {
+            for (int k = 0; k < kBoxRing && c->box_slot < 0; ++k)
+                if (!ctx->box_slot_busy[k]) c->box_slot = k;
+            if (c->box_slot >= 0) {
+                s = copy_with_box(ctx, (float *)c->xyz.p, p, n, c->box_slot, &c->box);
+                if (s == TC_OK) ctx->box_slot_busy[c->box_slot] = true; else c->box_slot = -1;
+                if (s != TC_OK) { recycle(ctx, c->xyz); delete c; return s; }
+                *out = c;
+                return TC_OK;
+            }
+        }
         if (s == TC_OK && hipMemcpyAsync(c->xyz.p, p, n * 3 * sizeof(float), from_host ? hipMemcpyHostToDevice : hipMemcpyDeviceToDevice,
                                          ctx->stream) != hipSuccess) s = fail(ctx, TC_GPU, "cloud upload failed");
         if (s == TC_OK && from_host && hipStreamSynchronize(ctx->stream) != hipSuccess) s = fail(ctx, TC_GPU, "cloud upload failed");
@@ -213,6 +233,7 @@
     if (!c) return;
     (void)hipSetDevice(c->ctx->device);
     (void)hipStreamSynchronize(c->ctx->stream);
+    if (c->box_slot >= 0) c->ctx->box_slot_busy[c->box_slot] = false;
     tc::recycle(c->ctx, c->xyz); tc::recycle(c->ctx, c->normals6);
     tc::recycle_index(c->ctx, c->ix);
     delete c;
diff --git a/threecrate_amd/csrc/grid.hip b/threecrate_amd/csrc/grid.hip
--- a/threecrate_amd/csrc/grid.hip
+++ b/threecrate_amd/csrc/grid.hip
@@ -126,6 +126,157 @@
     if (t < 30) state[(t + 1) * kBboxAccStride] = (t % 6 < 3) ? kOrdPlusInf : kOrdMinusInf;
 }
 
+
+constexpr int kCopyBoxBlocks = 512;
+constexpr size_t kCopyBoxRowsOffset = 128;
+constexpr size_t kCopyBoxBufBytes = kCopyBoxRowsOffset + ((size_t)kCopyBoxBlocks + kBoxRing) * 32 * sizeof(float);
+template <bool VEC>
+__global__ void __launch_bounds__(256) cloud_copy_box_kernel(const float *__restrict__ src, float *__restrict__ dst, uint32_t n,
+                                                            uint32_t *__restrict__ ticket, float *__restrict__ rows,
+                                                            float *__restrict__ out, uint32_t *__restrict__ done) {
+    __shared__ float sm[8][32];
+    float v[30];
+#pragma unroll
+    for (int k = 0; k < 30; ++k) v[k] = (k % 6 < 3) ? INFINITY : -INFINITY;
+    auto take = [&](float x, float y, float z, uint32_t i, int s) __attribute__((always_inline)) {
+        if (!(fabsf(x) <= 3.0e38f && fabsf(y) <= 3.0e38f && fabsf(z) <= 3.0e38f)) return;
+        v[0] = fminf(v[0], x); v[1] = fminf(v[1], y); v[2] = fminf(v[2], z);
+        v[3] = fmaxf(v[3], x); v[4] = fmaxf(v[4], y); v[5] = fmaxf(v[5], z);
+        const bool drawn = ((i * 2654435761u) >> 28) == 0u;
+#pragma unroll
+        for (int k = 0; k < 4; ++k) {
+            const bool on = drawn && k == s;
+            v[6 + 6 * k] = on ? fminf(v[6 + 6 * k], x) : v[6 + 6 * k]; v[7 + 6 * k] = on ? fminf(v[7 + 6 * k], y) : v[7 + 6 * k];
+            v[8 + 6 * k] = on ? fminf(v[8 + 6 * k], z) : v[8 + 6 * k]; v[9 + 6 * k] = on ? fmaxf(v[9 + 6 * k], x) : v[9 + 6 * k];
+            v[10 + 6 * k] = on ? fmaxf(v[10 + 6 * k], y) : v[10 + 6 * k]; v[11 + 6 * k] = on ? fmaxf(v[11 + 6 * k], z) : v[11 + 6 * k];
+        }
+    };
+    auto take_any = [&](float x, float y, float z, uint32_t i) __attribute__((always_inline)) { take(x, y, z, i, (int)(i & 3u)); };
+    const uint32_t gt = blockIdx.x * blockDim.x + threadIdx.x, stride = gridDim.x * blockDim.x;
+    if constexpr (VEC) {
+        const float4 *__restrict__ q = reinterpret_cast<const float4 *>(src);
+        float4 *__restrict__ w = reinterpret_cast<float4 *>(dst);
+        const uint32_t nq = n >> 2;
+        constexpr int U = 2;
+        for (uint32_t c0 = gt; c0 < nq; c0 += U * stride) {
+            float4 a[U], b[U], c[U];
+#pragma unroll
+            for (int u = 0; u < U; ++u) {
+                const uint32_t cc = c0 + (uint32_t)u * stride;
+                if (cc < nq) { a[u] = q[3 * (size_t)cc]; b[u] = q[3 * (size_t)cc + 1]; c[u] = q[3 * (size_t)cc + 2]; }
+            }
+#pragma unroll
+            for (int u = 0; u < U; ++u) {
+                const uint32_t cc = c0 + (uint32_t)u * stride;
+                if (cc < nq) {
+                    w[3 * (size_t)cc] = a[u]; w[3 * (size_t)cc + 1] = b[u]; w[3 * (size_t)cc + 2] = c[u];
+                    const uint32_t i = 4u * cc;
+                    take(a[u].x, a[u].y, a[u].z, i, 0);
+                    take(a[u].w, b[u].x, b[u].y, i + 1u, 1);
+                    take(b[u].z, b[u].w, c[u].x, i + 2u, 2);
+                    take(c[u].y, c[u].z, c[u].w, i + 3u, 3);
+                }
+            }
+        }
+        if (gt < (n & 3u)) {
+            const uint32_t i = (nq << 2) + gt;
+            const float x = src[3 * (size_t)i], y = src[3 * (size_t)i + 1], z = src[3 * (size_t)i + 2];
+            dst[3 * (size_t)i] = x; dst[3 * (size_t)i + 1] = y; dst[3 * (size_t)i + 2] = z;
+            take_any(x, y, z, i);
+        }
+    } else {
+        for (uint32_t i = gt; i < n; i += stride) {
+            const float x = src[3 * (size_t)i], y = src[3 * (size_t)i + 1], z = src[3 * (size_t)i + 2];
+            dst[3 * (size_t)i] = x; dst[3 * (size_t)i + 1] = y; dst[3 * (size_t)i + 2] = z;
+            take_any(x, y, z, i);
+        }
+    }
+#pragma unroll
+    for (int k = 0; k < 30; ++k) {
+#pragma unroll
+        for (int o = 32; o > 0; o >>= 1) {
+            const float t = __shfl_xor(v[k], o);
+            v[k] = (k % 6 < 3) ? fminf(v[k], t) : fmaxf(v[k], t);
+        }
+    }
+    if ((threadIdx.x & 63) == 0) {
+#pragma unroll
+        for (int k = 0; k < 30; ++k) sm[threadIdx.x >> 6][k] = v[k];
+    }
+    __syncthreads();
+    __shared__ uint32_t s_last;
+    if (threadIdx.x < 64) {
+        if (threadIdx.x < 30) {
+            const bool is_min = threadIdx.x % 6 < 3;
+            float r = sm[0][threadIdx.x];
+            for (int k = 1; k < 4; ++k) r = is_min ? fminf(r, sm[k][threadIdx.x]) : fmaxf(r, sm[k][threadIdx.x]);
+            __hip_atomic_store(&rows[(size_t)blockIdx.x * 32 + threadIdx.x], r, __ATOMIC_RELAXED, __HIP_MEMORY_SCOPE_AGENT);
+        }
+        asm volatile("s_waitcnt vmcnt(0)" ::: "memory");
+        if (threadIdx.x == 0) s_last = __hip_atomic_fetch_add(ticket, 1u, __ATOMIC_RELAXED, __HIP_MEMORY_SCOPE_AGENT) == gridDim.x - 1u ? 1u : 0u;
+    }
+    __syncthreads();
+    if (!s_last) return;
+    {
+        const uint32_t k = threadIdx.x & 31u, g8 = threadIdx.x >> 5;
+        const bool is_min = k % 6 < 3;
+        float r = is_min ? INFINITY : -INFINITY;
+        if (k < 30u)
+            for (uint32_t b = g8; b < gridDim.x; b += 8u) {
+                const float t = __hip_atomic_load(&rows[(size_t)b * 32 + k], __ATOMIC_RELAXED, __HIP_MEMORY_SCOPE_AGENT);
+                r = is_min ? fminf(r, t) : fmaxf(r, t);
+            }
+        sm[g8][k] = r;
+    }
+    __syncthreads();
+    if (threadIdx.x < 30) {
+        const bool is_min = threadIdx.x % 6 < 3;
+        float r = sm[0][threadIdx.x];
+        for (int k = 1; k < 8; ++k) r = is_min ? fminf(r, sm[k][threadIdx.x]) : fmaxf(r, sm[k][threadIdx.x]);
+        __hip_atomic_store(&out[threadIdx.x], r, __ATOMIC_RELAXED, __HIP_MEMORY_SCOPE_SYSTEM);
+    }
+    if (threadIdx.x == 0) __hip_atomic_store(ticket, 0u, __ATOMIC_RELAXED, __HIP_MEMORY_SCOPE_AGENT);
+    if (done) {
+        if (threadIdx.x < 30) __threadfence_system();
+        __syncthreads();
+        if (threadIdx.x == 0) __hip_atomic_store(done, 1u, __ATOMIC_RELEASE, __HIP_MEMORY_SCOPE_SYSTEM);
+    }
+}
+
+tc_status copy_with_box(tc_context *ctx, float *d_dst, const float *d_src, size_t n, int slot, PendingBox *out) {
+    if (n == 0 || n >= kMaxPoints || slot < 0 || slot >= kBoxRing) return fail(ctx, TC_INVALID_DATA, "copy_with_box: bad arguments");
+    hipStream_t st = ctx->stream;
+    if (!ctx->box_rows.p) {
+        if (tc_status s = ensure(ctx, ctx->box_rows, kCopyBoxBufBytes)) return s;
+        TC_HIP_TRY(ctx, hipMemsetAsync(ctx->box_rows.p, 0, kCopyBoxRowsOffset, st));
+    }
+    uint32_t *ticket = (uint32_t *)ctx->box_rows.p;
+    float *rows = (float *)((char *)ctx->box_rows.p + kCopyBoxRowsOffset);
+    float *h_vals = (float *)((char *)ctx->pinned + kBoxRingOffset + (size_t)slot * kBoxSlotBytes);
+    volatile uint32_t *h_flag = (volatile uint32_t *)(h_vals + 30);
+    float *d_out = rows + ((size_t)kCopyBoxBlocks + slot) * 32;
+    uint32_t *d_done = nullptr;
+    *out = PendingBox{};
+    if (pinned_poll_enabled()) {
+        d_out = (float *)pinned_dev_ptr(ctx, h_vals);
+        d_done = (uint32_t *)pinned_dev_ptr(ctx, (const void *)h_flag);
+        if (!d_out || !d_done) return fail(ctx, TC_GPU, "cloud upload: the pinned block has no device address");
+        *h_flag = 0u;
+        out->h_flag = h_flag; out->h_vals = h_vals;
+    } else {
+        out->d_vals = d_out;
+    }
+    const uint32_t n32 = (uint32_t)n;
+    ProfScope ps(ctx, "cloud_copy_box");
+    if ((((uintptr_t)d_src | (uintptr_t)d_dst) & 15u) == 0u)
+        hipLaunchKernelGGL(cloud_copy_box_kernel<true>, dim3(std::min<unsigned>((n32 / 4 + 255) / 256 + 1, kCopyBoxBlocks)), dim3(256), 0, st, d_src, d_dst, n32,
+                           ticket, rows, d_out, d_done);
+    else
+        hipLaunchKernelGGL(cloud_copy_box_kernel<false>, dim3(std::min<unsigned>((n32 + 255) / 256, kCopyBoxBlocks)), dim3(256), 0, st, d_src, d_dst, n32,
+                           ticket, rows, d_out, d_done);
+    TC_HIP_TRY(ctx, hipGetLastError());
+    return TC_OK;
+}
 
 __global__ void __launch_bounds__(256) cell_hist_kernel(const float *__restrict__ xyz, uint32_t n, GridGeom g,
                                                        const IcpState *__restrict__ st, TileGeom tg, int tile_major, uint32_t nkeys,
@@ -415,17 +566,31 @@
 }
 
 static tc_status cloud_bbox_impl(tc_context *ctx, const float *d_xyz, size_t n, float mn[3], float mx[3], float *rmn, float *rmx,
-                                 bool *clamped) {
+                                 bool *clamped, const PendingBox *box = nullptr) {
     hipStream_t st = ctx->stream;
     const int nb = (int)((n + 255) / 256);
     const int bb = std::min(nb, kBboxBlocks);
     const bool robust = rmn != nullptr && n >= 4096;
+    float known[30];
+    if (box) {
+        if (box->h_flag) {
+            if (tc_status s = wait_pinned_word(ctx, box->h_flag, "bounding box (cloud upload)")) return s;
+            std::memcpy(known, box->h_vals, sizeof(known));
+        } else {
+            float *hb2 = (float *)((char *)ctx->pinned + 2048);
+            TC_HIP_TRY(ctx, hipMemcpyAsync(hb2, box->d_vals, 30 * sizeof(float), hipMemcpyDeviceToHost, st));
+            TC_HIP_TRY(ctx, hipStreamSynchronize(st));
+            std::memcpy(known, hb2, sizeof(known));
+        }
+    }
+    float *hb = (float *)((char *)ctx->pinned + 2048);
+    if (box) hb = known;
+    else {
     const bool poll = pinned_poll_enabled();
     const bool fresh = ctx->bbox.p == nullptr;
     if (tc_status s = ensure(ctx, ctx->bbox, kBboxBufBytes)) return s;
     uint32_t *d_state = (uint32_t *)ctx->bbox.p;
     if (fresh) hipLaunchKernelGGL(bbox_state_init_kernel, dim3(1), dim3(64), 0, st, d_state);
-    float *hb = (float *)((char *)ctx->pinned + 2048);
     volatile uint32_t *h_done = (volatile uint32_t *)((char *)ctx->pinned + 2048 + 8192 + 192);
     float *d_out = (float *)((char *)ctx->bbox.p + kBboxStateBytes + 128);
     uint32_t *d_done = nullptr;
@@ -448,6 +613,7 @@
     } else {
         TC_HIP_TRY(ctx, hipMemcpyAsync(hb, d_out, 30 * sizeof(float), hipMemcpyDeviceToHost, st));
         TC_HIP_TRY(ctx, hipStreamSynchronize(st));
+    }
     }
     const float *hs = hb + 6;
     for (int c = 0; c < 3; ++c) { mn[c] = INFINITY; mx[c] = -INFINITY; }
@@ -618,7 +784,8 @@
                                                                      const IcpState *__restrict__ st, TileGeom tg, int tile_major,
                                                                      uint32_t *__restrict__ cs, float4 *__restrict__ pts,
                                                                      uint32_t *__restrict__ occ_ticket, uint32_t *__restrict__ occ_out,
-                                                                     unsigned long long *__restrict__ occ_host) {
+                                                                     unsigned long long *__restrict__ occ_host,
+                                                                     float *__restrict__ pts12, float4 *__restrict__ wsrc) {
     __shared__ uint32_t cnt[kBinKeysMax];
     __shared__ uint32_t rkey[kBinCap];
     __shared__ uint32_t ridx[kBinCap];
@@ -682,7 +849,13 @@
     __syncthreads();
     for (uint32_t i = tid; i < P; i += kBinPlaceThreads) slot[rkey[i]] = i;
     __syncthreads();
-    for (uint32_t t = tid; t < P; t += kBinPlaceThreads) pts[bs + t] = tmp[bs + slot[t]];
+    for (uint32_t t = tid; t < P; t += kBinPlaceThreads) {
+        float4 r = tmp[bs + slot[t]];
+        pts[bs + t] = r;
+        if (pts12) { float *o = pts12 + 3 * (size_t)(bs + t); o[0] = r.x; o[1] = r.y; o[2] = r.z; }
+        if (wsrc) { r.w = __uint_as_float(0xFFFFFFFFu); wsrc[bs + t] = r; }
+    }
+    if (pts12 && bin == nbins - 1 && tid < 48u) pts12[3 * (size_t)g.n + tid] = __uint_as_float(0x7F7F7F7Fu);
     if (tid == 0) {
         const unsigned long long mine = ((unsigned long long)s_occ << 32) | 1ull;
         const unsigned long long old = __hip_atomic_fetch_add(reinterpret_cast<unsigned long long *>(occ_ticket), mine, __ATOMIC_RELAXED, __HIP_MEMORY_SCOPE_AGENT);
@@ -706,8 +879,9 @@
 
 tc_status build_index(tc_context *ctx, DeviceIndex &ix, const float *d_xyz, size_t n, float cell_factor,
                       const GridGeom *reuse_geom, const IcpState *d_state_transform, const TileGeom *tile_major,
-                      float min_cell_edge, float target_ppo, bool strict_order) {
+                      float min_cell_edge, float target_ppo, bool strict_order, const PendingBox *box, BuildExtras *extras) {
     if (n == 0 || n >= kMaxPoints) return fail(ctx, TC_INVALID_DATA, "build_index: bad point count");
+    if (extras) extras->made = false;
     ctx->stat_indexed_points += n;
     ctx->stat_index_builds += 1;
     ix.vor_valid = false;
@@ -725,7 +899,7 @@
     } else {
         float mn[3], mx[3], rmn[3], rmx[3];
         bool clamped = false;
-        if (tc_status s = cloud_bbox_impl(ctx, d_xyz, n, mn, mx, rmn, rmx, &clamped)) return s;
+        if (tc_status s = cloud_bbox_impl(ctx, d_xyz, n, mn, mx, rmn, rmx, &clamped, box)) return s;
         if (dbg & 2048) clamped = false, std::memcpy(rmn, mn, sizeof(mn)), std::memcpy(rmx, mx, sizeof(mx));
         for (int c = 0; c < 3; ++c) {
             if (!(mn[c] <= mx[c]) || !std::isfinite(mn[c]) || !std::isfinite(mx[c])) { mn[c] = 0.0f; mx[c] = 0.0f; rmn[c] = 0.0f; rmx[c] = 0.0f; }
@@ -765,6 +939,7 @@
         volatile uint32_t *h_occ = (volatile uint32_t *)((char *)ctx->pinned + 2048 + 8192);
 
         bool binned_done = false;
+        if (extras) extras->made = false;
         if (binned_build_enabled() && pinned_poll_enabled() && !strict_order && n >= kAdaptMinPoints && n <= (1u << 24) && nkeys < 0x7FFFFFF0u) {
             const uint32_t keys = nkeys + 1u;
             uint32_t nbins = std::max<uint32_t>((n32 + kBinTarget - 1) / kBinTarget, (keys + kBinKeysMax - 1) / kBinKeysMax);
@@ -799,12 +974,14 @@
                     ProfScope ps(ctx, "cell_bin_place");
                     hipLaunchKernelGGL(bin_place_kernel, dim3(nbins), dim3(kBinPlaceThreads), 0, st, (const float4 *)ctx->build_tmp.p, (const uint32_t *)binstart,
                                        nbins, kpb, nkeys, g, d_state_transform, tg, tile_major ? 1 : 0, cs, (float4 *)ix.pts.p, occ_ticket,
-                                       (uint32_t *)ix.cell_start.p, d_occ_host);
+                                       (uint32_t *)ix.cell_start.p, d_occ_host, extras ? extras->pts12 : (float *)nullptr,
+                                       extras ? extras->wsrc : (float4 *)nullptr);
                 }
                 TC_HIP_TRY(ctx, hipGetLastError());
                 if (tc_status s = wait_pinned_word(ctx, h_max + 1, "index build (bin populations)")) return s;
                 if (h_max[0] <= kBinCap) {
                     binned_done = true;
+                    if (extras) extras->made = extras->pts12 || extras->wsrc;
                 } else if (dbg & 256) {
                     fprintf(stderr, "[tc] index: largest bin holds %u points (> %u): atomic counting sort\n", h_max[0], kBinCap);
                 }
diff --git a/threecrate_amd/csrc/icp.hip b/threecrate_amd/csrc/icp.hip
--- a/threecrate_amd/csrc/icp.hip
+++ b/threecrate_amd/csrc/icp.hip
@@ -1017,9 +1017,17 @@
     }
 }
 
+struct IcpFinishArgs { IcpState *st; const double *partials; uint32_t nblocks; int p2plane; IcpState *host_out; };
+__device__ __forceinline__ void icp_finish_body(IcpState *st, const double *partials, uint32_t nblocks, int p2plane, int from_sums);
+__device__ __forceinline__ void publish_state(const IcpState *st, IcpState *host_out, uint32_t *lds);
 __global__ void __launch_bounds__(256) icp_write_corr_kernel(GridView tgt, const float4 *__restrict__ src, uint32_t ns,
                                                             const uint32_t *__restrict__ corr_pos,
-                                                            uint32_t *__restrict__ corr) {
+                                                            uint32_t *__restrict__ corr, IcpFinishArgs fin) {
+    if (fin.st && blockIdx.x == 0) {
+        __shared__ uint32_t lds[64];
+        if (threadIdx.x == 0) icp_finish_body(fin.st, fin.partials, fin.nblocks, fin.p2plane, 0);
+        if (fin.host_out) publish_state(fin.st, fin.host_out, lds);
+    }
     const uint32_t j = blockIdx.x * blockDim.x + threadIdx.x;
     if (j >= ns) return;
     const uint32_t so = __float_as_uint(src[j].w);
@@ -1406,10 +1414,8 @@
     if ((int)threadIdx.x < kStateWords)
         __hip_atomic_store(reinterpret_cast<uint32_t *>(host_out) + threadIdx.x, lds[threadIdx.x], __ATOMIC_RELAXED, __HIP_MEMORY_SCOPE_SYSTEM);
 }
-__global__ void icp_finish_kernel(IcpState *__restrict__ st, const double *__restrict__ partials, uint32_t nblocks, int p2plane, int from_sums,
-                                  IcpState *__restrict__ host_out) {
-    __shared__ uint32_t lds[64];
-    if (threadIdx.x == 0 && !st->done) {
+__device__ __forceinline__ void icp_finish_body(IcpState *st, const double *partials, uint32_t nblocks, int p2plane, int from_sums) {
+    if (st->done) return;
     st->converged = 0;
     if (p2plane || st->kiss) {
         st->mse = st->prev_mse;
@@ -1420,7 +1426,11 @@
         st->mse = (c > 0.0) ? (float)(s / c) : st->prev_mse;
     }
     st->done = 1;
-    }
+}
+__global__ void icp_finish_kernel(IcpState *__restrict__ st, const double *__restrict__ partials, uint32_t nblocks, int p2plane, int from_sums,
+                                  IcpState *__restrict__ host_out) {
+    __shared__ uint32_t lds[64];
+    if (threadIdx.x == 0) icp_finish_body(st, partials, nblocks, p2plane, from_sums);
     if (host_out) publish_state(st, host_out, lds);
 }
 
@@ -1548,7 +1558,7 @@
 static tc_status icp_setup(tc_context *ctx, bool p2plane, const float *d_src, size_t ns, const float *d_tgt, size_t nt,
                            const float *d_nrm, size_t nstride, const float init[7], float max_dist, float conv_thr,
                            IcpSetup &out, int kiss = 0, DeviceIndex *tgt_prebuilt = nullptr, const DeviceIndex *src_presorted = nullptr,
-                           bool strict_source_order = false) {
+                           bool strict_source_order = false, bool wsrc_from_build = false) {
     if (nt >= (1ull << 28) || ns >= (1ull << 28)) return fail(ctx, TC_UNSUPPORTED, "ICP clouds are limited to 2^28 - 1 points");
     out.tix = tgt_prebuilt ? tgt_prebuilt : &ctx->tgt_index;
     if (!tgt_prebuilt) {
@@ -1571,12 +1581,20 @@
     hs->status = TC_OK;
     TC_HIP_TRY(ctx, hipMemcpyAsync(ctx->state.p, hs, sizeof(IcpState), hipMemcpyHostToDevice, ctx->stream));
     out.tg = plan_tiles((*out.tix).geom, ns);
+    if (tc_status s = ensure(ctx, ctx->icp_wsrc, 2 * (ns + 4) * sizeof(float4))) return s;
+    out.wsrc = (float4 *)ctx->icp_wsrc.p;
+    out.wl = out.wsrc + ns + 4;
+    bool wsrc_made = false;
     if (src_presorted && src_presorted->geom.n == ns) {
         out.src = (const float4 *)src_presorted->pts.p;
     } else {
-        if (ns > 0)
+        if (ns > 0) {
+            BuildExtras ex;
+            if (wsrc_from_build && !strict_source_order) ex.wsrc = out.wsrc;
             if (tc_status s = build_index(ctx, ctx->src_index, d_src, ns, 0.0f, &(*out.tix).geom, (const IcpState *)ctx->state.p, &out.tg, 0.0f, 0.0f,
-                                          strict_source_order)) return s;
+                                          strict_source_order, nullptr, &ex)) return s;
+            wsrc_made = ex.made;
+        }
         out.src = (const float4 *)ctx->src_index.pts.p;
     }
     out.l = plan_launch(ns);
@@ -1591,10 +1609,7 @@
         out.tix->pts12_valid = true;
     }
     out.tv = view_of((*out.tix));
-    if (tc_status s = ensure(ctx, ctx->icp_wsrc, 2 * (ns + 4) * sizeof(float4))) return s;
-    out.wsrc = (float4 *)ctx->icp_wsrc.p;
-    out.wl = out.wsrc + ns + 4;
-    if (ns > 0) {
+    if (ns > 0 && !wsrc_made) {
         ProfScope ps(ctx, "icp_working_source");
         hipLaunchKernelGGL(icp_working_source_kernel, dim3((unsigned)((ns + 255) / 256)), dim3(256), 0, ctx->stream, out.src, (uint32_t)ns, out.wsrc, (float4 *)nullptr);
     }
@@ -1685,7 +1700,7 @@
     const bool p2plane = mode == 1;
     IcpSetup su;
     if (tc_status s = icp_setup(ctx, p2plane, d_src, ns, d_tgt, nt, d_nrm, nstride, init, max_dist, conv_thr, su, kiss, tgt_prebuilt,
-                                mode == 2 ? nullptr : src_presorted)) return s;
+                                mode == 2 ? nullptr : src_presorted, false, mode != 2)) return s;
     hipStream_t st = ctx->stream;
     IcpState *dstate = (IcpState *)ctx->state.p;
     uint32_t *corr = (uint32_t *)ctx->corr.p, *corr_pos = match_words(su.wsrc);
@@ -1722,11 +1737,17 @@
     IcpState *hs_dev = (IcpState *)pinned_dev_ptr(ctx, hs);
     if (!hs_dev) return fail(ctx, TC_GPU, "ICP: the pinned block has no device address");
     hs->status = TC_GPU; hs->iterations = 0;
-    hipLaunchKernelGGL(icp_finish_kernel, dim3(1), dim3(64), 0, st, dstate, partials, su.l.mse_blocks, mode != 0 ? 1 : 0, 0, pinned_poll_enabled() ? hs_dev : nullptr);
-    if (!pinned_poll_enabled()) TC_HIP_TRY(ctx, hipMemcpyAsync(hs, dstate, sizeof(IcpState), hipMemcpyDeviceToHost, st));
+    IcpState *const pub = pinned_poll_enabled() ? hs_dev : nullptr;
+    const bool finish_in_write_out = res->corr_target != nullptr && ns > 0;
+    if (!finish_in_write_out) {
+        hipLaunchKernelGGL(icp_finish_kernel, dim3(1), dim3(64), 0, st, dstate, partials, su.l.mse_blocks, mode != 0 ? 1 : 0, 0, pub);
+        if (!pub) TC_HIP_TRY(ctx, hipMemcpyAsync(hs, dstate, sizeof(IcpState), hipMemcpyDeviceToHost, st));
+    }
     if (res->corr_target) {
+        const IcpFinishArgs fin = finish_in_write_out ? IcpFinishArgs{dstate, partials, su.l.mse_blocks, mode != 0 ? 1 : 0, pub} : IcpFinishArgs{};
         hipLaunchKernelGGL(icp_write_corr_kernel, dim3((unsigned)((ns + 255) / 256)), dim3(256), 0, st, su.tv, src, (uint32_t)ns,
-                           corr_pos, corr_on_device ? res->corr_target : corr);
+                           corr_pos, corr_on_device ? res->corr_target : corr, fin);
+        if (finish_in_write_out && !pub) TC_HIP_TRY(ctx, hipMemcpyAsync(hs, dstate, sizeof(IcpState), hipMemcpyDeviceToHost, st));
         if (!corr_on_device) TC_HIP_TRY(ctx, hipMemcpyAsync(res->corr_target, corr, ns * sizeof(uint32_t), hipMemcpyDeviceToHost, st));
     }
     TC_HIP_TRY(ctx, hipStreamSynchronize(st));
@@ -1844,14 +1865,14 @@
             uint32_t *all = (uint32_t *)ctx->out_a.p;
             if (nl > 0)
                 hipLaunchKernelGGL(icp_write_corr_kernel, dim3((unsigned)((nl + 255) / 256)), dim3(256), 0, st, su.tv, src, (uint32_t)nl, corr_pos,
-                                   all + (size_t)rank * rows);
+                                   all + (size_t)rank * rows, IcpFinishArgs{});
             if (tc_status s = comm_allgather(comm, all, rows * sizeof(uint32_t))) return s;
             TC_HIP_TRY(ctx, hipMemcpyAsync(res->corr_target, all, ns * sizeof(uint32_t), hipMemcpyDeviceToDevice, st));
         } else {
             const bool gather = shard_mode == TC_SHARD_SPATIAL && (W > 1 || (comm && comm->nccl));
             if (gather) hipLaunchKernelGGL(icp_zero_u32_kernel, dim3((unsigned)((ns + 255) / 256)), dim3(256), 0, st, corr, (uint32_t)ns);
             if (nl > 0)
-                hipLaunchKernelGGL(icp_write_corr_kernel, dim3((unsigned)((nl + 255) / 256)), dim3(256), 0, st, su.tv, src, (uint32_t)nl, corr_pos, corr);
+                hipLaunchKernelGGL(icp_write_corr_kernel, dim3((unsigned)((nl + 255) / 256)), dim3(256), 0, st, su.tv, src, (uint32_t)nl, corr_pos, corr, IcpFinishArgs{});
             if (gather)
                 if (tc_status s = comm_allreduce_u32(comm, corr, ns)) return s;
             TC_HIP_TRY(ctx, hipMemcpyAsync(res->corr_target, corr, n_setup * sizeof(uint32_t), hipMemcpyDeviceToDevice, st));
@@ -1954,7 +1975,7 @@
     if (res->corr_target) {
         uint32_t *corr = (uint32_t *)ctx->corr.p;
         hipLaunchKernelGGL(tc::icp_write_corr_kernel, dim3((unsigned)((s->ns + 255) / 256)), dim3(256), 0, st, s->su.tv,
-                           (const float4 *)ctx->src_index.pts.p, (uint32_t)s->ns, tc::match_words(s->su.wsrc), corr);
+                           (const float4 *)ctx->src_index.pts.p, (uint32_t)s->ns, tc::match_words(s->su.wsrc), corr, tc::IcpFinishArgs{});
         TC_HIP_TRY(ctx, hipMemcpyAsync(res->corr_target, corr, s->ns * sizeof(uint32_t), hipMemcpyDeviceToDevice, st));
     }
     TC_HIP_TRY(ctx, hipStreamSynchronize(st));
diff --git a/threecrate_amd/csrc/tc_internal.h b/threecrate_amd/csrc/tc_internal.h
--- a/threecrate_amd/csrc/tc_internal.h
+++ b/threecrate_amd/csrc/tc_internal.h
@@ -97,6 +97,20 @@
     ~ScopedBuf() { if (p) (void)hipFree(p); }
 };
 
+constexpr int kBoxRing = 4;
+constexpr size_t kBoxRingOffset = 16384, kBoxSlotBytes = 128;
+struct PendingBox {
+    volatile uint32_t *h_flag = nullptr;
+    const float *h_vals = nullptr;
+    const float *d_vals = nullptr;
+};
+
+struct BuildExtras {
+    float *pts12 = nullptr;
+    float4 *wsrc = nullptr;
+    bool made = false;
+};
+
 struct KernelTimer {
     std::string name;
     std::vector<std::pair<hipEvent_t, hipEvent_t>> pending;
@@ -174,6 +188,8 @@
     tc::DevBuf in_a, in_b, in_c;
     tc::DevBuf out_a;
     tc::DevBuf bbox;
+    tc::DevBuf box_rows;
+    bool box_slot_busy[tc::kBoxRing] = {};
     tc::DevBuf state;
     tc::DevBuf partials;
     tc::DevBuf corr;
@@ -200,7 +216,7 @@
     for (tc::DeviceIndex *ix : {&c.tgt_index, &c.src_index, &c.vox_index}) tc::for_each_buf(*ix, f);
     for (auto &b : c.clu) f(b);
     for (auto &b : c.fpfh) f(b);
-    for (tc::DevBuf *b : {&c.fpfh_np, &c.in_a, &c.in_b, &c.in_c, &c.out_a, &c.bbox, &c.state, &c.partials, &c.corr, &c.gicp_src_cov,
+    for (tc::DevBuf *b : {&c.fpfh_np, &c.in_a, &c.in_b, &c.in_c, &c.out_a, &c.bbox, &c.box_rows, &c.state, &c.partials, &c.corr, &c.gicp_src_cov,
                           &c.overflow, &c.normals_hard, &c.build_tmp, &c.dbg_times, &c.icp_wsrc}) f(*b);
 }
 
@@ -254,7 +270,9 @@
 
 tc_status build_index(tc_context *ctx, DeviceIndex &ix, const float *d_xyz, size_t n,
                       float cell_factor, const GridGeom *reuse_geom, const IcpState *d_state_transform,
-                      const TileGeom *tile_major = nullptr, float min_cell_edge = 0.0f, float target_ppo = 0.0f, bool strict_order = false);
+                      const TileGeom *tile_major = nullptr, float min_cell_edge = 0.0f, float target_ppo = 0.0f, bool strict_order = false,
+                      const PendingBox *box = nullptr, BuildExtras *extras = nullptr);
+tc_status copy_with_box(tc_context *ctx, float *d_dst, const float *d_src, size_t n, int slot, PendingBox *out);
 TileGeom make_tiles(const GridGeom &g, int tx, int ty, int tz);
 tc_status gather_normals(tc_context *ctx, DeviceIndex &ix, const float *d_normals, size_t stride);
 GridView view_of(const DeviceIndex &ix);
```

New measurement: 17960 it/s. Within noise of the previous version (-0.9%).
